# kolinko/effort

Measured on AMD Instinct MI355X. Metric: effective GB/s + tokens/s vs effort %, Mistral-7B FFN 4096x11008 fp16, higher is better.
Workload: dtype f16

## Files before the change

### effort_amd/_lib.py

```python
from __future__ import annotations

import ctypes as C
import os
import subprocess

_HERE = os.path.dirname(os.path.abspath(__file__))
LAB_LIB_PATH = os.path.join(_HERE, "libeffort_hip_lab.so")
LIB_PATH = (LAB_LIB_PATH if os.environ.get("EFFORT_HIP_LIB") == "lab" else os.environ.get("EFFORT_HIP_LIB")) or os.path.join(_HERE, "libeffort_hip.so")

ERRORS = {
    -1: "EFFORT_ERR_ARG", -2: "EFFORT_ERR_SHAPE", -3: "EFFORT_ERR_EFFORT", -4: "EFFORT_ERR_HIP",
    -5: "EFFORT_ERR_KIND", -6: "EFFORT_ERR_CONVERT", -7: "EFFORT_ERR_BLAS", -8: "EFFORT_ERR_COMM",
}


class EffortError(RuntimeError):
    def __init__(self, code: int, where: str, detail: str = ""):
        self.code = code
        super().__init__(f"{where}: {ERRORS.get(code, code)} {detail}".strip())


def build(verbose: bool = False) -> str:
    cmd = ["make", "-C", os.path.join(_HERE, "csrc"), "-j8", "all"]
    res = subprocess.run(cmd, capture_output=not verbose, text=True)
    if res.returncode != 0:
        raise RuntimeError("building libeffort_hip.so failed:\n" + (res.stdout or "") + (res.stderr or ""))
    return LIB_PATH


_P = C.c_void_p
_SIGS = {
    "effort_create": (_P, [C.c_int, _P]),
    "effort_destroy": (None, [_P]),
    "effort_set_stream": (C.c_int, [_P, _P]),
    "effort_sync": (C.c_int, [_P]),
    "effort_set_overlap": (C.c_int, [_P, C.c_int]),
    "effort_set_row_reuse": (C.c_int, [_P, C.c_int]),
    "effort_join": (C.c_int, [_P]),
    "effort_last_error": (C.c_char_p, [_P]),
    "effort_version": (C.c_char_p, []),
    "effort_weights_fp16": (_P, [_P, _P, _P, _P, C.c_int, C.c_int, C.c_int, C.c_int]),
    "effort_weights_fp16_pitched": (_P, [_P, _P, C.c_int, _P, _P, C.c_int, C.c_int, C.c_int, C.c_int]),
    "effort_aligned_row_pitch": (C.c_int, [C.c_int]),
    "effort_weights_q4": (_P, [_P, _P, _P, _P, _P, C.c_int64, C.c_int, C.c_int, C.c_int]),
    "effort_weights_free": (None, [_P]),
    "effort_weights_refresh": (C.c_int, [_P]),
    "effort_weights_align_rows": (C.c_int, [_P]),
    "effort_weights_row_pitch": (C.c_int, [_P]),
    "effort_weights_get_bound": (C.c_int, [_P, C.POINTER(C.c_float)]),
    "effort_weights_set_bound": (C.c_int, [_P, C.POINTER(C.c_float)]),
    "effort_weights_column_shard": (_P, [_P, C.c_int, C.c_int]),
    "effort_comm_unique_id": (C.c_int, [_P]),
    "effort_comm_create": (C.c_int, [_P, C.c_int, C.c_int, _P]),
    "effort_comm_destroy": (C.c_int, [_P]),
    "effort_comm_rank": (C.c_int, [_P]),
    "effort_comm_world": (C.c_int, [_P]),
    "effort_allgather_outputs": (C.c_int, [_P, _P, _P, C.c_int]),
    "effort_bucketmul": (C.c_int, [_P, _P, _P, _P, _P, C.c_double]),
    "effort_bucketmul_q4": (C.c_int, [_P, _P, _P, _P, _P, C.c_double]),
    "effort_bucketmul_group": (C.c_int, [_P, C.c_int, _P, _P, _P, _P, _P]),
    "effort_bucketmul_q4_group": (C.c_int, [_P, C.c_int, _P, _P, _P, _P, _P]),
    "effort_bucketmul_group_fused": (C.c_int, [_P, C.c_int, _P, _P, _P, _P, _P, _P, _P, _P]),
    "effort_bucketmul_q4_group_fused": (C.c_int, [_P, C.c_int, _P, _P, _P, _P, _P, _P, _P, _P]),
    "effort_group_dispatch_count": (C.c_int, [_P, C.c_int, C.POINTER(C.c_uint32)]),
    "effort_group_cutoff": (C.c_int, [_P, C.c_int, C.POINTER(C.c_float)]),
    "effort_debug_occupancy": (C.c_int, [_P, C.c_int, C.c_int, C.c_int, C.c_int]),
    "effort_set_persistent": (C.c_int, [_P, C.c_int]),
    "effort_debug_hook_lane": (C.c_int, [_P, C.c_int]),
    "effort_add_rmsnorm_mul": (C.c_int, [_P, _P, _P, _P, _P, C.c_int]),
    "effort_rope_kv": (C.c_int, [_P, _P, _P, _P, _P, _P, _P, _P, C.c_int, C.c_int, C.c_int, C.c_int, C.c_float]),
    "effort_attention": (C.c_int, [_P, _P, _P, _P, _P, _P, C.c_int, C.c_int, C.c_int]),
    "effort_rope_attention": (C.c_int, [_P, _P, _P, _P, _P, _P, _P, _P, C.c_int, C.c_int, C.c_int, C.c_int, C.c_float]),
    "effort_silu_mul": (C.c_int, [_P, _P, _P, _P, C.c_int]),
    "effort_fetch_row": (C.c_int, [_P, _P, _P, _P, C.c_int]),
    "effort_argmax": (C.c_int, [_P, _P, C.c_int, _P, _P, _P, C.c_int]),
    "effort_decode_status": (C.c_int, [_P, C.POINTER(C.c_int)]),
    "effort_sample": (C.c_int, [_P, _P, C.c_int, _P, _P, _P, _P, C.c_int, _P, _P]),
    "effort_topk": (C.c_int, [_P, _P, C.c_int, C.c_int, _P, _P]),
    "effort_sample_bits": (C.c_uint32, [C.c_uint32, C.c_uint32, C.c_uint32, C.c_uint32]),
    "effort_convert_status": (C.c_int, [_P, C.POINTER(C.c_int)]),
    "effort_q4_outlier_count": (C.c_int64, [C.c_int, C.c_int, C.c_double]),
    "effort_convert_q4": (C.c_int, [_P, _P, C.c_int, C.c_int, C.c_double, _P, _P, _P, _P]),
    "effort_top2_softmax": (C.c_int, [_P, _P, C.c_int, _P, _P]),
    "effort_mix2": (C.c_int, [_P, _P, _P, _P, _P, C.c_int]),
    "effort_moe_route": (C.c_int, [_P, _P, _P, _P, C.c_int, C.c_int, _P, _P, _P]),
    "effort_mix2_add": (C.c_int, [_P, _P, _P, _P, _P, C.c_int]),
    "effort_dense_gemv": (C.c_int, [_P, _P, _P, _P, C.c_int, C.c_int]),
    "effort_dense_gemv_expert": (C.c_int, [_P, _P, _P, _P, _P, C.c_int, C.c_int, C.c_int]),
    "effort_set_dense_backend": (C.c_int, [_P, C.c_int]),
    "effort_last_dispatch_count": (C.c_int, [_P, C.POINTER(C.c_uint32)]),
    "effort_last_cutoff": (C.c_int, [_P, C.POINTER(C.c_float)]),
    "effort_calc_dispatch": (C.c_int, [_P, _P, _P, _P, C.c_double, _P, _P]),
    "effort_convert_fp16": (C.c_int, [_P, _P, C.c_int, C.c_int, _P, _P, _P]),
    "effort_convert_fp16_pitched": (C.c_int, [_P, _P, C.c_int, C.c_int, _P, C.c_int, _P, _P]),
    "effort_cosine": (C.c_int, [_P, _P, _P, C.c_int, C.POINTER(C.c_float)]),
    "effort_set_split_cutoff": (C.c_int, [_P, C.c_int]),
    "effort_set_tuning": (C.c_int, [_P, C.c_int, C.c_int, C.c_int]),
    "effort_is_lab_build": (C.c_int, []),
    "effort_enable_kernel_timing": (C.c_int, [_P, C.c_int]),
    "effort_debug_stamps": (C.c_int, [_P, C.POINTER(C.c_ulonglong)]),
    "effort_debug_slice_counts": (C.c_int, [_P, C.c_int, C.POINTER(C.c_uint32), C.c_int]),
    "effort_debug_plan": (C.c_int, [C.c_int, C.c_int, C.c_int, C.c_int, _P, _P, _P, _P, _P, _P, C.c_int, C.c_int, C.c_int, C.c_int, _P, _P, _P, _P, _P, _P, _P, _P, _P]),
    "effort_debug_check_bundle": (C.c_int, [C.c_int, C.c_int, C.c_int, C.c_int, C.c_int, C.c_int]),
    "effort_debug_variants": (C.c_int, [C.c_int, _P, C.c_int]),
    "effort_debug_last_variant": (C.c_int, [_P, C.c_int, _P]),
    "effort_debug_lanes": (C.c_int, [C.c_int, C.c_int, _P, C.c_int64, _P]),
    "effort_debug_trace": (C.c_int, [_P, C.POINTER(C.c_ulonglong), C.c_int]),
    "effort_kernel_clock": (C.c_int, [_P, C.POINTER(C.c_double), C.POINTER(C.c_int)]),
    "effort_kernel_timing": (C.c_int, [_P, C.POINTER(C.c_double), C.POINTER(C.c_double), C.POINTER(C.c_double), C.POINTER(C.c_int)]),
}

_lib = None


def lib() -> C.CDLL:
    global _lib
    if _lib is None:
        if not os.path.exists(LIB_PATH):
            raise RuntimeError(
                f"{LIB_PATH} is missing: the HIP extension has not been built "
                "(run `python -c 'import __graft_entry__ as g; g.build()'` or `make -C effort_amd/csrc`). "
                "effort_amd has no CPU fallback.")
        import torch
        l = C.CDLL(LIB_PATH)
        for name, (res, args) in _SIGS.items():
            if (name.startswith("effort_debug_") or name == "effort_is_lab_build") and os.environ.get("EFFORT_HIP_LIB") and not hasattr(l, name):
                continue
            fn = getattr(l, name)
            fn.restype = res
            fn.argtypes = args
        _lib = l
    return _lib


def exported_symbols() -> list[str]:
    return sorted(_SIGS)
```

### effort_amd/csrc/api.hip

```cpp
#include <dlfcn.h>
#include <rccl/rccl.h>
#include <rocblas/rocblas.h>

#include <cstdio>
#include <cstring>
#include <map>
#include <mutex>
#include <new>
#include <vector>

#include "../../include/effort_hip.h"
#include "../../include/effort_hip_debug.h"
#include "effort_internal.h"
#include "lanes.h"
#include "plan.h"
#include "sample_device.h"

using namespace effort;

static constexpr size_t kStampBytes = (size_t)(kTraceOff + kTraceItems * 12) * 8;

struct Lane {
    hipStream_t own = nullptr;
    hipEvent_t done = nullptr;
    bool dirty = false;
    float* d_cutoff = nullptr;
    uint32_t* d_count = nullptr;
    float* d_slabs = nullptr;
    uint32_t* d_counters = nullptr;
    uint32_t* d_sliceCounts = nullptr;
    uint32_t* d_queue = nullptr;
    uint32_t lastCalls = 1, lastSliceOff[effort::kMaxGroup] = {0}, lastSlices[effort::kMaxGroup] = {0};
    uint32_t lastLaunches = 0;
    effort::LaunchedVariant lastVariant[effort::kMaxLaunches] = {};
};

struct effort_ctx {
    static constexpr int kMaxLanes = effort::kMaxLanes;
    int device = 0;
    hipStream_t stream = nullptr;
    int numCU = 256;
    Lane lane[kMaxLanes];
    LaneBook book;
    int lastLane = 0;
    hipEvent_t forkEv = nullptr;
    size_t slabBytes = 0;
    uint32_t* d_blockScratch = nullptr;
    uint16_t* d_vhalf = nullptr;
    size_t vhalfElems = 0;
    float* d_cos = nullptr;
    uint16_t* d_convVals = nullptr;
    size_t convElems = 0;
    int* d_status = nullptr;
    int persistent = -1;
    static constexpr uint32_t kMaxTiles = 1024, kMaxSlices = 4096;
    static constexpr size_t kSlabBytes = (size_t)64 << 20;
    unsigned long long* d_tstamp = nullptr;
    double wallClockKHz = 100000.0;
    rocblas_handle blas = nullptr;
    ncclComm_t comm = nullptr;
    int commRank = 0, commWorld = 1;
    bool denseRocblas = false;
    int tuneW = 0, tuneE = 0, tuneS = 0;
    bool splitCutoff = false;
    bool rowReuse = false;
    bool timing = false;
    bool clock = false;
    bool trace = false;
    static constexpr int kMaxSamples = 4096;
    hipEvent_t* ev = nullptr;
    int nSamples = 0;
    char err[256] = {0};
};

struct effort_w {
    effort_ctx* ctx = nullptr;
    Format fmt = kFp16;
    const uint16_t* buckets = nullptr;
    const uint16_t* bucketsSrc = nullptr;
    uint16_t* aligned = nullptr;
    uint32_t rowPitch = 0;
    uint32_t srcPitch = 0;
    const void* stats = nullptr;
    const uint16_t* probes = nullptr;
    uint32_t inDim = 0, outDim = 0, rowsPerIn = 0, numExperts = 1, cols = 0;
    bool view = false;
    effort_w* parent = nullptr;
    uint32_t viewTrim = 0;
    int views = 0;
    bool dead = false;
    float* rankBound = nullptr;
    uint16_t* means16 = nullptr;
    uint64_t nOutliers = 0;
    uint32_t* olBlockPtr = nullptr;
    uint32_t* olEntry = nullptr;
    uint32_t* olMeta = nullptr;
};

static int fail(effort_ctx* c, int code, const char* what, hipError_t e = hipSuccess) {
    if (c) {
        if (e != hipSuccess) snprintf(c->err, sizeof(c->err), "%s: %s", what, hipGetErrorString(e));
        else snprintf(c->err, sizeof(c->err), "%s", what);
    }
    return code;
}
#define HIP_TRY(ctx, call)                                                   \
    do {                                                                     \
        hipError_t e_ = (call);                                              \
        if (e_ != hipSuccess) return fail((ctx), EFFORT_ERR_HIP, #call, e_); \
    } while (0)

struct RcclApi {
    void* lib = nullptr;
    ncclResult_t (*GetUniqueId)(ncclUniqueId*) = nullptr;
    ncclResult_t (*CommInitRank)(ncclComm_t*, int, ncclUniqueId, int) = nullptr;
    ncclResult_t (*CommDestroy)(ncclComm_t) = nullptr;
    ncclResult_t (*AllGather)(const void*, void*, size_t, ncclDataType_t, ncclComm_t, hipStream_t) = nullptr;
    const char* (*GetErrorString)(ncclResult_t) = nullptr;
    bool ok = false;
};
static const RcclApi& rccl() {
    static RcclApi api = [] {
        RcclApi a;
        for (const char* name : {"librccl.so.1", "librccl.so", "/opt/rocm/lib/librccl.so.1", "/opt/rocm/lib/librccl.so"}) {
            a.lib = dlopen(name, RTLD_NOW | RTLD_GLOBAL);
            if (a.lib) break;
        }
        if (!a.lib) return a;
        a.GetUniqueId = reinterpret_cast<decltype(a.GetUniqueId)>(dlsym(a.lib, "ncclGetUniqueId"));
        a.CommInitRank = reinterpret_cast<decltype(a.CommInitRank)>(dlsym(a.lib, "ncclCommInitRank"));
        a.CommDestroy = reinterpret_cast<decltype(a.CommDestroy)>(dlsym(a.lib, "ncclCommDestroy"));
        a.AllGather = reinterpret_cast<decltype(a.AllGather)>(dlsym(a.lib, "ncclAllGather"));
        a.GetErrorString = reinterpret_cast<decltype(a.GetErrorString)>(dlsym(a.lib, "ncclGetErrorString"));
        a.ok = a.GetUniqueId && a.CommInitRank && a.CommDestroy && a.AllGather && a.GetErrorString;
        return a;
    }();
    return api;
}

extern "C" const char* effort_version(void) { return "effort-hip 0.1 (gfx950)"; }
static char g_createErr[256] = "null context";
extern "C" const char* effort_last_error(effort_ctx* c) { return c ? c->err : g_createErr; }

static bool lane_alloc(effort_ctx* c, Lane& L) {
    bool ok = hipMalloc(&L.d_cutoff, 512) == hipSuccess && hipMalloc(&L.d_count, 16) == hipSuccess &&
              hipMalloc(&L.d_slabs, c->slabBytes) == hipSuccess && hipMalloc(&L.d_counters, effort_ctx::kMaxTiles * 4) == hipSuccess &&
              hipMalloc(&L.d_sliceCounts, effort_ctx::kMaxSlices * 4) == hipSuccess && hipMalloc(&L.d_queue, kQueueWords * 4) == hipSuccess;
    if (!ok) return false;
    hipMemset(L.d_counters, 0, effort_ctx::kMaxTiles * 4);
    hipMemset(L.d_sliceCounts, 0, effort_ctx::kMaxSlices * 4);
    hipMemset(L.d_queue, 0, kQueueWords * 4);
    hipMemset(L.d_cutoff, 0, 512);
    hipMemset(L.d_count, 0, 16);
    return true;
}
static std::mutex g_poolMutex;
static std::map<int, std::vector<hipStream_t>> g_streamPool;
static std::map<int, std::vector<hipEvent_t>> g_eventPool;
static hipStream_t pool_stream(int device) {
    std::lock_guard<std::mutex> lk(g_poolMutex);
    auto& pool = g_streamPool[device];
    if (!pool.empty()) { hipStream_t s = pool.back(); pool.pop_back(); return s; }
    hipStream_t s = nullptr;
    return hipStreamCreateWithFlags(&s, hipStreamNonBlocking) == hipSuccess ? s : nullptr;
}
static hipEvent_t pool_event(int device) {
    std::lock_guard<std::mutex> lk(g_poolMutex);
    auto& pool = g_eventPool[device];
    if (!pool.empty()) { hipEvent_t e = pool.back(); pool.pop_back(); return e; }
    hipEvent_t e = nullptr;
    return hipEventCreateWithFlags(&e, hipEventDisableTiming) == hipSuccess ? e : nullptr;
}
static void pool_put(int device, hipStream_t s) { if (s) { std::lock_guard<std::mutex> lk(g_poolMutex); g_streamPool[device].push_back(s); } }
static void pool_put(int device, hipEvent_t e) { if (e) { std::lock_guard<std::mutex> lk(g_poolMutex); g_eventPool[device].push_back(e); } }

static void lane_free(int device, Lane& L) {
    pool_put(device, L.own);
    pool_put(device, L.done);
    hipFree(L.d_cutoff); hipFree(L.d_count); hipFree(L.d_slabs); hipFree(L.d_counters); hipFree(L.d_sliceCounts); hipFree(L.d_queue);
    L = Lane();
}

extern "C" effort_ctx* effort_create(int device, void* stream) {
    if (hipSetDevice(device) != hipSuccess) return nullptr;
    effort_ctx* c = new (std::nothrow) effort_ctx();
    if (!c) return nullptr;
    c->device = device;
    c->stream = reinterpret_cast<hipStream_t>(stream);
    hipDeviceProp_t prop;
    if (hipGetDeviceProperties(&prop, device) == hipSuccess) c->numCU = prop.multiProcessorCount;
    c->slabBytes = effort_ctx::kSlabBytes;
    {
        static std::mutex m; static std::map<int, bool> prepared;
        std::lock_guard<std::mutex> lk(m);
        if (!prepared[device]) {
            const hipError_t pe = bucket_mul_prepare_device();
            if (pe != hipSuccess) { snprintf(g_createErr, sizeof(g_createErr), "effort_create: kernel attributes: %s", hipGetErrorString(pe)); delete c; return nullptr; }
            prepared[device] = true;
        }
    }
    bool ok = lane_alloc(c, c->lane[0]) && hipMalloc(&c->d_blockScratch, 4096 * 4) == hipSuccess &&
              hipMalloc(&c->d_cos, 16) == hipSuccess && hipMalloc(&c->d_status, 16) == hipSuccess &&
              hipMalloc(&c->d_tstamp, kStampBytes) == hipSuccess;
    if (!ok) { snprintf(g_createErr, sizeof(g_createErr), "effort_create: out of device memory for the context scratch"); effort_destroy(c); return nullptr; }
    int khz = 0;
    if (hipDeviceGetAttribute(&khz, hipDeviceAttributeWallClockRate, device) == hipSuccess && khz > 0) c->wallClockKHz = khz;
    hipMemset(c->d_tstamp, 0, kStampBytes);
    { unsigned long long init[2] = {~0ull, 0ull}; hipMemcpy(c->d_tstamp, init, 16, hipMemcpyHostToDevice); }
    hipMemset(c->d_status, 0, 16);
    return c;
}

static hipError_t lane_mark(Lane& L) {
    if (!L.dirty) return hipSuccess;
    const hipError_t e = hipEventRecord(L.done, L.own);
    if (e == hipSuccess) L.dirty = false;
    return e;
}
static hipError_t wait_for_lanes(effort_ctx* c, hipStream_t st, uint32_t set) {
    for (int i = 0; i < effort_ctx::kMaxLanes; i++) if (set >> i & 1u) {
        hipError_t e = lane_mark(c->lane[i]);
        if (e == hipSuccess) e = hipStreamWaitEvent(st, c->lane[i].done, 0);
        if (e != hipSuccess) return e;
    }
    return hipSuccess;
}
static unsigned long long capture_of(hipStream_t st) {
    hipStreamCaptureStatus cap = hipStreamCaptureStatusNone;
    unsigned long long id = 0;
    if (hipStreamGetCaptureInfo(st, &cap, &id) != hipSuccess) { (void)hipGetLastError(); return 0; }
    return cap == hipStreamCaptureStatusActive ? (id ? id : ~0ull) : 0ull;
}
static bool lanes_match_capture(effort_ctx* c, unsigned long long now) {
    uint32_t dropped = 0;
    if (!c->book.match_capture(now, &dropped)) { snprintf(c->err, sizeof(c->err), "%s", kLanesPendingBeforeCapture); return false; }
    for (int i = 0; i < effort_ctx::kMaxLanes; i++) if (dropped >> i & 1u) c->lane[i].dirty = false;
    return true;
}
static int join_lanes(effort_ctx* c) {
    if (c->book.pending_lanes()) {
        if (!lanes_match_capture(c, capture_of(c->stream))) return EFFORT_ERR_ARG;
        const hipError_t e = wait_for_lanes(c, c->stream, c->book.pending_lanes());
        if (e != hipSuccess) { snprintf(c->err, sizeof(c->err), "join: %s", hipGetErrorString(e)); return EFFORT_ERR_HIP; }
    }
    c->book.join();
    return EFFORT_OK;
}
struct LaneChoice {
    bool laned = false;
    LanePick pick;
    LaunchRanges ranges;
    unsigned long long capNow = 0;
    bool forked = false;
};
static int choose_lane(effort_ctx* c, LaneChoice& lc, int n, const effort_w* const* ws, const float* const* vs, const uint32_t* const* expNos,
                       float* const* outs, const void* const* vAux, const float* const* resids) {
    if (lc.laned) {
        lc.capNow = capture_of(c->stream);
        if (!lanes_match_capture(c, lc.capNow)) return EFFORT_ERR_ARG;
        if (c->book.full()) { const int jrc = join_lanes(c); if (jrc != EFFORT_OK) return jrc; }
        for (int i = 0; i < n; i++)
            lc.ranges.call(vs[i], expNos ? expNos[i] : nullptr, vAux ? vAux[i] : nullptr, resids ? resids[i] : nullptr, outs[i], ws[i]->inDim, ws[i]->outDim);
        lc.pick = c->book.pick(lc.ranges);
    } else if (c->book.nLanes > 1) {
        { const int jrc = join_lanes(c); if (jrc != EFFORT_OK) return jrc; }
    }
    return EFFORT_OK;
}
static int fork_lane(effort_ctx* c, LaneChoice& lc) {
    if (!lc.laned || lc.forked) return EFFORT_OK;
    Lane& L = c->lane[lc.pick.lane];
    bool wait = true;
    if (lc.capNow == 0) {
        const hipError_t q = hipStreamQuery(c->stream);
        if (q == hipSuccess) wait = false;
        else {
            (void)hipGetLastError();
            if (q != hipErrorNotReady) return fail(c, EFFORT_ERR_HIP, "hipStreamQuery", q);
        }
    }
    if (wait) {
        HIP_TRY(c, hipEventRecord(c->forkEv, c->stream));
        HIP_TRY(c, hipStreamWaitEvent(L.own, c->forkEv, 0));
    }
    lc.forked = true;
    L.dirty = true;
    const uint32_t waits = c->book.commit(lc.pick, lc.ranges, lc.capNow, wait);
    const hipError_t e = wait_for_lanes(c, L.own, waits);
    if (e != hipSuccess) { c->book.keep_pending(waits, lc.capNow); return fail(c, EFFORT_ERR_HIP, "lane wait", e); }
    return EFFORT_OK;
}

extern "C" int effort_set_overlap(effort_ctx* c, int lanes) {
    if (!c || lanes < 1 || lanes > effort_ctx::kMaxLanes) return EFFORT_ERR_ARG;
    hipSetDevice(c->device);
    int rc = join_lanes(c);
    if (rc != EFFORT_OK) return rc;
    if (lanes > 1) {
        if (!c->forkEv && !(c->forkEv = pool_event(c->device))) return fail(c, EFFORT_ERR_HIP, "set_overlap: event");
        for (int i = 0; i < lanes; i++) {
            Lane& L = c->lane[i];
            if (!L.d_slabs && !lane_alloc(c, L)) return fail(c, EFFORT_ERR_HIP, "set_overlap: out of device memory for a lane's scratch");
            if (!L.own && !(L.own = pool_stream(c->device))) return fail(c, EFFORT_ERR_HIP, "set_overlap: stream");
            if (!L.done && !(L.done = pool_event(c->device))) return fail(c, EFFORT_ERR_HIP, "set_overlap: event");
        }
    }
    c->book.reset(lanes); c->lastLane = 0;
    return EFFORT_OK;
}
extern "C" int effort_join(effort_ctx* c) {
    if (!c) return EFFORT_ERR_ARG;
    return join_lanes(c);
}

extern "C" void effort_destroy(effort_ctx* c) {
    if (!c) return;
    hipSetDevice(c->device);
    for (int i = 0; i < effort_ctx::kMaxLanes; i++) if (c->lane[i].own) hipStreamSynchronize(c->lane[i].own);
    hipStreamSynchronize(c->stream);
    if (c->comm) rccl().CommDestroy(c->comm);
    if (c->blas) rocblas_destroy_handle(c->blas);
    if (c->ev) { for (int i = 0; i < effort_ctx::kMaxSamples * 4; i++) if (c->ev[i]) hipEventDestroy(c->ev[i]); delete[] c->ev; }
    for (int i = 0; i < effort_ctx::kMaxLanes; i++) lane_free(c->device, c->lane[i]);
    pool_put(c->device, c->forkEv);
    hipFree(c->d_blockScratch); hipFree(c->d_vhalf); hipFree(c->d_cos); hipFree(c->d_convVals); hipFree(c->d_status); hipFree(c->d_tstamp);
    delete c;
}

extern "C" int effort_set_stream(effort_ctx* c, void* stream) {
    if (!c) return EFFORT_ERR_ARG;
    if (reinterpret_cast<hipStream_t>(stream) != c->stream && join_lanes(c) != EFFORT_OK) return EFFORT_ERR_HIP;
    c->stream = reinterpret_cast<hipStream_t>(stream);
    if (c->blas) rocblas_set_stream(c->blas, c->stream);
    return EFFORT_OK;
}

extern "C" int effort_sync(effort_ctx* c) {
    if (!c) return EFFORT_ERR_ARG;
    { const int jrc = join_lanes(c); if (jrc != EFFORT_OK) return jrc; }
    HIP_TRY(c, hipStreamSynchronize(c->stream));
    return EFFORT_OK;
}

static int check_shape(uint32_t inDim, uint32_t outDim) {
    if (inDim < (uint32_t)kProbes || outDim == 0 || outDim % 32 || outDim > 16384) return EFFORT_ERR_SHAPE;
    return EFFORT_OK;
}
static int check_bundle(Format fmt, int inDim, int outDim, int percentLoad, int numExperts, int rowPitchBytes, uint32_t* pitchOut) {
    if (inDim <= 0 || outDim <= 0 || numExperts < 1 || inDim > 65535 || check_shape((uint32_t)inDim, (uint32_t)outDim) != EFFORT_OK) return EFFORT_ERR_SHAPE;
    int pitch;
    if (fmt == kFp16) {
        if (percentLoad < 1 || percentLoad > 16) return EFFORT_ERR_SHAPE;
        pitch = rowPitchBytes ? rowPitchBytes : outDim / 16 * 2;
        if (pitch < outDim / 16 * 2 || pitch % 4) return EFFORT_ERR_SHAPE;
    } else {
        if (rowPitchBytes) return EFFORT_ERR_SHAPE;
        percentLoad = 8; pitch = outDim / 32 * 2;
    }
    const size_t rows = (size_t)numExperts * (size_t)percentLoad * (size_t)inDim;
    if (rows * (size_t)pitch > 0xFFFFFFFFull || rows * 8u > 0xFFFFFFFFull) return EFFORT_ERR_SHAPE;
    if (pitchOut) *pitchOut = (uint32_t)pitch;
    return EFFORT_OK;
}
extern "C" int effort_debug_check_bundle(int q4, int inDim, int outDim, int percentLoad, int numExperts, int rowPitchBytes) {
    return check_bundle(q4 ? kQ4 : kFp16, inDim, outDim, percentLoad, numExperts, rowPitchBytes, nullptr);
}

static int register_bound(effort_ctx* c, effort_w* w) {
    hipSetDevice(c->device);
    const size_t rows = (size_t)w->numExperts * w->rowsPerIn * w->inDim;
    float* scratch = nullptr;
    bool ok = (w->rankBound || hipMalloc(&w->rankBound, (size_t)w->numExperts * 4) == hipSuccess) && hipMalloc(&scratch, rows * 4) == hipSuccess;
    if (ok) ok = launch_rank_bound(w->fmt, w->bucketsSrc, w->srcPitch / 2u, w->stats, w->numExperts, w->rowsPerIn, w->inDim, w->cols, scratch, w->rankBound, c->stream) == hipSuccess;
    if (ok && w->fmt == kFp16) {
        ok = w->means16 || hipMalloc(&w->means16, rows * 2) == hipSuccess;
        if (ok) ok = launch_compact_means(w->stats, w->means16, (uint32_t)rows, c->stream) == hipSuccess;
    }
    if (ok) ok = hipStreamSynchronize(c->stream) == hipSuccess;
    hipFree(scratch);
    return ok ? EFFORT_OK : fail(c, EFFORT_ERR_HIP, "weight registration: rank bound");
}

extern "C" int effort_aligned_row_pitch(int outDim) {
    if (outDim <= 0 || outDim % 32 || outDim > 16384) return EFFORT_ERR_SHAPE;
    return (outDim / 16 * 2 + 127) / 128 * 128;
}

extern "C" effort_w* effort_weights_fp16_pitched(effort_ctx* c, const void* buckets, int rowPitchBytes, const void* stats, const void* probes,
                                                 int inDim, int outDim, int percentLoad, int numExperts) {
    if (!c || !buckets || !stats || !probes) { fail(c, EFFORT_ERR_ARG, "effort_weights_fp16: null argument"); return nullptr; }
    uint32_t pitch = 0;
    if (check_bundle(kFp16, inDim, outDim, percentLoad, numExperts, rowPitchBytes, &pitch) != EFFORT_OK) {
        fail(c, EFFORT_ERR_SHAPE, "effort_weights_fp16: unsupported shape or row pitch (a multiple of 4 bytes >= 2*cols; buckets < 4 GiB; stats, 8 bytes a bucket row, < 4 GiB)"); return nullptr; }
    effort_w* w = new (std::nothrow) effort_w();
    if (!w) return nullptr;
    w->ctx = c; w->fmt = kFp16;
    w->buckets = static_cast<const uint16_t*>(buckets); w->stats = stats; w->probes = static_cast<const uint16_t*>(probes);
    w->inDim = inDim; w->outDim = outDim; w->rowsPerIn = percentLoad; w->numExperts = numExperts; w->cols = outDim / 16;
    w->bucketsSrc = w->buckets; w->rowPitch = w->srcPitch = pitch;
    if (register_bound(c, w) != EFFORT_OK) { effort_weights_free(w); return nullptr; }
    return w;
}
extern "C" effort_w* effort_weights_fp16(effort_ctx* c, const void* buckets, const void* stats, const void* probes,
                                         int inDim, int outDim, int percentLoad, int numExperts) {
    return effort_weights_fp16_pitched(c, buckets, 0, stats, probes, inDim, outDim, percentLoad, numExperts);
}

extern "C" effort_w* effort_weights_q4(effort_ctx* c, const void* buckets, const void* stats, const void* probes,
                                       const void* outliers, int64_t nOutliers, int inDim, int outDim, int numExperts) {
    if (!c || !buckets || !stats || !probes) { fail(c, EFFORT_ERR_ARG, "effort_weights_q4: null argument"); return nullptr; }
    if (nOutliers < 0 || check_bundle(kQ4, inDim, outDim, 8, numExperts, 0, nullptr) != EFFORT_OK) {
        fail(c, EFFORT_ERR_SHAPE, "effort_weights_q4: unsupported shape (or buckets >= 4 GiB, or stats, 8 bytes a bucket row, >= 4 GiB)"); return nullptr; }
    effort_w* w = new (std::nothrow) effort_w();
    if (!w) return nullptr;
    w->ctx = c; w->fmt = kQ4;
    w->buckets = static_cast<const uint16_t*>(buckets); w->stats = stats; w->probes = static_cast<const uint16_t*>(probes);
    w->inDim = inDim; w->outDim = outDim; w->rowsPerIn = 8; w->numExperts = numExperts; w->cols = outDim / 32;
    w->bucketsSrc = w->buckets; w->rowPitch = w->srcPitch = w->cols * 2u;
    if (register_bound(c, w) != EFFORT_OK) { effort_weights_free(w); return nullptr; }
    if (outliers && nOutliers > 0) {
        if (outDim > 65536) { fail(c, EFFORT_ERR_SHAPE, "effort_weights_q4: outliers need outDim <= 65536"); effort_weights_free(w); return nullptr; }
        hipSetDevice(c->device);
        {
            int bad[2] = {0, 0};
            bool okv = hipMemsetAsync(c->d_status + 2, 0, 8, c->stream) == hipSuccess &&
                       launch_validate_outliers(static_cast<const float*>(outliers), (uint64_t)nOutliers, (uint32_t)inDim, (uint32_t)outDim, c->d_status + 2, c->stream) == hipSuccess &&
                       hipMemcpyAsync(bad, c->d_status + 2, 8, hipMemcpyDeviceToHost, c->stream) == hipSuccess && hipStreamSynchronize(c->stream) == hipSuccess;
            if (!okv || bad[0] || bad[1]) {
                fail(c, okv ? EFFORT_ERR_ARG : EFFORT_ERR_HIP, !okv ? "effort_weights_q4: outlier validation" :
                     bad[0] ? "effort_weights_q4: outlier entries outside the matrix (inIdx >= inDim or outIdx >= outDim)"
                            : "effort_weights_q4: outlier values that are not f16 numbers (the table comes from an f16 matrix, q4_draft.py:58-67)");
                effort_weights_free(w); return nullptr;
            }
        }
        uint32_t *tmp = nullptr, *rowPtr = nullptr;
        w->nOutliers = (uint64_t)nOutliers;
        const uint32_t olBlocks = ((uint32_t)outDim + 63u) / 64u;
        bool ok = hipMalloc(&rowPtr, ((size_t)outDim + 2) * 4) == hipSuccess && hipMalloc(&w->olBlockPtr, ((size_t)olBlocks + 1) * 4) == hipSuccess &&
                  hipMalloc(&w->olMeta, (size_t)olBlocks * 64 * 4) == hipSuccess &&
                  hipMalloc(&w->olEntry, ((size_t)nOutliers + 64) * 4) == hipSuccess && hipMalloc(&tmp, 4 * (size_t)nOutliers * 4) == hipSuccess;
        if (ok) ok = hipMemsetAsync(w->olEntry + (size_t)nOutliers, 0, 64 * 4, c->stream) == hipSuccess;
        if (ok) ok = launch_build_outlier_index(static_cast<const float*>(outliers), w->nOutliers, (uint32_t)inDim, (uint32_t)outDim, rowPtr, w->olBlockPtr,
                                                w->olEntry, w->olMeta, tmp, c->stream) == hipSuccess;
        if (ok) ok = hipStreamSynchronize(c->stream) == hipSuccess;
        hipFree(tmp);
        uint32_t longest = 0;
        if (ok) ok = hipMemcpy(&longest, rowPtr + (size_t)outDim + 1, 4, hipMemcpyDeviceToHost) == hipSuccess;
        hipFree(rowPtr);
        if (!ok) { fail(c, EFFORT_ERR_HIP, "effort_weights_q4: outlier index"); effort_weights_free(w); return nullptr; }
        if (longest >= (1u << 24)) { fail(c, EFFORT_ERR_SHAPE, "effort_weights_q4: more than 2^24 outliers on one output"); effort_weights_free(w); return nullptr; }
    }
    return w;
}

static int copy_aligned(effort_w* w) {
    const size_t rows = (size_t)w->numExperts * w->rowsPerIn * w->inDim;
    HIP_TRY(w->ctx, hipMemcpy2DAsync(w->aligned, w->rowPitch, w->bucketsSrc, w->srcPitch, (size_t)w->cols * 2, rows, hipMemcpyDeviceToDevice, w->ctx->stream));
    HIP_TRY(w->ctx, hipStreamSynchronize(w->ctx->stream));
    return EFFORT_OK;
}
extern "C" int effort_weights_refresh(effort_w* w) {
    if (!w || !w->ctx || w->dead) return EFFORT_ERR_ARG;
    if (w->view) return fail(w->ctx, EFFORT_ERR_ARG, "effort_weights_refresh: a column shard takes its bound from the full handle -- refresh that one and shard again");
    hipSetDevice(w->ctx->device);
    int rc = join_lanes(w->ctx);
    if (rc == EFFORT_OK) rc = register_bound(w->ctx, w);
    if (rc == EFFORT_OK && w->aligned) rc = copy_aligned(w);
    return rc;
}
extern "C" int effort_weights_align_rows(effort_w* w) {
    if (!w || !w->ctx || w->dead) return EFFORT_ERR_ARG;
    if (w->aligned || w->rowPitch % 128u == 0u) return EFFORT_OK;
    hipSetDevice(w->ctx->device);
    const uint32_t pitch = (w->cols * 2u + 127u) / 128u * 128u;
    const size_t rows = (size_t)w->numExperts * w->rowsPerIn * w->inDim;
    if (rows * pitch > 0xFFFFFFFFull) return fail(w->ctx, EFFORT_ERR_SHAPE, "effort_weights_align_rows: the padded buckets would reach 4 GiB");
    if (hipMalloc(&w->aligned, rows * pitch) != hipSuccess) return fail(w->ctx, EFFORT_ERR_HIP, "effort_weights_align_rows: out of device memory");
    HIP_TRY(w->ctx, hipMemsetAsync(w->aligned, 0, rows * pitch, w->ctx->stream));
    w->rowPitch = pitch;
    const int rc = copy_aligned(w);
    if (rc != EFFORT_OK) { hipFree(w->aligned); w->aligned = nullptr; w->rowPitch = w->srcPitch; return rc; }
    w->buckets = w->aligned;
    return EFFORT_OK;
}
extern "C" int effort_weights_row_pitch(const effort_w* w) { return w ? (int)w->rowPitch : EFFORT_ERR_ARG; }
extern "C" int effort_weights_get_bound(effort_w* w, float* host_out) {
    if (!w || !w->ctx || !host_out || !w->rankBound) return EFFORT_ERR_ARG;
    HIP_TRY(w->ctx, hipMemcpy(host_out, w->rankBound, (size_t)w->numExperts * 4, hipMemcpyDeviceToHost));
    return EFFORT_OK;
}
extern "C" int effort_weights_set_bound(effort_w* w, const float* host_in) {
    if (!w || !w->ctx || !host_in || !w->rankBound || w->dead) return EFFORT_ERR_ARG;
    for (uint32_t e = 0; e < w->numExperts; e++) if (!(host_in[e] >= 0.0f)) return EFFORT_ERR_ARG;
    { const int jrc = join_lanes(w->ctx); if (jrc != EFFORT_OK) return jrc; }
    HIP_TRY(w->ctx, hipStreamSynchronize(w->ctx->stream));
    HIP_TRY(w->ctx, hipMemcpy(w->rankBound, host_in, (size_t)w->numExperts * 4, hipMemcpyHostToDevice));
    return EFFORT_OK;
}

static std::mutex g_viewMutex;
extern "C" void effort_weights_free(effort_w* w) {
    if (!w) return;
    if (w->view) {
        effort_w* const par = w->parent;
        hipFree(w->rankBound);
        delete w;
        bool last = false;
        if (par) { std::lock_guard<std::mutex> lk(g_viewMutex); last = --par->views == 0 && par->dead; if (last) par->dead = false; }
        if (last) effort_weights_free(par);
        return;
    }
    {
        std::lock_guard<std::mutex> lk(g_viewMutex);
        if (w->views > 0) { w->dead = true; return; }
    }
    hipFree(w->olBlockPtr); hipFree(w->olEntry); hipFree(w->olMeta);
    hipFree(w->aligned); hipFree(w->rankBound); hipFree(w->means16);
    delete w;
}

extern "C" effort_w* effort_weights_column_shard(const effort_w* full, int rank, int world) {
    if (!full || !full->ctx) return nullptr;
    effort_ctx* c = full->ctx;
    const uint32_t unit = full->fmt == kFp16 ? 16u : 32u;
    if (world < 1 || rank < 0 || rank >= world || full->cols % (uint32_t)world || (full->cols / (uint32_t)world) % 2u) {
        fail(c, EFFORT_ERR_SHAPE, "effort_weights_column_shard: the bucket columns must split evenly into an even number per rank"); return nullptr; }
    const uint32_t per = full->cols / (uint32_t)world, outDim = per * unit;
    if (check_shape(full->inDim, outDim) != EFFORT_OK) { fail(c, EFFORT_ERR_SHAPE, "effort_weights_column_shard: shard shape"); return nullptr; }
    if (full->nOutliers && outDim % 64u) {
        fail(c, EFFORT_ERR_SHAPE, "effort_weights_column_shard: the shard must hold whole blocks of the outlier index"); return nullptr; }
    effort_w* w = new (std::nothrow) effort_w();
    if (!w) return nullptr;
    {
        std::lock_guard<std::mutex> lk(g_viewMutex);
        if (full->view || full->dead) { fail(c, EFFORT_ERR_ARG, "effort_weights_column_shard: shard a full, live handle"); delete w; return nullptr; }
        const_cast<effort_w*>(full)->views++;
    }
    *w = *full;
    w->view = true; w->parent = const_cast<effort_w*>(full); w->views = 0; w->dead = false;
    w->aligned = nullptr; w->rankBound = nullptr;
    w->buckets = full->buckets + (size_t)rank * per;
    w->viewTrim = (uint32_t)((size_t)rank * per * 2u);
    w->bucketsSrc = w->buckets; w->srcPitch = full->rowPitch;
    w->cols = per; w->outDim = outDim;
    hipSetDevice(c->device);
    if (hipMalloc(&w->rankBound, (size_t)w->numExperts * 4) != hipSuccess ||
        hipMemcpy(w->rankBound, full->rankBound, (size_t)w->numExperts * 4, hipMemcpyDeviceToDevice) != hipSuccess) {
        fail(c, EFFORT_ERR_HIP, "effort_weights_column_shard: bound"); hipFree(w->rankBound);
        effort_w* const par = w->parent;
        delete w;
        bool last;
        { std::lock_guard<std::mutex> lk(g_viewMutex); last = --par->views == 0 && par->dead; if (last) par->dead = false; }
        if (last) effort_weights_free(par);
        return nullptr; }
    if (full->nOutliers) {
        w->olBlockPtr = full->olBlockPtr + (size_t)rank * outDim / 64u;
        w->olMeta = full->olMeta + (size_t)rank * outDim;
    }
    return w;
}
extern "C" int effort_comm_unique_id(void* id_out) {
    if (!id_out) return EFFORT_ERR_ARG;
    static_assert(sizeof(ncclUniqueId) == EFFORT_COMM_ID_BYTES, "effort_hip.h: EFFORT_COMM_ID_BYTES");
    if (!rccl().ok) return EFFORT_ERR_COMM;
    return rccl().GetUniqueId(static_cast<ncclUniqueId*>(id_out)) == ncclSuccess ? EFFORT_OK : EFFORT_ERR_COMM;
}
extern "C" int effort_comm_create(effort_ctx* c, int rank, int world, const void* id) {
    if (!c || !id || world < 1 || rank < 0 || rank >= world) return fail(c, EFFORT_ERR_ARG, "comm_create: bad argument");
    if (c->comm) return fail(c, EFFORT_ERR_ARG, "comm_create: the context has a communicator already");
    hipSetDevice(c->device);
    ncclUniqueId uid;
    memcpy(&uid, id, sizeof(uid));
    if (!rccl().ok) return fail(c, EFFORT_ERR_COMM, "comm_create: librccl.so could not be opened (dlopen) -- multi-GPU needs RCCL");
    const ncclResult_t r = rccl().CommInitRank(&c->comm, world, uid, rank);
    if (r != ncclSuccess) { c->comm = nullptr; snprintf(c->err, sizeof(c->err), "ncclCommInitRank: %s", rccl().GetErrorString(r)); return EFFORT_ERR_COMM; }
    c->commRank = rank; c->commWorld = world;
    return EFFORT_OK;
}
extern "C" int effort_comm_destroy(effort_ctx* c) {
    if (!c) return EFFORT_ERR_ARG;
    if (c->comm) { hipSetDevice(c->device); effort_sync(c); rccl().CommDestroy(c->comm); c->comm = nullptr; c->commRank = 0; c->commWorld = 1; }
    return EFFORT_OK;
}
extern "C" int effort_comm_rank(effort_ctx* c) { return c ? c->commRank : EFFORT_ERR_ARG; }
extern "C" int effort_comm_world(effort_ctx* c) { return c ? c->commWorld : EFFORT_ERR_ARG; }
extern "C" int effort_allgather_outputs(effort_ctx* c, const float* send, float* recv, int count) {
    if (!c || !send || !recv || count < 1) return fail(c, EFFORT_ERR_ARG, "allgather_outputs: bad argument");
    if (!c->comm) return fail(c, EFFORT_ERR_ARG, "allgather_outputs: no communicator (effort_comm_create)");
    { const int jrc = join_lanes(c); if (jrc != EFFORT_OK) return jrc; }
    const ncclResult_t r = rccl().AllGather(send, recv, (size_t)count, ncclFloat, c->comm, c->stream);
    if (r != ncclSuccess) { snprintf(c->err, sizeof(c->err), "ncclAllGather: %s", rccl().GetErrorString(r)); return EFFORT_ERR_COMM; }
    return EFFORT_OK;
}

static int ensure_timing(effort_ctx* c) {
    if (c->ev) return EFFORT_OK;
    c->ev = new (std::nothrow) hipEvent_t[effort_ctx::kMaxSamples * 4]();
    if (!c->ev) return EFFORT_ERR_HIP;
    for (int i = 0; i < effort_ctx::kMaxSamples * 4; i++) HIP_TRY(c, hipEventCreate(&c->ev[i]));
    return EFFORT_OK;
}

static PlanEnv plan_env(const effort_ctx* c, bool laned, bool thinEffort) {
    PlanEnv env;
    env.numCU = c->numCU; env.nLanes = c->book.nLanes; env.laned = laned;
    env.persistent = c->persistent; env.tuneW = c->tuneW; env.tuneE = c->tuneE; env.tuneS = c->tuneS;
    env.splitCutoff = c->splitCutoff; env.clock = c->clock;
    env.slabBytes = c->slabBytes; env.maxTiles = effort_ctx::kMaxTiles; env.maxSlices = effort_ctx::kMaxSlices;
    env.thinEffort = thinEffort;
#ifdef EFFORT_LAB
    static const uint32_t ablate = getenv("EFFORT_ABLATE") ? (uint32_t)atoi(getenv("EFFORT_ABLATE")) : 0u;
    static const bool noJobs = getenv("EFFORT_NO_CUTJOBS") != nullptr, noCompact = getenv("EFFORT_NO_COMPACT_MEANS") != nullptr;
    env.ablate = ablate; env.noJobs = noJobs; env.noCompact = noCompact;
    if (getenv("EFFORT_TAIL_CALLS")) {
        env.tailCalls = atoi(getenv("EFFORT_TAIL_CALLS"));
        env.tailMult = getenv("EFFORT_TAIL_MULT") ? atoi(getenv("EFFORT_TAIL_MULT")) : 2;
    }
#endif
    return env;
}
static PlanCall plan_call(const effort_w* w, int pre, bool resid) {
    return PlanCall{w->inDim, w->outDim, w->cols, w->rowsPerIn, w->rowPitch, w->numExperts, w->means16 != nullptr, (uint16_t)pre, resid};
}
static bool thin_effort(int n, const double* efforts) {
    double sum = 0.0;
    for (int i = 0; i < n; i++) sum += efforts[i];
    return sum < 0.08 * n;
}

static int do_group(effort_ctx* c, Format fmt, int n, const effort_w* const* ws, const float* const* vs,
                    const uint32_t* const* expNos, float* const* outs, const double* efforts,
                    const int* prologues = nullptr, const void* const* vAux = nullptr, const float* const* resids = nullptr) {
    if (!c || !ws || !vs || !outs || !efforts) return fail(c, EFFORT_ERR_ARG, "bucketmul: null argument");
    if (n < 1 || n > kMaxGroup) return fail(c, EFFORT_ERR_ARG, "bucketmul: group size outside 1..32");
    PlanCall pc[kMaxGroup];
    for (int i = 0; i < n; i++) {
        if (!ws[i] || !vs[i] || !outs[i]) return fail(c, EFFORT_ERR_ARG, "bucketmul: null argument");
        if (ws[i]->dead) return fail(c, EFFORT_ERR_ARG, "bucketmul: the handle was freed (its buffers live on only for its column shards)");
        if (ws[i]->fmt != fmt) return fail(c, EFFORT_ERR_KIND, "bucketmul: weight handle of the wrong kind");
        if (!(efforts[i] >= 0.0 && efforts[i] <= 1.0)) return fail(c, EFFORT_ERR_EFFORT, "bucketmul: effort outside [0,1]");
        const int pre = prologues ? prologues[i] : 0;
        if (pre < 0 || pre > 2 || (pre && (!vAux || !vAux[i]))) return fail(c, EFFORT_ERR_ARG, "bucketmul: bad input prologue");
        if (pre && c->splitCutoff) return fail(c, EFFORT_ERR_KIND, "bucketmul: input prologues need the fused cutoff");
        if (pre && fmt == kQ4 && ws[i]->olBlockPtr && (uint32_t)ws[i]->inDim > bucket_mul_ol_lds_floats())
            return fail(c, EFFORT_ERR_SHAPE, "bucketmul: an input prologue on a Q4 handle with outliers needs inDim <= 16384 (materialise the input, or register without outliers)");
        pc[i] = plan_call(ws[i], pre, resids && resids[i]);
    }
    LaneChoice lc;
    lc.laned = c->book.nLanes > 1 && !c->timing && !c->clock;
    const PlanEnv env = plan_env(c, lc.laned, thin_effort(n, efforts));
    GroupPlan plan;
    if (plan_group(fmt, env, n, pc, &plan) != EFFORT_OK) return fail(c, plan.err, plan.msg);
    const bool tm = c->timing && c->nSamples < effort_ctx::kMaxSamples;
    hipEvent_t* ev = tm ? c->ev + 4 * c->nSamples : nullptr;
    { const int lrc = choose_lane(c, lc, n, ws, vs, expNos, outs, vAux, resids); if (lrc != EFFORT_OK) return lrc; }
    Lane& L = c->lane[lc.pick.lane];
    const hipStream_t st = lc.laned ? L.own : c->stream;
    c->lastLane = lc.pick.lane;
    if (tm) HIP_TRY(c, hipEventRecord(ev[0], st));
    L.lastLaunches = 0;
    for (uint32_t l = 0; l < plan.nLaunches; l++) {
        const LaunchPlan& lp = plan.launch[l];
        GroupKArgs ga;
        memset(&ga, 0, sizeof(ga));
        ga.groupDone = L.d_counters + effort_ctx::kMaxTiles - 1;
        ga.slabs = L.d_slabs; ga.counters = L.d_counters; ga.sliceCounts = L.d_sliceCounts; ga.cutoff = L.d_cutoff + lp.first;
        ga.tstamp = c->clock ? c->d_tstamp : nullptr;
        ga.ablate = env.ablate; ga.trace = (c->clock && c->trace) ? 1u : 0u;
        ga.split = (c->splitCutoff ? 1u : 0u) | (lp.compact ? 4u : 0u) | (c->rowReuse ? 8u : 0u);
        ga.numCU = (uint32_t)c->numCU; ga.queue = L.d_queue;
        ga.count = lp.count; ga.totalTiles = lp.totalTiles; ga.totalItems = lp.totalItems;
        ga.persistent = lp.persistent; ga.cutJobs = lp.cutJobs; ga.staggerSleeps = lp.staggerSleeps;
        for (uint32_t k = 0; k < lp.count; k++) {
            const int i = (int)(lp.first + k);
            const effort_w* w = ws[i];
            const CallPlan& p = plan.call[i];
            CallDesc& a = ga.call[k];
            a.buckets = w->buckets; a.stats = lp.compact ? (const void*)w->means16 : w->stats; a.rankBound = w->rankBound; a.probes = w->probes; a.v = vs[i];
            a.expNo = expNos ? expNos[i] : nullptr; a.out = outs[i];
            a.ol = OutlierIndex{fmt == kQ4 ? w->olBlockPtr : nullptr, w->olEntry, w->olMeta};
            a.q = (uint16_t)(int)((double)(kProbes - 1) * (1.0 - efforts[i]));
            a.bucketsTrim = (uint16_t)w->viewTrim;
            a.pre = pc[i].pre; a.vAux = a.pre ? vAux[i] : nullptr; a.resid = resids ? resids[i] : nullptr;
            a.slabOff = p.slabOff; a.tileOff = (uint16_t)p.tileOff; a.sliceOff = (uint16_t)p.sliceOff; a.geom = (uint16_t)p.geom;
            ga.geom[p.geom] = p.g;
            ga.wgEnd8[k] = (uint16_t)p.itemEnd8;
            L.lastSliceOff[i] = p.sliceOff; L.lastSlices[i] = p.g.slices;
        }
        { const int frc = fork_lane(c, lc); if (frc != EFFORT_OK) return frc; }
        if (c->splitCutoff && !(env.ablate & 1u)) HIP_TRY(c, launch_find_cutoff_group(ga, st));
        HIP_TRY(c, launch_bucket_mul(fmt, plan.W, plan.E, ga, st, &L.lastVariant[l]));
        L.lastLaunches = l + 1u;
    }
    L.lastCalls = (uint32_t)n;
    if (tm) { HIP_TRY(c, hipEventRecord(ev[1], st)); c->nSamples++; }
    return EFFORT_OK;
}

extern "C" int effort_bucketmul(effort_ctx* c, const effort_w* w, const float* v, const uint32_t* expNo, float* out, double effort) {
    return do_group(c, kFp16, 1, &w, &v, &expNo, &out, &effort);
}
extern "C" int effort_bucketmul_q4(effort_ctx* c, const effort_w* w, const float* v, const uint32_t* expNo, float* out, double effort) {
    return do_group(c, kQ4, 1, &w, &v, &expNo, &out, &effort);
}
extern "C" int effort_bucketmul_group(effort_ctx* c, int n, const effort_w* const* ws, const float* const* vs,
                                      const uint32_t* const* expNos, float* const* outs, const double* efforts) {
    return do_group(c, kFp16, n, ws, vs, expNos, outs, efforts);
}
extern "C" int effort_bucketmul_group_fused(effort_ctx* c, int n, const effort_w* const* ws, const float* const* vs,
                                            const uint32_t* const* expNos, float* const* outs, const double* efforts,
                                            const int* prologues, const void* const* vAux, const float* const* resids) {
    return do_group(c, kFp16, n, ws, vs, expNos, outs, efforts, prologues, vAux, resids);
}
extern "C" int effort_bucketmul_q4_group_fused(effort_ctx* c, int n, const effort_w* const* ws, const float* const* vs,
                                               const uint32_t* const* expNos, float* const* outs, const double* efforts,
                                               const int* prologues, const void* const* vAux, const float* const* resids) {
    return do_group(c, kQ4, n, ws, vs, expNos, outs, efforts, prologues, vAux, resids);
}
extern "C" int effort_bucketmul_q4_group(effort_ctx* c, int n, const effort_w* const* ws, const float* const* vs,
                                         const uint32_t* const* expNos, float* const* outs, const double* efforts) {
    return do_group(c, kQ4, n, ws, vs, expNos, outs, efforts);
}

extern "C" int effort_calc_dispatch(effort_ctx* c, const effort_w* w, const float* v, const uint32_t* expNo, double effort,
                                    float* dispatch, uint32_t* count) {
    if (!c || !w || !v || !dispatch || w->dead) return fail(c, EFFORT_ERR_ARG, "calc_dispatch: null argument (or a freed handle)");
    if (!(effort >= 0.0 && effort <= 1.0)) return fail(c, EFFORT_ERR_EFFORT, "calc_dispatch: effort outside [0,1]");
    { const int jrc = join_lanes(c); if (jrc != EFFORT_OK) return jrc; }
    Lane& L = c->lane[0];
    c->lastLane = 0;
    const PlanCall pc = plan_call(w, 0, false);
    GroupPlan plan;
    if (plan_group(w->fmt, plan_env(c, false, false), 1, &pc, &plan) != EFFORT_OK) return fail(c, plan.err, "calc_dispatch: geometry");
    const MulGeom& g = plan.call[0].g;
    const uint32_t q = (uint32_t)(int)((double)(kProbes - 1) * (1.0 - effort));
    HIP_TRY(c, launch_find_cutoff(v, w->probes, expNo, q, L.d_cutoff, L.d_count, nullptr, c->stream));
    HIP_TRY(c, launch_calc_dispatch(w->fmt, w->stats, v, expNo, L.d_cutoff, g, dispatch, count, L.d_count, c->d_blockScratch, c->stream));
    L.lastCalls = 1; L.lastSlices[0] = 0;
    L.lastLaunches = 0;
    return EFFORT_OK;
}

extern "C" int effort_group_dispatch_count(effort_ctx* c, int idx, uint32_t* host_out) {
    if (!c || !host_out || idx < 0 || (uint32_t)idx >= c->lane[c->lastLane].lastCalls) return EFFORT_ERR_ARG;
    { const int jrc = join_lanes(c); if (jrc != EFFORT_OK) return jrc; }
    Lane& L = c->lane[c->lastLane];
    if (L.lastSlices[idx] == 0) {
        HIP_TRY(c, hipMemcpyAsync(host_out, L.d_count, 4, hipMemcpyDeviceToHost, c->stream));
        HIP_TRY(c, hipStreamSynchronize(c->stream));
        return EFFORT_OK;
    }
    static thread_local uint32_t h[effort_ctx::kMaxSlices];
    HIP_TRY(c, hipMemcpyAsync(h, L.d_sliceCounts + L.lastSliceOff[idx], (size_t)L.lastSlices[idx] * 4, hipMemcpyDeviceToHost, c->stream));
    HIP_TRY(c, hipStreamSynchronize(c->stream));
    uint32_t n = 0;
    for (uint32_t i = 0; i < L.lastSlices[idx]; i++) n += h[i];
    *host_out = n;
    return EFFORT_OK;
}
extern "C" int effort_debug_slice_counts(effort_ctx* c, int idx, uint32_t* host, int maxSlices) {
    if (!c || !host || idx < 0 || (uint32_t)idx >= c->lane[c->lastLane].lastCalls || maxSlices < 1) return EFFORT_ERR_ARG;
    { const int jrc = join_lanes(c); if (jrc != EFFORT_OK) return jrc; }
    Lane& L = c->lane[c->lastLane];
    const uint32_t n = L.lastSlices[idx] < (uint32_t)maxSlices ? L.lastSlices[idx] : (uint32_t)maxSlices;
    if (n) HIP_TRY(c, hipMemcpyAsync(host, L.d_sliceCounts + L.lastSliceOff[idx], (size_t)n * 4, hipMemcpyDeviceToHost, c->stream));
    HIP_TRY(c, hipStreamSynchronize(c->stream));
    return (int)n;
}
extern "C" int effort_debug_plan(int q4, int numCU, int lanes, int n, const int* inDim, const int* outDim, const int* percentLoad,
                                 const int* prologue, const int* hasResid, const double* effort, int persistent, int tuneW, int tuneE, int tuneS,
                                 int* we, int* slices, int* tiles, int* sliceRows, int* launchOf,
                                 int* launchPersistent, int* launchCutJobs, int* launchCompact, int* launchStagger) {
    if (numCU < 1 || lanes < 1 || lanes > effort_ctx::kMaxLanes || n < 1 || n > kMaxGroup || !inDim || !outDim || !effort || !we || !slices || !tiles ||
        !sliceRows || !launchOf || !launchPersistent || !launchCutJobs || !launchCompact || !launchStagger) return EFFORT_ERR_ARG;
    const Format fmt = q4 ? kQ4 : kFp16;
    effort_ctx c0;
    c0.numCU = numCU; c0.book.nLanes = lanes; c0.persistent = persistent; c0.tuneW = tuneW; c0.tuneE = tuneE; c0.tuneS = tuneS;
    c0.slabBytes = effort_ctx::kSlabBytes;
    PlanCall pc[kMaxGroup];
    for (int i = 0; i < n; i++) {
        const int load = q4 ? 8 : (percentLoad ? percentLoad[i] : 16);
        if (inDim[i] <= 0 || outDim[i] <= 0 || check_shape((uint32_t)inDim[i], (uint32_t)outDim[i]) != EFFORT_OK || load < 1 || load > 16) return EFFORT_ERR_SHAPE;
        if (!(effort[i] >= 0.0 && effort[i] <= 1.0)) return EFFORT_ERR_EFFORT;
        const uint32_t cols = (uint32_t)outDim[i] / (q4 ? 32u : 16u);
        pc[i] = PlanCall{(uint32_t)inDim[i], (uint32_t)outDim[i], cols, (uint32_t)load, cols * 2u, 1u, !q4, (uint16_t)(prologue ? prologue[i] : 0), hasResid && hasResid[i]};
    }
    GroupPlan plan;
    const int rc = plan_group(fmt, plan_env(&c0, lanes > 1, thin_effort(n, effort)), n, pc, &plan);
    if (rc != EFFORT_OK) return rc;
    we[0] = plan.W; we[1] = plan.E;
    for (int i = 0; i < n; i++) {
        const CallPlan& p = plan.call[i];
        slices[i] = (int)p.g.slices; tiles[i] = (int)p.g.tiles; sliceRows[i] = (int)p.g.sliceRows; launchOf[i] = (int)p.launch;
    }
    for (uint32_t l = 0; l < plan.nLaunches; l++) {
        const LaunchPlan& lp = plan.launch[l];
        launchPersistent[l] = (int)lp.persistent; launchCutJobs[l] = (int)lp.cutJobs; launchCompact[l] = lp.compact ? 1 : 0; launchStagger[l] = (int)lp.staggerSleeps;
    }
    return (int)plan.nLaunches;
}
extern "C" int effort_debug_variants(int q4, int* rows, int maxRows) {
    if (maxRows < 0 || (maxRows > 0 && !rows)) return EFFORT_ERR_ARG;
    return bucket_mul_variants(q4 ? kQ4 : kFp16, rows, maxRows);
}
extern "C" int effort_debug_last_variant(effort_ctx* c, int launch, int* out8) {
    if (!c || !out8 || launch < 0) return EFFORT_ERR_ARG;
    const Lane& L = c->lane[c->lastLane];
    if ((uint32_t)launch >= L.lastLaunches) return EFFORT_ERR_ARG;
    const LaunchedVariant& v = L.lastVariant[launch];
    const uint32_t w[8] = {v.W, v.E, v.fused, v.compact, v.lean, v.persistent, v.grid, v.totalItems};
    for (int i = 0; i < 8; i++) out8[i] = (int)w[i];
    return EFFORT_OK;
}
extern "C" int effort_group_cutoff(effort_ctx* c, int idx, float* host_out) {
    if (!c || !host_out || idx < 0 || (uint32_t)idx >= c->lane[c->lastLane].lastCalls) return EFFORT_ERR_ARG;
    { const int jrc = join_lanes(c); if (jrc != EFFORT_OK) return jrc; }
    Lane& L = c->lane[c->lastLane];
    HIP_TRY(c, hipMemcpyAsync(host_out, L.d_cutoff + idx, 4, hipMemcpyDeviceToHost, c->stream));
    HIP_TRY(c, hipStreamSynchronize(c->stream));
    return EFFORT_OK;
}
extern "C" int effort_last_dispatch_count(effort_ctx* c, uint32_t* host_out) { return effort_group_dispatch_count(c, 0, host_out); }
extern "C" int effort_last_cutoff(effort_ctx* c, float* host_out) { return effort_group_cutoff(c, 0, host_out); }

extern "C" int effort_set_dense_backend(effort_ctx* c, int rocblas) {
    if (!c) return EFFORT_ERR_ARG;
    c->denseRocblas = rocblas != 0;
    return EFFORT_OK;
}
extern "C" int effort_dense_gemv(effort_ctx* c, const void* W, const float* v, float* out, int inDim, int outDim) {
    if (!c || !W || !v || !out || inDim <= 0 || outDim <= 0) return fail(c, EFFORT_ERR_ARG, "dense_gemv: bad argument");
    { const int jrc = join_lanes(c); if (jrc != EFFORT_OK) return jrc; }
    if (inDim % 16) return fail(c, EFFORT_ERR_SHAPE, "dense_gemv: inDim % 16 != 0 (helpers/mps.swift:18)");
    if (!c->denseRocblas && dense_gemv_supported((uint32_t)inDim, (uint32_t)outDim)) {
        HIP_TRY(c, launch_dense_gemv(static_cast<const uint16_t*>(W), v, out, (uint32_t)inDim, (uint32_t)outDim, c->stream));
        return EFFORT_OK;
    }
    if (!c->blas) {
        if (rocblas_create_handle(&c->blas) != rocblas_status_success) return fail(c, EFFORT_ERR_BLAS, "rocblas_create_handle");
        rocblas_set_stream(c->blas, c->stream);
        rocblas_set_pointer_mode(c->blas, rocblas_pointer_mode_host);
    }
    if ((size_t)inDim > c->vhalfElems) {
        HIP_TRY(c, hipStreamSynchronize(c->stream));
        hipFree(c->d_vhalf); c->d_vhalf = nullptr; c->vhalfElems = 0;
        HIP_TRY(c, hipMalloc(&c->d_vhalf, (size_t)inDim * 2));
        c->vhalfElems = inDim;
    }
    HIP_TRY(c, launch_f32_to_f16(v, c->d_vhalf, inDim, c->stream));
    const float alpha = 1.0f, beta = 0.0f;
    rocblas_status s = rocblas_hssgemv_strided_batched(c->blas, rocblas_operation_transpose, inDim, outDim, &alpha,
                                                       static_cast<const rocblas_half*>(W), inDim, 0,
                                                       reinterpret_cast<const rocblas_half*>(c->d_vhalf), 1, 0, &beta, out, 1, 0, 1);
    if (s != rocblas_status_success) return fail(c, EFFORT_ERR_BLAS, "rocblas_hssgemv_strided_batched");
    return EFFORT_OK;
}
extern "C" int effort_dense_gemv_expert(effort_ctx* c, const void* W, const uint32_t* expNo, const float* v, float* out, int inDim, int outDim,
                                        int numExperts) {
    if (!c || !W || !expNo || !v || !out || inDim <= 0 || outDim <= 0 || numExperts <= 0) return fail(c, EFFORT_ERR_ARG, "dense_gemv_expert: bad argument");
    { const int jrc = join_lanes(c); if (jrc != EFFORT_OK) return jrc; }
    if (!dense_gemv_supported((uint32_t)inDim, (uint32_t)outDim) || (size_t)numExperts * outDim * inDim * 2 > 0xFFFFFFFFull)
        return fail(c, EFFORT_ERR_SHAPE, "dense_gemv_expert: inDim % 16 != 0, inDim > 65536, or a stack of 4 GiB or more");
    HIP_TRY(c, launch_dense_gemv_expert(static_cast<const uint16_t*>(W), expNo, v, out, (uint32_t)inDim, (uint32_t)outDim, (uint32_t)numExperts, c->stream));
    return EFFORT_OK;
}

extern "C" int effort_convert_fp16_pitched(effort_ctx* c, const void* W, int outDim, int inDim, void* buckets, int rowPitchBytes, void* stats, void* probes) {
    if (!c || !W || !buckets || !stats || !probes) return fail(c, EFFORT_ERR_ARG, "convert_fp16: null argument");
    { const int jrc = join_lanes(c); if (jrc != EFFORT_OK) return jrc; }
    if (outDim <= 0 || inDim < kProbes || !(outDim >= kProbes || kProbes % outDim == 0) || outDim > 16384 || inDim > 32000 ||
        outDim % 16 || (outDim / 16) % 4)
        return fail(c, EFFORT_ERR_CONVERT, "convert_fp16: bucketize preconditions violated");
    const int pitch = rowPitchBytes ? rowPitchBytes : outDim / 16 * 2;
    if (pitch < outDim / 16 * 2 || pitch % 8) return fail(c, EFFORT_ERR_CONVERT, "convert_fp16: row pitch must be a multiple of 8 bytes >= 2*cols");
    const size_t elems = (size_t)outDim * inDim;
    if (elems > c->convElems) {
        HIP_TRY(c, hipStreamSynchronize(c->stream));
        hipFree(c->d_convVals); c->d_convVals = nullptr; c->convElems = 0;
        HIP_TRY(c, hipMalloc(&c->d_convVals, elems * 2));
        c->convElems = elems;
    }
    HIP_TRY(c, launch_convert_fp16(static_cast<const uint16_t*>(W), outDim, inDim, static_cast<uint16_t*>(buckets), (uint32_t)pitch / 2u,
                                   static_cast<uint16_t*>(stats), static_cast<uint16_t*>(probes), c->d_convVals, c->d_status, c->stream));
    return EFFORT_OK;
}
extern "C" int effort_convert_fp16(effort_ctx* c, const void* W, int outDim, int inDim, void* buckets, void* stats, void* probes) {
    return effort_convert_fp16_pitched(c, W, outDim, inDim, buckets, 0, stats, probes);
}

extern "C" int64_t effort_q4_outlier_count(int inDim, int outDim, double perc) {
    if (inDim <= 0 || outDim <= 0 || !(perc >= 0.0 && perc <= 1.0)) return EFFORT_ERR_ARG;
    return (int64_t)((double)((int64_t)inDim * outDim) * perc);
}
extern "C" int effort_convert_q4(effort_ctx* c, const void* core2, int inDim, int outDim, double perc, void* buckets, void* stats, void* probes,
                                 void* outliers) {
    if (!c || !core2 || !buckets || !stats || !probes) return fail(c, EFFORT_ERR_ARG, "convert_q4: null argument");
    { const int jrc = join_lanes(c); if (jrc != EFFORT_OK) return jrc; }
    if (inDim <= 0 || outDim <= 0 || outDim % 32 || (int64_t)inDim * outDim >= (1ll << 32) || !(perc >= 0.0 && perc <= 1.0))
        return fail(c, EFFORT_ERR_CONVERT, "convert_q4: outDim % 32 != 0 (q4_draft.py:299), or a matrix of 2^32 elements or more");
    const int64_t cnt = effort_q4_outlier_count(inDim, outDim, perc);
    if (cnt >= (1ll << 31)) return fail(c, EFFORT_ERR_CONVERT, "convert_q4: 2^31 outliers or more (the candidate sort counts in int)");
    if (cnt > 0 && !outliers) return fail(c, EFFORT_ERR_ARG, "convert_q4: outliers buffer missing");
    hipSetDevice(c->device);
    HIP_TRY(c, launch_convert_q4(static_cast<const uint16_t*>(core2), (uint32_t)inDim, (uint32_t)outDim, (uint32_t)cnt, static_cast<uint16_t*>(buckets),
                                 static_cast<float*>(stats), static_cast<uint16_t*>(probes), static_cast<float*>(outliers), c->numCU, c->stream));
    return EFFORT_OK;
}

extern "C" int effort_cosine(effort_ctx* c, const float* a, const float* b, int n, float* host_out) {
    if (!c || !a || !b || !host_out || n <= 0) return EFFORT_ERR_ARG;
    { const int jrc = join_lanes(c); if (jrc != EFFORT_OK) return jrc; }
    HIP_TRY(c, launch_cosine(a, b, n, c->d_cos, c->stream));
    HIP_TRY(c, hipMemcpyAsync(host_out, c->d_cos, 4, hipMemcpyDeviceToHost, c->stream));
    HIP_TRY(c, hipStreamSynchronize(c->stream));
    return EFFORT_OK;
}

extern "C" int effort_add_rmsnorm_mul(effort_ctx* c, float* h, const float* delta, const void* w, float* out, int n) {
    if (!c || !h || !w || !out || n <= 0) return fail(c, EFFORT_ERR_ARG, "add_rmsnorm_mul: bad argument");
    { const int jrc = join_lanes(c); if (jrc != EFFORT_OK) return jrc; }
    HIP_TRY(c, launch_add_rmsnorm_mul(h, delta, static_cast<const uint16_t*>(w), out, (uint32_t)n, c->stream));
    return EFFORT_OK;
}
extern "C" int effort_rope_kv(effort_ctx* c, const float* xq, const float* xk, const float* xv, float* qOut, float* kCache,
                              float* vCache, const uint32_t* pos, int numHeads, int numHeadsKV, int headDim, int maxTokens, float ropeBase) {
    if (!c || !xq || !xk || !xv || !qOut || !kCache || !vCache || !pos) return fail(c, EFFORT_ERR_ARG, "rope_kv: null argument");
    { const int jrc = join_lanes(c); if (jrc != EFFORT_OK) return jrc; }
    if (numHeads <= 0 || numHeadsKV <= 0 || numHeads % numHeadsKV || headDim < 2 || headDim > 1024 || headDim % 2 || !(ropeBase > 1.0f) || maxTokens <= 0)
        return fail(c, EFFORT_ERR_SHAPE, "rope_kv: bad head geometry");
    HIP_TRY(c, launch_rope_kv(xq, xk, xv, qOut, kCache, vCache, pos, numHeads, numHeadsKV, headDim, ropeBase, (uint32_t)maxTokens, c->d_status + 1, c->stream));
    return EFFORT_OK;
}
extern "C" int effort_attention(effort_ctx* c, const float* q, const float* kCache, const float* vCache, const uint32_t* pos,
                                float* out, int numHeads, int headDim, int maxTokens) {
    if (!c || !q || !kCache || !vCache || !pos || !out) return fail(c, EFFORT_ERR_ARG, "attention: null argument");
    { const int jrc = join_lanes(c); if (jrc != EFFORT_OK) return jrc; }
    if (numHeads <= 0 || maxTokens <= 0 || maxTokens > 8192 || (headDim != 64 && headDim != 128 && headDim != 256))
        return fail(c, EFFORT_ERR_SHAPE, "attention: headDim 64/128/256, maxTokens <= 8192");
    HIP_TRY(c, launch_attention(q, kCache, vCache, pos, out, numHeads, headDim, maxTokens, c->stream));
    return EFFORT_OK;
}
extern "C" int effort_rope_attention(effort_ctx* c, const float* xq, const float* xk, const float* xv, float* kCache, float* vCache,
                                     const uint32_t* pos, float* out, int numHeads, int numHeadsKV, int headDim, int maxTokens, float ropeBase) {
    if (!c || !xq || !xk || !xv || !kCache || !vCache || !pos || !out) return fail(c, EFFORT_ERR_ARG, "rope_attention: null argument");
    { const int jrc = join_lanes(c); if (jrc != EFFORT_OK) return jrc; }
    if (numHeads <= 0 || numHeadsKV <= 0 || numHeads % numHeadsKV || maxTokens <= 0 || maxTokens > 8192 || !(ropeBase > 1.0f) ||
        (headDim != 64 && headDim != 128 && headDim != 256))
        return fail(c, EFFORT_ERR_SHAPE, "rope_attention: headDim 64/128/256, maxTokens <= 8192");
    HIP_TRY(c, launch_rope_attention(xq, xk, xv, kCache, vCache, pos, out, numHeads, numHeadsKV, headDim, maxTokens, ropeBase, c->d_status + 1, c->stream));
    return EFFORT_OK;
}
extern "C" int effort_silu_mul(effort_ctx* c, const float* x1, const float* x3, float* out, int n) {
    if (!c || !x1 || !x3 || !out || n <= 0) return fail(c, EFFORT_ERR_ARG, "silu_mul: bad argument");
    { const int jrc = join_lanes(c); if (jrc != EFFORT_OK) return jrc; }
    HIP_TRY(c, launch_silu_mul(x1, x3, out, (uint32_t)n, c->stream));
    return EFFORT_OK;
}
extern "C" int effort_fetch_row(effort_ctx* c, const void* emb, const uint32_t* id, float* out, int n) {
    if (!c || !emb || !id || !out || n <= 0) return fail(c, EFFORT_ERR_ARG, "fetch_row: bad argument");
    { const int jrc = join_lanes(c); if (jrc != EFFORT_OK) return jrc; }
    HIP_TRY(c, launch_fetch_row(static_cast<const uint16_t*>(emb), id, out, (uint32_t)n, c->stream));
    return EFFORT_OK;
}
extern "C" int effort_top2_softmax(effort_ctx* c, const float* gate, int n, uint32_t* idx2, float* val2) {
    if (!c || !gate || !idx2 || !val2 || n < 1) return fail(c, EFFORT_ERR_ARG, "top2_softmax: bad argument");
    { const int jrc = join_lanes(c); if (jrc != EFFORT_OK) return jrc; }
    HIP_TRY(c, launch_top2_softmax(gate, (uint32_t)n, idx2, val2, c->stream));
    return EFFORT_OK;
}
extern "C" int effort_mix2(effort_ctx* c, const float* f0, const float* f1, const float* val2, float* out, int n) {
    if (!c || !f0 || !f1 || !val2 || !out || n <= 0) return fail(c, EFFORT_ERR_ARG, "mix2: bad argument");
    { const int jrc = join_lanes(c); if (jrc != EFFORT_OK) return jrc; }
    HIP_TRY(c, launch_mix2(f0, f1, val2, out, (uint32_t)n, c->stream));
    return EFFORT_OK;
}
extern "C" int effort_moe_route(effort_ctx* c, const float* h, const void* normW, const void* gateW, int n, int numExperts, float* gateOut,
                                uint32_t* idx2, float* val2) {
    if (!c || !h || !normW || !gateW || !idx2 || !val2) return fail(c, EFFORT_ERR_ARG, "moe_route: null argument");
    { const int jrc = join_lanes(c); if (jrc != EFFORT_OK) return jrc; }
    if (n <= 0 || numExperts <= 0 || !moe_route_supported((uint32_t)n, (uint32_t)numExperts))
        return fail(c, EFFORT_ERR_SHAPE, "moe_route: n % 16 == 0, 16 <= n <= 16384, 1 <= numExperts <= 64");
    HIP_TRY(c, launch_moe_route(h, static_cast<const uint16_t*>(normW), static_cast<const uint16_t*>(gateW), (uint32_t)n, (uint32_t)numExperts, gateOut,
                                idx2, val2, c->stream));
    return EFFORT_OK;
}
extern "C" int effort_mix2_add(effort_ctx* c, float* h, const float* f0, const float* f1, const float* val2, int n) {
    if (!c || !h || !f0 || !f1 || !val2 || n <= 0) return fail(c, EFFORT_ERR_ARG, "mix2_add: bad argument");
    { const int jrc = join_lanes(c); if (jrc != EFFORT_OK) return jrc; }
    HIP_TRY(c, launch_mix2_add(h, f0, f1, val2, (uint32_t)n, c->stream));
    return EFFORT_OK;
}
extern "C" int effort_argmax(effort_ctx* c, const float* logits, int n, uint32_t* idOut, uint32_t* pos, uint32_t* history, int historyLen) {
    if (!c || !logits || !idOut || !pos || n <= 0 || (history && historyLen <= 0)) return fail(c, EFFORT_ERR_ARG, "argmax: bad argument");
    { const int jrc = join_lanes(c); if (jrc != EFFORT_OK) return jrc; }
    HIP_TRY(c, launch_argmax(logits, (uint32_t)n, idOut, pos, history, (uint32_t)(history ? historyLen : 0), c->d_status + 1, c->stream));
    return EFFORT_OK;
}
extern "C" int effort_sample(effort_ctx* c, const float* logits, int n, const effort_sample_params* params, uint32_t* idOut, uint32_t* pos,
                             uint32_t* history, int historyLen, uint32_t* topkIdx, float* topkVal) {
    if (!c || !logits || !params || !idOut || !pos || n <= 0 || (history && historyLen <= 0)) return fail(c, EFFORT_ERR_ARG, "sample: bad argument");
    { const int jrc = join_lanes(c); if (jrc != EFFORT_OK) return jrc; }
    HIP_TRY(c, launch_sample(logits, (uint32_t)n, params, idOut, pos, history, (uint32_t)(history ? historyLen : 0), c->d_status + 1, topkIdx, topkVal,
                             c->stream));
    return EFFORT_OK;
}
extern "C" int effort_topk(effort_ctx* c, const float* logits, int n, int k, uint32_t* idx, float* val) {
    if (!c || !logits || !idx || !val || n <= 0 || k < 1 || k > EFFORT_SAMPLE_MAX_K) return fail(c, EFFORT_ERR_ARG, "topk: bad argument (1 <= k <= 64)");
    { const int jrc = join_lanes(c); if (jrc != EFFORT_OK) return jrc; }
    HIP_TRY(c, launch_topk(logits, (uint32_t)n, (uint32_t)k, idx, val, c->stream));
    return EFFORT_OK;
}
extern "C" uint32_t effort_sample_bits(uint32_t seedLo, uint32_t seedHi, uint32_t stream, uint32_t pos) { return philox_x0(seedLo, seedHi, stream, pos); }
extern "C" int effort_decode_status(effort_ctx* c, int* host_out) {
    if (!c || !host_out) return EFFORT_ERR_ARG;
    { const int jrc = join_lanes(c); if (jrc != EFFORT_OK) return jrc; }
    HIP_TRY(c, hipMemcpyAsync(host_out, c->d_status + 1, 4, hipMemcpyDeviceToHost, c->stream));
    HIP_TRY(c, hipMemsetAsync(c->d_status + 1, 0, 4, c->stream));
    HIP_TRY(c, hipStreamSynchronize(c->stream));
    return EFFORT_OK;
}
extern "C" int effort_convert_status(effort_ctx* c, int* host_out) {
    if (!c || !host_out) return EFFORT_ERR_ARG;
    { const int jrc = join_lanes(c); if (jrc != EFFORT_OK) return jrc; }
    HIP_TRY(c, hipMemcpyAsync(host_out, c->d_status, 4, hipMemcpyDeviceToHost, c->stream));
    HIP_TRY(c, hipMemsetAsync(c->d_status, 0, 4, c->stream));
    HIP_TRY(c, hipStreamSynchronize(c->stream));
    return EFFORT_OK;
}

extern "C" int effort_set_tuning(effort_ctx* c, int W, int E, int S) {
    if (!c) return EFFORT_ERR_ARG;
    if ((W || E) && !supported(W ? W : 16, E ? E : 1)) return fail(c, EFFORT_ERR_ARG, "set_tuning: unsupported (waves, elems)");
    if (S < 0) return EFFORT_ERR_ARG;
    c->tuneW = W; c->tuneE = E; c->tuneS = S;
    return EFFORT_OK;
}

extern "C" int effort_debug_occupancy(effort_ctx* c, int q4, int W, int E, int ldsBytes) {
    if (!c || !supported(W, E)) return EFFORT_ERR_ARG;
    return bucket_mul_occupancy(q4 ? kQ4 : kFp16, W, E, (size_t)ldsBytes);
}

extern "C" int effort_set_persistent(effort_ctx* c, int wgPerCU) {
    if (!c || wgPerCU < -1 || wgPerCU > 8) return EFFORT_ERR_ARG;
    c->persistent = wgPerCU;
    return EFFORT_OK;
}

extern "C" int effort_debug_hook_lane(effort_ctx* c, int lane) {
    if (!c || lane < 0 || lane >= c->book.nLanes) return EFFORT_ERR_ARG;
    c->lastLane = lane;
    return EFFORT_OK;
}

extern "C" int effort_set_row_reuse(effort_ctx* c, int reuse) {
    if (!c) return EFFORT_ERR_ARG;
    c->rowReuse = reuse != 0;
    return EFFORT_OK;
}

extern "C" int effort_set_split_cutoff(effort_ctx* c, int split) {
    if (!c) return EFFORT_ERR_ARG;
    c->splitCutoff = split != 0;
    return EFFORT_OK;
}

#ifdef EFFORT_LAB
static constexpr bool kLabBuild = true;
#else
static constexpr bool kLabBuild = false;
#endif
static int lab_only(effort_ctx* c) { return fail(c, EFFORT_ERR_KIND, "device-clock stamps / traces are compiled into libeffort_hip_lab.so only (EFFORT_HIP_LIB=lab)"); }
extern "C" int effort_is_lab_build(void) { return kLabBuild ? 1 : 0; }

extern "C" int effort_enable_kernel_timing(effort_ctx* c, int enable) {
    if (!c) return EFFORT_ERR_ARG;
    if (!kLabBuild && enable >= 2) return lab_only(c);
    if (enable == 1) { int rc = ensure_timing(c); if (rc != EFFORT_OK) return rc; }
    c->timing = enable == 1;
    c->clock = kLabBuild && enable != 0;
    c->trace = kLabBuild && enable == 3;
    if (c->trace) HIP_TRY(c, hipMemsetAsync(c->d_tstamp + kTraceOff, 0, (size_t)kTraceItems * 96, c->stream));
    c->nSamples = 0;
    HIP_TRY(c, hipMemsetAsync(c->d_tstamp, 0, 4096, c->stream));
    HIP_TRY(c, hipMemsetAsync(c->d_tstamp, 0xFF, 8, c->stream));
    return EFFORT_OK;
}

extern "C" int effort_debug_stamps(effort_ctx* c, unsigned long long* host32) {
    if (!c || !host32) return EFFORT_ERR_ARG;
    if (!kLabBuild) return lab_only(c);
    HIP_TRY(c, hipMemcpyAsync(host32, c->d_tstamp + 8, 192, hipMemcpyDeviceToHost, c->stream));
    unsigned long long lines[32 * 8];
    HIP_TRY(c, hipMemcpyAsync(lines, c->d_tstamp + 64, sizeof(lines), hipMemcpyDeviceToHost, c->stream));
    HIP_TRY(c, hipStreamSynchronize(c->stream));
    for (int i = 0; i < 8; i++) { host32[24 + i] = 0; for (int l = 0; l < 32; l++) host32[24 + i] += lines[l * 8 + i]; }
    return EFFORT_OK;
}

extern "C" int effort_debug_trace(effort_ctx* c, unsigned long long* host, int maxRecords) {
    if (!c || !host || maxRecords < 1 || maxRecords > kTraceItems) return EFFORT_ERR_ARG;
    if (!kLabBuild) return lab_only(c);
    HIP_TRY(c, hipMemcpyAsync(host, c->d_tstamp + kTraceOff, (size_t)maxRecords * 64, hipMemcpyDeviceToHost, c->stream));
    HIP_TRY(c, hipMemcpyAsync(host + (size_t)maxRecords * 8, c->d_tstamp + kTraceOff + (size_t)kTraceItems * 8, (size_t)maxRecords * 32, hipMemcpyDeviceToHost, c->stream));
    HIP_TRY(c, hipStreamSynchronize(c->stream));
    return EFFORT_OK;
}

extern "C" int effort_kernel_clock(effort_ctx* c, double* mul_us_avg, int* n_launches) {
    if (!c) return EFFORT_ERR_ARG;
    if (!kLabBuild) return lab_only(c);
    unsigned long long h[4] = {0, 0, 0, 0};
    HIP_TRY(c, hipMemcpyAsync(h, c->d_tstamp, 32, hipMemcpyDeviceToHost, c->stream));
    HIP_TRY(c, hipStreamSynchronize(c->stream));
// ... 23 lines not shown
```

### effort_amd/csrc/bucket_mul.hip

```cpp
#include <cstring>
#include <type_traits>

#include "cutoff_device.h"

namespace effort {

constexpr int kBatch = 16;
template <int E> __host__ __device__ constexpr int batch_rows() { return E >= 4 ? 8 : kBatch; }
constexpr int kRounds = 16;

#ifndef EFFORT_ABLATE_NOSCATTER
#define EFFORT_ABLATE_NOSCATTER 0
#endif
#ifndef EFFORT_ABLATE_NOLOAD
#define EFFORT_ABLATE_NOLOAD 0
#endif

constexpr int kMinWavesPerEU = 4;

#ifndef EFFORT_ROW_AUX
#define EFFORT_ROW_AUX 2
#endif
constexpr int kRowAux = EFFORT_ROW_AUX;
#define GA_PERSISTENT(ga) (PERSIST ? (ga).persistent : 0u)
#define GA_CUTJOBS(ga) (PERSIST ? (ga).cutJobs : 0u)
#ifndef EFFORT_LAB
#define EFFORT_PRODUCT_ONLY 1
#if defined(EFFORT_CUT_FINE) || defined(EFFORT_LEAN_STAMPS) || EFFORT_ABLATE_NOSCATTER || EFFORT_ABLATE_NOLOAD
#error "lab switches need -DEFFORT_LAB (they belong in libeffort_hip_lab.so / build/variants, never in the shipped library)"
#endif
#endif
#ifdef EFFORT_PRODUCT_ONLY
constexpr bool kProductOnly = true;
#else
constexpr bool kProductOnly = false;
#endif
#ifdef EFFORT_PRODUCT_ONLY
#define GA_TSTAMP(ga) ((unsigned long long*)nullptr)
#define GA_ABLATE(ga) 0u
#define GA_TRACE(ga) 0u
#elif defined(EFFORT_LEAN_STAMPS)
#define GA_TSTAMP(ga) ((ga).tstamp)
#define GA_ABLATE(ga) (PERSIST ? (ga).ablate : 0u)
#define GA_TRACE(ga) 0u
#else
#define GA_TSTAMP(ga) (PERSIST ? (ga).tstamp : nullptr)
#define GA_ABLATE(ga) (PERSIST ? (ga).ablate : 0u)
#define GA_TRACE(ga) (PERSIST ? (ga).trace : 0u)
#endif
#ifdef EFFORT_LEAN_STAMPS
constexpr bool kLeanStamps = true;
#else
constexpr bool kLeanStamps = false;
#endif
constexpr uint32_t kMaxLdsBytes = 160u * 1024u - 1024u;
constexpr int kSc1 = 16;

template <int FMT> struct Fmt;
template <> struct Fmt<kFp16> { static constexpr int kAcc = 16, kSlots = 16; };
template <> struct Fmt<kQ4> { static constexpr int kAcc = 32, kSlots = 64; };

template <int FMT> struct MeanT;
template <> struct MeanT<kFp16> { typedef uint16_t type; };
template <> struct MeanT<kQ4> { typedef float type; };

template <int E> struct Piece;
template <> struct Piece<1> {
    uint32_t w;
    template <int AUX> __device__ __forceinline__ void load(__amdgpu_buffer_rsrc_t r, uint32_t voff, uint32_t soff) { w = __builtin_amdgcn_raw_buffer_load_b16(r, voff, soff, AUX); }
    __device__ __forceinline__ uint32_t word(int) const { return w & 0xFFFFu; }
    __device__ __forceinline__ uint32_t dword(int) const { return w; }
};
template <> struct Piece<2> {
    uint32_t w;
    template <int AUX> __device__ __forceinline__ void load(__amdgpu_buffer_rsrc_t r, uint32_t voff, uint32_t soff) { w = __builtin_amdgcn_raw_buffer_load_b32(r, voff, soff, AUX); }
    __device__ __forceinline__ uint32_t word(int j) const { return (w >> (16 * j)) & 0xFFFFu; }
    __device__ __forceinline__ uint32_t dword(int) const { return w; }
};
template <> struct Piece<4> {
    uint32_t w[2];
    template <int AUX> __device__ __forceinline__ void load(__amdgpu_buffer_rsrc_t r, uint32_t voff, uint32_t soff) {
        auto t = __builtin_amdgcn_raw_buffer_load_b64(r, voff, soff, AUX); w[0] = t[0]; w[1] = t[1];
    }
    __device__ __forceinline__ uint32_t word(int j) const { return (w[j >> 1] >> (16 * (j & 1))) & 0xFFFFu; }
    __device__ __forceinline__ uint32_t dword(int j) const { return w[j >> 1]; }
};
__host__ __device__ inline uint32_t align_up(uint32_t x, uint32_t a) { return (x + a - 1) / a * a; }

constexpr int kOlBatch = 16;
constexpr uint32_t kOlLdsFloats = 16384;
template <int E> __host__ __device__ inline uint32_t ol_outputs_per_item(const MulGeom& g) { return align_up((32u * E * 64u + g.slices - 1u) / g.slices, 64u); }
constexpr uint32_t kOlEarlyFloats = 4096;
constexpr int kOlMerged = 8;
constexpr uint32_t kOlSumFloats = 1024;
template <int E> __host__ __device__ inline uint32_t ol_scratch_bytes(const MulGeom& g) {
    const uint32_t per = ol_outputs_per_item<E>(g);
    return (per > kOlSumFloats ? per : kOlSumFloats) * 4u + (g.inDim <= kOlLdsFloats ? g.inDim * 4u : 0u);
}

template <int FMT, int E, int W>
__host__ __device__ inline LdsPlan plan_lds(const MulGeom* geoms, int nGeoms, bool merge) {
    uint32_t slots = 0, vrows = 0, ol = 0, vEarly = 0;
    for (int i = 0; i < nGeoms; i++) {
        const MulGeom& g = geoms[i];
        if (!g.slices) continue;
        slots = slots > g.slots ? slots : g.slots;
        const uint32_t vr = align_up(g.sliceRows, 64);
        vrows = vrows > vr ? vrows : vr;
        if (FMT != kFp16) {
            const uint32_t x = ol_scratch_bytes<E>(g); ol = ol > x ? ol : x;
            if (merge && W == 8 && g.inDim <= kOlEarlyFloats) vEarly = vEarly > g.inDim * 4u ? vEarly : g.inDim * 4u;
        }
    }
    LdsPlan p;
    uint32_t o = 0;
    p.offM = o; o += align_up(slots, 64) * 4;
    p.offV[0] = o; o += vrows * 4;
    p.offV[1] = FMT == kFp16 ? o : p.offV[0];
    if (FMT == kFp16) o += vrows * 4;
    if (FMT != kFp16 && o < ol) o = align_up(ol, 16);
    p.offA = o; o += (uint32_t)Fmt<FMT>::kSlots * E * 64 * 4;
    p.offL = o; o += align_up(slots * 2, 16);
    const uint32_t tbl = cutoff_table_bytes(64 * W);
    if (o < p.offA + tbl) o = p.offA + tbl;
    p.offC = o; o += 2048;
    p.offO = vEarly ? o : 0u; o += vEarly;
    static_assert(kCutoffLdsBytes <= 1280, "the cutoff scratch must end below the flags of the misc region");
    p.total = o;
    return p;
}
struct ItemRef { uint32_t ci, t, s; };

__device__ __forceinline__ bool locate_item(const GroupKArgs& ga, const uint32_t item, ItemRef& r) {
    uint32_t ci = 0;
    for (uint32_t i = 0; i + 1 < ga.count; i++) if ((item >> 3) >= (uint32_t)ga.wgEnd8[i]) ci = i + 1;
    ci = __builtin_amdgcn_readfirstlane(ci);
    const MulGeom& g = ga.geom[ga.call[ci].geom];
    const uint32_t b = item - (ci ? (uint32_t)ga.wgEnd8[ci - 1] * 8u : 0u), xcd = b & 7u, k = b >> 3;
    r.ci = ci;
    if ((g.slices & 7u) == 0u) {
        r.s = (k / g.tiles) * 8u + ((xcd + ci) & 7u); r.t = k % g.tiles;
        return true;
    }
    const uint32_t per = (uint32_t)ga.wgEnd8[ci] - (ci ? (uint32_t)ga.wgEnd8[ci - 1] : 0u);
    const uint32_t idx = ((xcd + ci) & 7u) * per + k;
    r.s = idx / g.tiles; r.t = idx - r.s * g.tiles;
    return r.s < g.slices;
}

typedef uint32_t u32x4 __attribute__((ext_vector_type(4)));
__device__ __forceinline__ void lds_dma_dword(const u32x4 rsrc, const uint32_t voff, const uint32_t ldsAddr) {
    uint32_t keep;
    asm volatile("s_mov_b32 %0, m0\n\ts_mov_b32 m0, %2\n\ts_nop 0\n\tbuffer_load_dword %1, %3, 0 offen lds\n\ts_mov_b32 m0, %0"
                 : "=&s"(keep) : "v"(voff), "s"(ldsAddr), "s"(rsrc) : "memory");
}
__device__ __forceinline__ u32x4 make_rsrc(const void* base, uint32_t bytes) {
    const uint64_t p = (uint64_t)(size_t)base;
    u32x4 r;
    r[0] = __builtin_amdgcn_readfirstlane((uint32_t)p); r[1] = __builtin_amdgcn_readfirstlane((uint32_t)(p >> 32) & 0xFFFFu);
    r[2] = __builtin_amdgcn_readfirstlane(bytes); r[3] = 0x00020000u;
    return r;
}

template <int FMT, int W, bool COMPACT>
__device__ __forceinline__ void stage_issue(const GroupKArgs& ga, const ItemRef& r, const int tid, char* smem, const LdsPlan& lp, const uint32_t par) {
    constexpr int NT = 64 * W;
    using lds_v = __attribute__((address_space(3))) void;
    const CallDesc& a = ga.call[__builtin_amdgcn_readfirstlane(r.ci)];
    const MulGeom& g = ga.geom[a.geom];
    const uint32_t wave = __builtin_amdgcn_readfirstlane(tid >> 6);
    const uint32_t B = g.sliceRows, j0 = __builtin_amdgcn_readfirstlane(r.s) * B, nb = min(B, g.inDim - j0), lg = g.sliceLog2;
    const uint32_t e = a.expNo ? a.expNo[0] : 0u;
    const uint32_t rowBase = e * g.expertRows;
    const uint32_t rowsPerIn = g.rowsPerIn, inDim = g.inDim, mask = (1u << lg) - 1u;
    const uint32_t nSlots = FMT == kFp16 ? (rowsPerIn << lg) : (nb << 3);
    constexpr bool compact = COMPACT && FMT == kFp16;
    const u32x4 rs = make_rsrc(a.stats, (uint32_t)((size_t)g.numExperts * g.expertRows * (compact ? 2u : 8u)));
    const u32x4 rv = make_rsrc(a.v, inDim * 4u);
    const uint32_t ldsM = __builtin_amdgcn_readfirstlane((uint32_t)(size_t)(lds_v*)(smem + lp.offM));
    const uint32_t ldsV = __builtin_amdgcn_readfirstlane((uint32_t)(size_t)(lds_v*)(smem + ((par & 1u) ? lp.offV[1] : lp.offV[0])));
    if constexpr (compact) {
#pragma unroll
        for (int rr = 0; rr < kRounds / 2; rr++) {
            if (((uint32_t)(rr * NT) + wave * 64u) * 2u >= nSlots) continue;
            const uint32_t c = ((uint32_t)(rr * NT) + (uint32_t)tid) * 2u, rank = c >> lg, jl = c & mask;
            const bool ok = rank < rowsPerIn && jl < nb;
            lds_dma_dword(rs, (rowBase + (ok ? rank * inDim + j0 + jl : j0)) * 2u, ldsM + ((uint32_t)(rr * NT) + wave * 64u) * 4u);
        }
    } else
#pragma unroll
    for (int rr = 0; rr < kRounds; rr++) {
        if ((uint32_t)(rr * NT) + wave * 64u >= nSlots) continue;
        const uint32_t c = rr * NT + tid;
        uint32_t voff;
        if (FMT == kFp16) {
            const uint32_t rank = c >> lg, jl = c & mask;
            const bool ok = rank < rowsPerIn && jl < nb;
            voff = (rowBase + (ok ? rank * inDim + j0 + jl : j0)) * 8u + 4u;
        } else {
            voff = ((rowBase + j0 * 8u + (c < nSlots ? c : 0u)) * 2u + 1u) * 4u;
        }
        lds_dma_dword(rs, voff, ldsM + ((uint32_t)(rr * NT) + wave * 64u) * 4u);
    }
#pragma unroll
    for (int u = 0; u < (FMT == kFp16 ? 1 : 2); u++) {
        if ((uint32_t)(u * NT) + wave * 64u >= nb) continue;
        lds_dma_dword(rv, (j0 + (uint32_t)(u * NT + tid)) * 4u, ldsV + ((uint32_t)(u * NT) + wave * 64u) * 4u);
    }
}

template <int FMT, int E, int W, bool FUSED, bool COMPACT, bool PERSIST, typename Prefetch>
__device__ __forceinline__ void mul_item(const GroupKArgs& ga, const uint32_t item, const ItemRef& ref, char* smem, const LdsPlan& lp, uint32_t& cachedCall,
                                         float& cachedCutoff, const uint32_t par, const bool staged, const bool firstItem, Prefetch prefetch) {
    constexpr int NACC = Fmt<FMT>::kAcc;
    constexpr int TILE_F = NACC * E * 64;
    constexpr int TILE_L = Fmt<FMT>::kSlots * E * 64;
    constexpr int NT = 64 * W;
    constexpr int VPT = 4096 / NT;
    constexpr int KB = batch_rows<E>();

    const uint32_t ci = __builtin_amdgcn_readfirstlane(ref.ci), s = __builtin_amdgcn_readfirstlane(ref.s), t = __builtin_amdgcn_readfirstlane(ref.t);
    const CallDesc& a = ga.call[ci];
    const MulGeom& g = ga.geom[a.geom];
    float* const a_slabs = ga.slabs + (size_t)a.slabOff * 64u;
    uint32_t* const a_counters = ga.counters + a.tileOff;
    uint32_t* const a_sliceCounts = ga.sliceCounts + a.sliceOff;
    float* const a_cutoff = ga.cutoff + ci;
    (void)item;

    int tid0 = threadIdx.x;
    asm volatile("" : "+v"(tid0));
    const int tid = tid0, lane = tid & 63;
#ifdef EFFORT_CUT_FINE
    const bool wstamp = false;
#else
    const bool wstamp = GA_TSTAMP(ga) && tid == 0;
#endif
    unsigned long long ph[6] = {0, 0, 0, 0, 0, 0};
    if (wstamp) ph[0] = wall_clock64();
#ifdef EFFORT_CUT_FINE
    const bool stampCut = GA_TSTAMP(ga) && item == 0 && tid == 0, stamp = false;
#define EFFORT_PSTAMP(i) if (stampCut) GA_TSTAMP(ga)[26 + (i)] = clock64();
#else
#define EFFORT_PSTAMP(i)
    const bool stamp = GA_TSTAMP(ga) && item == 0 && tid == 0;
    const bool stampCut = stamp;
#endif
    if (stamp) GA_TSTAMP(ga)[16] = wall_clock64();
    const int wave = __builtin_amdgcn_readfirstlane(tid >> 6);
    const uint32_t B = g.sliceRows;
    const uint32_t offC = __builtin_amdgcn_readfirstlane(lp.offC), offL = __builtin_amdgcn_readfirstlane(lp.offL), offM = __builtin_amdgcn_readfirstlane(lp.offM);
    const uint32_t offA = __builtin_amdgcn_readfirstlane(lp.offA);
    int* acc = reinterpret_cast<int*>(smem + offA);
    float* vblk = reinterpret_cast<float*>(smem + __builtin_amdgcn_readfirstlane((par & 1u) ? lp.offV[1] : lp.offV[0]));
    uint32_t* flags = reinterpret_cast<uint32_t*>(smem + offC + 1280);
    float* wbound = reinterpret_cast<float*>(smem + offC + 1344);
    uint16_t* list = reinterpret_cast<uint16_t*>(smem + offL);
    const uint32_t* m32 = reinterpret_cast<const uint32_t*>(smem + offM);
    const float* means = reinterpret_cast<const float*>(smem + offM);

    const uint32_t j0 = s * B;
    uint32_t vSlabOff = (s * g.tiles + t) * (uint32_t)(TILE_F * 4), vSlabBytes = (uint32_t)min((size_t)0xFFFFFFFFu, (size_t)g.slices * g.tiles * TILE_F * 4);
    uint32_t vSlices = g.slices, vSliceStride = g.tiles * (uint32_t)(TILE_F * 4);
    if constexpr (!PERSIST) asm volatile("" : "+v"(vSlabOff), "+v"(vSlabBytes), "+v"(vSlices), "+v"(vSliceStride));
    const uint32_t nb = min(B, g.inDim - j0);
    const uint32_t e = a.expNo ? a.expNo[0] : 0u;

    EFFORT_PSTAMP(1)
    if (!staged) stage_issue<FMT, W, COMPACT>(ga, ref, tid, smem, lp, par);
    EFFORT_PSTAMP(2)
    constexpr bool kPreZero = !PERSIST;
    if constexpr (kPreZero) cutoff_table_zero<NT>(reinterpret_cast<uint32_t*>(smem + offA), tid);
    constexpr bool kOlMerge = FMT != kFp16 && W == 8 && (!PERSIST || kProductOnly);
    const uint32_t olPer = ol_outputs_per_item<E>(g);
    bool olAny = false, olEarly = false;
    uint32_t olParts = 1u, olStride = 0u;
    uint32_t olBFirst = 0u, olNB = 0u;
    float olVx[kOlMerge ? 8 : 1]; uint32_t olMeta0 = 0u, olBeg0 = 0u, olEnd0 = 0u;
    auto ol_share = [&]() {
        const uint32_t oBeg = min(t * (uint32_t)TILE_F + s * olPer, g.outDim);
        const uint32_t oEnd = max(oBeg, min(min(t * (uint32_t)TILE_F + (s + 1u) * olPer, (t + 1u) * (uint32_t)TILE_F), g.outDim));
        olBFirst = oBeg >> 6; olNB = ((oEnd + 63u) >> 6) - olBFirst;
        olParts = (olNB && olNB < (uint32_t)W) ? (uint32_t)W / olNB : 1u;
        olStride = olNB * 64u;
    };
    if constexpr (FMT != kFp16) {
        olAny = a.ol.blockPtr != nullptr;
        if (olAny) {
            if constexpr (kOlMerge) {
                ol_share();
                olEarly = g.inDim <= kOlEarlyFloats && lp.offO != 0u;
                if (olEarly) {
                    if constexpr (FUSED) {
                        if (a.pre == (uint16_t)kPreNone) {
#pragma unroll
                            for (int u = 0; u < 8; u++) olVx[u] = a.v[min((uint32_t)(u * NT + tid), g.inDim - 1u)];
                        }
                    } else {
#pragma unroll
                    for (int u = 0; u < 8; u++) olVx[u] = a.v[min((uint32_t)(u * NT + tid), g.inDim - 1u)];
                    }
                    if ((uint32_t)wave < olNB * olParts) {
                        const uint32_t bq = (uint32_t)wave / olParts;
                        olMeta0 = a.ol.meta[(size_t)(olBFirst + bq) * 64u + (uint32_t)lane];
                        olBeg0 = a.ol.blockPtr[olBFirst + bq]; olEnd0 = a.ol.blockPtr[olBFirst + bq + 1u];
                    }
                }
            }
        }
    }
    const float rankBound = a.rankBound[e];
    float vj[VPT]; uint16_t prj[VPT];
    const uint16_t* pr = a.probes + (size_t)e * kProbes;
    const bool fused = (ga.split & 1u) == 0u;
#pragma unroll
    for (int i = 0; i < VPT; i++) { vj[i] = 0.0f; prj[i] = 0; }
    const bool needCut = fused && cachedCall != ci;
    const bool viaJob = needCut && GA_CUTJOBS(ga) != 0u && !firstItem;
    const uint32_t pre = FUSED ? (uint32_t)a.pre : (uint32_t)kPreNone;
    float rawn[VPT]; uint32_t auxc[VPT]; uint32_t auxS = 0u;
    uint32_t auxS1 = 0u;
    const bool preAny = FUSED && pre != (uint32_t)kPreNone;
#pragma unroll
    for (int i = 0; i < VPT; i++) { rawn[i] = 0.0f; auxc[i] = 0u; }
    if (preAny) {
        const bool gate = pre == (uint32_t)kPreSiluGate;
        if (needCut || !gate) {
#pragma unroll
            for (int i = 0; i < VPT; i++) rawn[i] = *(a.v + tid + NT * i);
        }
        if (needCut) {
#pragma unroll
            for (int i = 0; i < VPT; i++) {
                auxc[i] = gate ? __float_as_uint(*(reinterpret_cast<const float*>(a.vAux) + tid + NT * i)) : (uint32_t)reinterpret_cast<const uint16_t*>(a.vAux)[tid + NT * i];
                prj[i] = pr[tid + NT * i];
            }
        }
        const uint32_t js = j0 + min((uint32_t)tid, nb - 1u);
        auxS = gate ? __float_as_uint(*(reinterpret_cast<const float*>(a.vAux) + js)) : (uint32_t)reinterpret_cast<const uint16_t*>(a.vAux)[js];
        if constexpr (FUSED && FMT != kFp16) {
            const uint32_t js1 = j0 + min((uint32_t)(tid + NT), nb - 1u);
            auxS1 = gate ? __float_as_uint(*(reinterpret_cast<const float*>(a.vAux) + js1)) : (uint32_t)reinterpret_cast<const uint16_t*>(a.vAux)[js1];
            if (olEarly && !needCut) {
                if (gate) {
#pragma unroll
                    for (int i = 0; i < VPT; i++) rawn[i] = *(a.v + tid + NT * i);
                }
#pragma unroll
                for (int i = 0; i < VPT; i++)
                    auxc[i] = gate ? __float_as_uint(*(reinterpret_cast<const float*>(a.vAux) + tid + NT * i)) : (uint32_t)reinterpret_cast<const uint16_t*>(a.vAux)[tid + NT * i];
            }
        }
    }
    const uint32_t lg = g.sliceLog2;
    const uint32_t nSlots = FMT == kFp16 ? (g.rowsPerIn << lg) : (nb << 3);
    float normInv = 1.0f;
    if (FUSED && pre == kPreRmsNorm) {
        constexpr int R = 1024 / NT;
        static_assert(R >= 1 && R * NT == 1024 && R * W == 16, "fused rmsNorm: the workgroup must divide add_rmsnorm_mul_kernel's 1024 threads");
        float part[R];
#pragma unroll
        for (int r = 0; r < R; r++) part[r] = 0.0f;
#pragma unroll
        for (int i = 0; i < VPT; i++) part[i % R] += rawn[i] * rawn[i];
        for (uint32_t base = 4096u + (uint32_t)tid; base < g.inDim; base += 1024u) {
#pragma unroll
            for (int r = 0; r < R; r++) {
                const uint32_t j = base + (uint32_t)(r * NT);
                if (j < g.inDim) { const float x = *(a.v + j); part[r] += x * x; }
            }
        }
#pragma unroll
        for (int r = 0; r < R; r++) {
            part[r] = wave_sum_f32(part[r]);
            if (lane == 0) wbound[r * W + wave] = part[r];
        }
        __syncthreads();
        float tot = 0.0f;
#pragma unroll
        for (int w2 = 0; w2 < 16; w2++) tot += wbound[w2];
        normInv = 1.0f / sqrtf(tot / (float)g.inDim + 1e-5f);
        __syncthreads();
    }
    auto xform = [&](float x, uint32_t aux) -> float {
        if (!FUSED) return x;
        if (pre == kPreSiluGate) return __uint_as_float(aux) * x / (1.0f + expf(-x));
        if (pre == kPreRmsNorm) return (x * normInv) * half_bits_to_float((uint16_t)aux);
        return x;
    };
    auto load_cut_inputs = [&]() {
        if (preAny) {
#pragma unroll
            for (int i = 0; i < VPT; i++) vj[i] = xform(rawn[i], auxc[i]);
        } else {
#pragma unroll
            for (int i = 0; i < VPT; i++) { vj[i] = *(a.v + tid + NT * i); prj[i] = pr[tid + NT * i]; }
        }
    };
    if constexpr (kPreZero) {
        asm volatile("s_waitcnt lgkmcnt(0)" ::: "memory");
        __builtin_amdgcn_s_barrier();
    }
    if (needCut && !viaJob) load_cut_inputs();
    EFFORT_PSTAMP(3)
    uint32_t* const cutWords = ga.queue + 9 * 16;
    uint32_t cutWord = 0;
    if (viaJob && tid == 0 && !(GA_ABLATE(ga) & 32u)) cutWord = __hip_atomic_load(&cutWords[ci], __ATOMIC_RELAXED, __HIP_MEMORY_SCOPE_AGENT);
    asm volatile("s_waitcnt vmcnt(0)" ::: "memory");
    EFFORT_PSTAMP(4)
    uint32_t vColOK = 0, voff = 0, vRecords = 0, vBuckLo = 0, vBuckHi = 0, vRowPitch = 0, vInDim = 0, vRow0 = 0;
    auto stream_geom = [&]() {
        const uint32_t col = t * (64u * E) + (uint32_t)lane * E;
        vColOK = col < g.cols ? 1u : 0u;
        voff = (vColOK ? col : (g.cols - 1u) / (uint32_t)E * (uint32_t)E) * 2u;
        vRecords = (uint32_t)min((size_t)0xFFFFFFFFu, (size_t)g.numExperts * g.expertRows * g.rowPitch - (size_t)a.bucketsTrim);
        vBuckLo = (uint32_t)(size_t)a.buckets; vBuckHi = (uint32_t)((size_t)a.buckets >> 32);
        vRowPitch = g.rowPitch; vInDim = g.inDim; vRow0 = e * g.expertRows + (FMT == kFp16 ? j0 : j0 * 8u);
    };
    if constexpr (!PERSIST) {
        stream_geom();
        asm volatile("" : "+v"(vColOK), "+v"(voff), "+v"(vRecords), "+v"(vBuckLo), "+v"(vBuckHi), "+v"(vRowPitch), "+v"(vInDim), "+v"(vRow0));
    }
    if constexpr (kOlMerge) {
        if (olEarly) {
            float* const vf = reinterpret_cast<float*>(smem + __builtin_amdgcn_readfirstlane(lp.offO));
#pragma unroll
            for (int u = 0; u < 8; u++) {
                if constexpr (FUSED) { if ((uint32_t)(u * NT + tid) < g.inDim) vf[u * NT + tid] = preAny ? xform(rawn[u % VPT], auxc[u % VPT]) : olVx[u]; }
                else if ((uint32_t)(u * NT + tid) < g.inDim) vf[u * NT + tid] = olVx[u];
            }
        }
    }
    float bound = 0.0f;
#pragma unroll
    for (int u = 0; u < (FMT == kFp16 ? 1 : 2); u++) {
        const uint32_t jl = tid + u * NT;
        if (jl < nb) {
            float x = vblk[jl];
            if constexpr (FUSED && FMT != kFp16) { if (preAny) { x = xform(x, u ? auxS1 : auxS); vblk[jl] = x; } }
            else
            if (preAny) { x = xform(x, auxS); vblk[jl] = x; }
            bound += fabsf(x);
        }
    }
    bound = wave_sum_f32(bound);
    if (lane == 0) wbound[wave] = bound;
    if (tid == 0) { flags[4] = 0u; flags[5] = (uint32_t)(W * KB); }
    if (stamp) GA_TSTAMP(ga)[17] = wall_clock64();
    if (wstamp) ph[1] = wall_clock64();

    uint32_t* tbl = reinterpret_cast<uint32_t*>(smem + offA);
    float cutoff;
    bool fromJob = false;
    if (viaJob) {
        if (tid == 0) {
            for (int spin = 0; spin < ((GA_ABLATE(ga) & 32u) ? 0 : 20000) && !(cutWord >> 31); spin++) {
                __builtin_amdgcn_s_sleep(8);
                cutWord = __hip_atomic_load(&cutWords[ci], __ATOMIC_RELAXED, __HIP_MEMORY_SCOPE_AGENT);
            }
            flags[2] = cutWord >> 31;
            flags[3] = cutWord & 0x7FFFFFFFu;
        }
        __syncthreads();
        fromJob = flags[2] != 0u;
        if (fromJob) { cutoff = __uint_as_float(flags[3]); cachedCall = ci; cachedCutoff = cutoff; }
        else load_cut_inputs();
    }
    if (fromJob) {
    } else if (needCut) {
        cutoff = block_find_cutoff<NT, kPreZero>(vj, prj, a.q, smem + offC, tbl, []() {}, stampCut ? GA_TSTAMP(ga) + 8 : nullptr);
        cachedCall = ci; cachedCutoff = cutoff;
    } else if (fused) {
        cutoff = cachedCutoff;
        __syncthreads();
    } else {
        cutoff = a_cutoff[0];
        __syncthreads();
    }
    const uint32_t slotCap = __builtin_amdgcn_readfirstlane((lp.offV[0] - lp.offM) / 4u) - 1u;
    const uint16_t* m16 = reinterpret_cast<const uint16_t*>(m32);
    auto load_block = [&](int blk, uint32_t (&mraw)[4], float (&vq)[4]) {
#pragma unroll
        for (int u = 0; u < 4; u++) {
            const uint32_t c = min((uint32_t)((blk * 4 + u) * NT + tid), slotCap);
            if constexpr (COMPACT && FMT == kFp16) { mraw[u] = (uint32_t)m16[c] << 16; vq[u] = 0.0f; }
            else { mraw[u] = m32[c]; vq[u] = FMT != kFp16 ? vblk[min(c >> 3, nb - 1u)] : 0.0f; }
        }
    };
    uint32_t mraw0[4]; float vq0[4];
    load_block(0, mraw0, vq0);
    const uint32_t jlSel = (uint32_t)tid & ((1u << lg) - 1u);
    float axRaw = 0.0f;
    if (FMT == kFp16) axRaw = vblk[min(jlSel, nb - 1u)];
    float wb[W];
#pragma unroll
    for (int w2 = 0; w2 < W; w2++) wb[w2] = wbound[w2];
    __builtin_amdgcn_sched_barrier(0);
    for (int i = tid; i < TILE_L; i += NT) acc[i] = 0;
    float L = 0.0f;
#pragma unroll
    for (int w2 = 0; w2 < W; w2++) L += wb[w2];
    L *= rankBound;
    int kexp = 30 - (int)((__float_as_uint(L) >> 23) & 0xFFu) + 126;
    kexp = L > 0.0f ? max(-100, min(100, kexp)) : 0;
    const float scale = __uint_as_float((uint32_t)(127 + kexp) << 23), unscale = __uint_as_float((uint32_t)(127 - kexp) << 23);
    if (stamp) GA_TSTAMP(ga)[18] = wall_clock64();
    if (wstamp) ph[2] = wall_clock64();

    const float ax = (FMT == kFp16 && jlSel < nb) ? fabsf(axRaw) : 0.0f;
    const bool sel = !(GA_ABLATE(ga) & 8u);
    uint32_t keepMask = 0;
// ... 737 lines not shown
```

### effort_amd/csrc/effort_internal.h

```cpp
#pragma once
#include <hip/hip_runtime.h>
#include <hip/hip_fp16.h>
#include <stdint.h>

#include <map>
#include <mutex>
#include <utility>

namespace effort {

constexpr int kWave = 64;
constexpr int kProbes = 4096;
constexpr float kCutoffScale = 100000.0f;

enum Format : int { kFp16 = 0, kQ4 = 1 };

struct MulGeom {
    uint32_t inDim;
    uint32_t outDim;
    uint32_t cols;
    uint32_t rowsPerIn;
    uint32_t expertRows;
    uint32_t tiles;
    uint32_t slices;
    uint32_t sliceRows;
    uint32_t sliceLog2;
    uint32_t slots;
    uint32_t rowPitch;
    uint32_t numExperts;
    uint32_t elems;
};

struct OutlierIndex {
    const uint32_t* blockPtr;
    const uint32_t* entry;
    const uint32_t* meta;
};

#ifndef EFFORT_MAX_GROUP
#define EFFORT_MAX_GROUP 32
#endif
constexpr int kMaxGroup = EFFORT_MAX_GROUP;
constexpr int kMaxGeoms = 4;
constexpr int kQueueWords = 11 * 16;
constexpr int kTraceOff = 512, kTraceItems = 4096;
enum Prologue : uint16_t { kPreNone = 0, kPreSiluGate = 1, kPreRmsNorm = 2 };
struct CallDesc {
    const uint16_t* buckets;
    const void* stats;
    const float* rankBound;
    const uint16_t* probes;
    const float* v;
    const uint32_t* expNo;
    float* out;
    OutlierIndex ol;
    uint16_t q;
    uint16_t bucketsTrim;
    uint32_t slabOff;
    uint16_t tileOff;
    uint16_t sliceOff;
    uint16_t geom;
    uint16_t pre;
    const void* vAux;
    const float* resid;
};
struct LdsPlan { uint32_t offM, offV[2], offA, offL, offC, offO, total; };
struct GroupKArgs {
    uint32_t count;
    uint32_t totalTiles;
    uint32_t persistent;
    uint32_t numCU;
    uint32_t ablate;
    uint32_t split;
    uint32_t cutJobs;
    uint32_t trace;
    LdsPlan lp;
    uint32_t totalItems;
    uint32_t staggerSleeps;
    uint32_t* groupDone;
    uint32_t* queue;
    float* slabs;
    uint32_t* counters;
    uint32_t* sliceCounts;
    float* cutoff;
    unsigned long long* tstamp;
    uint16_t wgEnd8[kMaxGroup];
    MulGeom geom[kMaxGeoms];
    CallDesc call[kMaxGroup];
};
static_assert(sizeof(CallDesc) == 112 && sizeof(GroupKArgs) <= 4000, "the launch descriptor must fit the kernel-argument segment");

__device__ __forceinline__ float half_bits_to_float(uint16_t h) { return __half2float(__ushort_as_half(h)); }

__device__ __forceinline__ float bf16_round(float f) {
    uint32_t u = __float_as_uint(f);
    if ((u & 0x7FFFFFFFu) > 0x7F800000u) u |= 0x00400000u;
    else u += 0x7FFFu + ((u >> 16) & 1u);
    return __uint_as_float(u & 0xFFFF0000u);
}

typedef __bf16 effort_bf16x2 __attribute__((ext_vector_type(2)));
typedef float effort_f32x2 __attribute__((ext_vector_type(2)));
__device__ __forceinline__ uint32_t bf16_pack2(float x, float y) {
    effort_f32x2 v; v[0] = x; v[1] = y;
    const effort_bf16x2 r = __builtin_convertvector(v, effort_bf16x2);
    uint32_t u; __builtin_memcpy(&u, &r, 4); return u;
}

#define EFFORT_DPP_SCAN(v, OP, IDENT)                                                                 \
    v = OP(v, __builtin_amdgcn_update_dpp(IDENT, v, 0x111, 0xf, 0xf, false));          \
    v = OP(v, __builtin_amdgcn_update_dpp(IDENT, v, 0x112, 0xf, 0xf, false));          \
    v = OP(v, __builtin_amdgcn_update_dpp(IDENT, v, 0x114, 0xf, 0xf, false));          \
    v = OP(v, __builtin_amdgcn_update_dpp(IDENT, v, 0x118, 0xf, 0xf, false));          \
    v = OP(v, __builtin_amdgcn_update_dpp(IDENT, v, 0x142, 0xa, 0xf, false));       \
    v = OP(v, __builtin_amdgcn_update_dpp(IDENT, v, 0x143, 0xc, 0xf, false));
__device__ __forceinline__ int dpp_op_add(int a, int b) { return a + b; }
__device__ __forceinline__ int dpp_op_umin(int a, int b) { return (int)min((uint32_t)a, (uint32_t)b); }
__device__ __forceinline__ int dpp_op_umax(int a, int b) { return (int)max((uint32_t)a, (uint32_t)b); }
__device__ __forceinline__ uint32_t wave_prefix_sum_u32(uint32_t x) { int v = (int)x; EFFORT_DPP_SCAN(v, dpp_op_add, 0) return (uint32_t)v; }
__device__ __forceinline__ uint32_t wave_sum_u32(uint32_t x) { int v = (int)x; EFFORT_DPP_SCAN(v, dpp_op_add, 0) return (uint32_t)__builtin_amdgcn_readlane(v, 63); }
__device__ __forceinline__ uint32_t wave_min_u32(uint32_t x) { int v = (int)x; EFFORT_DPP_SCAN(v, dpp_op_umin, -1) return (uint32_t)__builtin_amdgcn_readlane(v, 63); }
__device__ __forceinline__ uint32_t wave_max_u32(uint32_t x) { int v = (int)x; EFFORT_DPP_SCAN(v, dpp_op_umax, 0) return (uint32_t)__builtin_amdgcn_readlane(v, 63); }
__device__ __forceinline__ float wave_sum_f32(float x) {
    int v = __float_as_int(x);
#define EFFORT_FADD_(a, b) __float_as_int(__int_as_float(a) + __int_as_float(b))
    EFFORT_DPP_SCAN(v, EFFORT_FADD_, 0)
#undef EFFORT_FADD_
    return __int_as_float(__builtin_amdgcn_readlane(v, 63));
}

__device__ __forceinline__ float wave_max_f32(float x) {
    int v = __float_as_int(x);
#define EFFORT_FMAX_(a, b) __float_as_int(fmaxf(__int_as_float(a), __int_as_float(b)))
    EFFORT_DPP_SCAN(v, EFFORT_FMAX_, (int)0xFF800000)
#undef EFFORT_FMAX_
    return __int_as_float(__builtin_amdgcn_readlane(v, 63));
}
__device__ __forceinline__ float row16_sum_f32(float x) {
    int v = __float_as_int(x);
#define EFFORT_FADD_(a, b) __float_as_int(__int_as_float(a) + __int_as_float(b))
    v = EFFORT_FADD_(v, __builtin_amdgcn_update_dpp(0, v, 0x111, 0xf, 0xf, false));
    v = EFFORT_FADD_(v, __builtin_amdgcn_update_dpp(0, v, 0x112, 0xf, 0xf, false));
    v = EFFORT_FADD_(v, __builtin_amdgcn_update_dpp(0, v, 0x114, 0xf, 0xf, false));
    v = EFFORT_FADD_(v, __builtin_amdgcn_update_dpp(0, v, 0x118, 0xf, 0xf, false));
#undef EFFORT_FADD_
    return __int_as_float(v);
}

inline hipError_t allow_full_lds(const void* fn) {
    static std::mutex m;
    static std::map<std::pair<const void*, int>, bool> done;
    int dev = 0;
    hipError_t e = hipGetDevice(&dev);
    if (e != hipSuccess) return e;
    std::lock_guard<std::mutex> lk(m);
    bool& d = done[std::make_pair(fn, dev)];
    if (d) return hipSuccess;
    hipFuncAttributes fa;
    e = hipFuncGetAttributes(&fa, fn);
    if (e == hipSuccess) e = hipFuncSetAttribute(fn, hipFuncAttributeMaxDynamicSharedMemorySize, (int)(160u * 1024u - (uint32_t)fa.sharedSizeBytes));
    if (e == hipSuccess) d = true;
    return e;
}

bool dense_gemv_supported(uint32_t inDim, uint32_t outDim);
hipError_t launch_dense_gemv(const uint16_t* W_f16, const float* v, float* out, uint32_t inDim, uint32_t outDim, hipStream_t st);
hipError_t launch_dense_gemv_expert(const uint16_t* W_f16, const uint32_t* expNo, const float* v, float* out, uint32_t inDim, uint32_t outDim,
                                    uint32_t numExperts, hipStream_t st);
hipError_t launch_find_cutoff(const float* v, const uint16_t* probes, const uint32_t* expNo, uint32_t q,
                              float* cutoff, uint32_t* dispatchCount, unsigned long long* tstamp, hipStream_t st);

struct LaunchedVariant { uint32_t W, E, fused, compact, lean, persistent, grid, totalItems; };
hipError_t launch_bucket_mul(Format fmt, int wavesPerGroup, int elemsPerLane, const GroupKArgs& ga, hipStream_t st, LaunchedVariant* ran = nullptr);
int bucket_mul_variants(Format fmt, int* rows, int maxRows);
hipError_t bucket_mul_prepare_device();
hipError_t launch_find_cutoff_group(const GroupKArgs& ga, hipStream_t st);
size_t bucket_mul_lds_bytes(Format fmt, int wavesPerGroup, int elemsPerLane, const MulGeom& g, bool lean);
uint32_t bucket_mul_max_candidates(int wavesPerGroup);
uint32_t bucket_mul_ol_lds_floats();
int bucket_mul_occupancy(Format fmt, int wavesPerGroup, int elemsPerLane, size_t ldsBytes);

hipError_t launch_calc_dispatch(Format fmt, const void* stats, const float* v, const uint32_t* expNo,
                                const float* cutoff, const MulGeom& g, float* dispatch, uint32_t* count,
                                uint32_t* ctxCount, uint32_t* blockScratch, hipStream_t st);

hipError_t launch_convert_fp16(const uint16_t* W, uint32_t outDim, uint32_t inDim, uint16_t* buckets, uint32_t pitchCols,
                               uint16_t* stats, uint16_t* probes, uint16_t* scratchVals, int* status, hipStream_t st);

hipError_t launch_convert_q4(const uint16_t* core2, uint32_t inDim, uint32_t outDim, uint32_t cnt, uint16_t* buckets, float* stats, uint16_t* probes,
                             float* outliers, int numCU, hipStream_t st);

hipError_t launch_compact_means(const void* stats_f16x4, uint16_t* means, uint32_t rows, hipStream_t st);
hipError_t launch_rank_bound(Format fmt, const uint16_t* buckets, uint32_t pitchCols, const void* stats, uint32_t numExperts, uint32_t rowsPerIn,
                             uint32_t inDim, uint32_t cols, float* rowScratch, float* rankBound, hipStream_t st);
hipError_t launch_add_rmsnorm_mul(float* h, const float* delta, const uint16_t* w, float* out, uint32_t n, hipStream_t st);
hipError_t launch_rope_kv(const float* xq, const float* xk, const float* xv, float* qOut, float* kCache, float* vCache,
                          const uint32_t* pos, uint32_t numHeads, uint32_t numHeadsKV, uint32_t headDim, float ropeBase, uint32_t maxTokens,
                          int* status, hipStream_t st);
hipError_t launch_attention(const float* q, const float* kCache, const float* vCache, const uint32_t* pos, float* out,
                            uint32_t numHeads, uint32_t headDim, uint32_t maxTokens, hipStream_t st);
hipError_t launch_rope_attention(const float* xq, const float* xk, const float* xv, float* kCache, float* vCache, const uint32_t* pos,
                                 float* out, uint32_t numHeads, uint32_t numHeadsKV, uint32_t headDim, uint32_t maxTokens, float ropeBase,
                                 int* status, hipStream_t st);
hipError_t launch_silu_mul(const float* x1, const float* x3, float* out, uint32_t n, hipStream_t st);
hipError_t launch_fetch_row(const uint16_t* emb, const uint32_t* id, float* out, uint32_t n, hipStream_t st);
hipError_t launch_top2_softmax(const float* gate, uint32_t n, uint32_t* idx, float* val, hipStream_t st);
hipError_t launch_mix2(const float* f0, const float* f1, const float* val, float* out, uint32_t n, hipStream_t st);
hipError_t launch_mix2_add(float* h, const float* f0, const float* f1, const float* val, uint32_t n, hipStream_t st);
bool moe_route_supported(uint32_t n, uint32_t numExperts);
hipError_t launch_moe_route(const float* h, const uint16_t* w, const uint16_t* gateW, uint32_t n, uint32_t numExperts, float* gateOut,
                            uint32_t* idx, float* val, hipStream_t st);
hipError_t launch_argmax(const float* logits, uint32_t n, uint32_t* idOut, uint32_t* pos, uint32_t* history, uint32_t historyLen,
                         int* status, hipStream_t st);

hipError_t launch_sample(const float* logits, uint32_t n, const void* params, uint32_t* idOut, uint32_t* pos, uint32_t* history, uint32_t historyLen,
                         int* status, uint32_t* topkIdx, float* topkVal, hipStream_t st);
hipError_t launch_topk(const float* logits, uint32_t n, uint32_t k, uint32_t* idx, float* val, hipStream_t st);

hipError_t launch_f32_to_f16(const float* in, uint16_t* out, uint32_t n, hipStream_t st);
hipError_t launch_cosine(const float* a, const float* b, uint32_t n, float* out3, hipStream_t st);
hipError_t launch_validate_outliers(const float* outliers, uint64_t n, uint32_t inDim, uint32_t outDim, int* bad, hipStream_t st);
hipError_t launch_build_outlier_index(const float* outliers, uint64_t n, uint32_t inDim, uint32_t outDim, uint32_t* rowPtr,
                                      uint32_t* blockPtr, uint32_t* entry, uint32_t* meta, uint32_t* tmp, hipStream_t st);
hipError_t launch_sort_pairs_u32(const uint32_t* keysIn, uint32_t* keysOut, const uint32_t* valsIn, uint32_t* valsOut, uint64_t n, hipStream_t st);

}
```

### effort_amd/csrc/plan.h

```cpp
#pragma once
#include "effort_internal.h"

namespace effort {

constexpr int kMaxLaunches = kMaxGroup / kMaxGeoms + 1;

struct PlanEnv {
    int numCU = 256, nLanes = 1;
    bool laned = false;
    int persistent = -1;
    int tuneW = 0, tuneE = 0, tuneS = 0;
    bool splitCutoff = false, clock = false;
    uint32_t ablate = 0;
    bool noJobs = false, noCompact = false;
    size_t slabBytes = 0;
    uint32_t maxTiles = 0, maxSlices = 0;
    bool thinEffort = false;
    int tailCalls = 0, tailMult = 0;
};
struct PlanCall {
    uint32_t inDim, outDim, cols, rowsPerIn, rowPitch, numExperts;
    bool hasMeans16;
    uint16_t pre;
    bool hasResid;
};
struct CallPlan {
    MulGeom g;
    uint32_t mult;
    uint32_t launch, geom;
    uint32_t slabOff, tileOff, sliceOff;
    uint32_t itemEnd8;
};
struct LaunchPlan {
    uint32_t first, count;
    uint32_t persistent, cutJobs, staggerSleeps;
    bool compact;
    uint32_t totalItems, totalTiles, realItems;
};
struct GroupPlan {
    int W = 0, E = 0;
    int err = 0;
    const char* msg = "";
    uint32_t nLaunches = 0;
    CallPlan call[kMaxGroup];
    LaunchPlan launch[kMaxLaunches];
};

bool supported(int W, int E);
int plan_group(Format fmt, const PlanEnv& env, int n, const PlanCall* calls, GroupPlan* plan);

}
```

### effort_amd/csrc/plan.hip

```cpp
#include <cstring>

#include "../../include/effort_hip.h"
#include "plan.h"

namespace effort {

static uint32_t round8(uint32_t x) { return (x + 7u) / 8u * 8u; }
static uint32_t min_slices(uint32_t inDim) { return round8((inDim + 511u) / 512u); }
static uint32_t max_slices(uint32_t inDim) { return round8((inDim + 127u) / 128u); }
static uint32_t tiles_at(const PlanCall& w, int E) { return (w.cols + 64 * E - 1) / (64 * E); }
static uint32_t group_tiles(int n, const PlanCall* ws, int E) {
    uint32_t t = 0;
    for (int i = 0; i < n; i++) t += tiles_at(ws[i], E);
    return t;
}
static uint32_t padded_items(uint32_t tiles, uint32_t slices) { return round8(tiles * slices); }
static uint32_t padded_min_items(int n, const PlanCall* ws, int E) {
    uint32_t t = 0;
    for (int i = 0; i < n; i++) t += padded_items(tiles_at(ws[i], E), min_slices(ws[i].inDim));
    return t;
}
static bool fits_one_round(const PlanEnv& env, int n, uint32_t tiles, uint32_t allTiles, uint32_t s) {
    const bool same = allTiles == (uint32_t)n * tiles;
    return (same ? (uint32_t)n * padded_items(tiles, s) : allTiles * s + 7u * (uint32_t)n) <= (uint32_t)env.numCU;
}

bool supported(int W, int E) {
    return (W == 16 && (E == 1 || E == 2 || E == 4)) || (W == 8 && (E == 1 || E == 2 || E == 4)) ||
           (W == 4 && (E == 1 || E == 2 || E == 4)) || (W == 2 && E == 4);
}

static uint32_t q4_one_round(const PlanEnv& env, uint32_t inDim, uint32_t groupTiles1) {
    if (env.nLanes > 1 || env.tuneS || !groupTiles1) return 0;
    const uint32_t sMin = (inDim + 831u) / 832u;
    const uint32_t S = (uint32_t)env.numCU * 15u / 8u / groupTiles1;
    return S >= sMin && S >= 2u ? S : 0u;
}
static uint32_t q4_one_per_cu(const PlanEnv& env, uint32_t inDim, uint32_t tiles1, int n, uint32_t groupTiles1) {
    if (env.nLanes > 1 || env.tuneS || n < 3 || n > 9) return 0;
    const uint32_t sMin = (inDim + 831u) / 832u, hi = max_slices(inDim);
    auto fits = [&](uint32_t s) { return fits_one_round(env, n, tiles1, groupTiles1 ? groupTiles1 : (uint32_t)n * tiles1, s); };
    uint32_t S = sMin > 2u ? sMin : 2u;
    if (!fits(S)) return 0;
    const uint32_t top = env.thinEffort ? min_slices(inDim) : hi;
    while (S < top && S < hi && fits(S + 1u)) S++;
    return S;
}
static uint32_t pick_slices(const PlanEnv& env, Format fmt, const PlanCall& w, int groupSize, int E, uint32_t groupTiles = 0, bool fill = true) {
    const uint32_t tiles = tiles_at(w, E);
    const uint32_t lo = min_slices(w.inDim), hi = max_slices(w.inDim);
    if (fmt != kFp16 && (E == 1 || groupSize >= 8) && fill) {
        const uint32_t S = q4_one_per_cu(env, w.inDim, tiles, groupSize, groupTiles);
        if (S) return S;
    }
    if (fmt != kFp16 && E == 1 && groupSize >= 8 && groupTiles) {
        const uint32_t S = q4_one_round(env, w.inDim, groupTiles);
        if (S) return S;
    }
    if (groupSize >= 8 && (fmt != kFp16 || !fill || env.nLanes > 1 || env.thinEffort)) return lo;
    const uint32_t target = (E == 1 && fmt == kFp16) ? (uint32_t)env.numCU : (uint32_t)env.numCU * 3u / 4u;
    const uint32_t allTiles = groupTiles ? groupTiles : (uint32_t)groupSize * tiles;
    uint32_t S = (target / allTiles + 4u) / 8u * 8u;
    if (S < lo) S = lo;
    if (S > hi) S = hi;
    if ((w.inDim & (w.inDim - 1u)) == 0u && (S & (S - 1u)) != 0u) {
        uint32_t up = 8u;
        while (up < S) up <<= 1;
        S = up <= hi ? up : up >> 1;
    }
    if (fmt == kFp16 && fill && groupSize >= 3 && env.nLanes <= 1) {
        auto fits = [&](uint32_t s) { return fits_one_round(env, groupSize, tiles, allTiles, s); };
        if (fits(S)) { if (!env.thinEffort) while (S < hi && fits(S + 1u)) S++; }
        else {
            uint32_t s2 = S;
            while (s2 > lo && !fits(s2)) s2--;
            if (fits(s2)) S = s2;
        }
    }
    return S;
}

static int pick_elems(const PlanEnv& env, Format fmt, int n, const PlanCall* ws) {
    if (env.tuneE) return env.tuneE;
    if (fmt != kFp16) {
        if (n < 8) return 1;
        uint32_t inMax = 0;
        for (int i = 0; i < n; i++) inMax = inMax > ws[i].inDim ? inMax : ws[i].inDim;
        if (n < 10) {
            uint32_t tMax = 0;
            bool same = true;
            for (int i = 0; i < n; i++) {
                const uint32_t t = tiles_at(ws[i], 1);
                same = same && (tMax == 0 || t == tMax); tMax = tMax > t ? tMax : t;
            }
            if (q4_one_per_cu(env, inMax, tMax, n, same ? 0u : group_tiles(n, ws, 1))) return 1;
        }
        if (n >= 10) {
            if (q4_one_round(env, inMax, group_tiles(n, ws, 1))) return 1;
        }
        return 2;
    }
    if (env.tuneS) return 2;
    auto items = [&](int E) {
        uint32_t t = 0;
        const uint32_t gt = group_tiles(n, ws, E);
        for (int i = 0; i < n; i++) t += tiles_at(ws[i], E) * pick_slices(env, fmt, ws[i], n, E, gt, false);
        return t;
    };
    const uint32_t numCU = (uint32_t)env.numCU;
    auto only_wide_tiles_fit = [&] { return padded_min_items(n, ws, 1) > numCU && padded_min_items(n, ws, 2) <= numCU; };
    auto fill = [&](int E) {
        double used = 0, have = 0;
        for (int i = 0; i < n; i++) { used += ws[i].cols; have += (double)tiles_at(ws[i], E) * 64 * E; }
        return have > 0 ? used / have : 1.0;
    };
    const double f1 = fill(1), f2 = fill(2), f4 = fill(4), best = f1 > f2 ? (f1 > f4 ? f1 : f4) : (f2 > f4 ? f2 : f4);
    if (n >= 8) {
        const uint32_t i4 = items(4);
        if (((i4 > numCU / 2 && i4 <= numCU) || i4 >= 3u * numCU) && f4 >= 0.8 * best) return 4;
        if (f2 >= 0.8 * best) return 2;
        if (env.nLanes <= 1 && f2 >= 0.7 * best && only_wide_tiles_fit()) return 2;
        return 1;
    }
    const uint32_t i2 = items(2);
    if (f2 < 0.8 * best) return 1;
    if (n >= 3 && f4 >= 0.8 * best && env.nLanes <= 1) {
        uint32_t lo2 = 0, lo4 = 0;
        for (int i = 0; i < n; i++) {
            const uint32_t lo = min_slices(ws[i].inDim);
            lo2 += tiles_at(ws[i], 2) * lo; lo4 += tiles_at(ws[i], 4) * lo;
        }
        if (lo2 > numCU && lo4 <= numCU * 15u / 16u) return 4;
    }
    bool narrow = true;
    for (int i = 0; i < n; i++) narrow = narrow && ws[i].cols <= 256u;
    if (narrow && f1 >= 0.8 * best && n >= 3 && env.nLanes <= 1 && f2 >= 0.8 * best && only_wide_tiles_fit()) return 2;
    if (narrow && f1 >= 0.8 * best && !(env.nLanes > 1 && n >= 3)) return 1;
    return (i2 * 10u < numCU * 3u / 4u * 6u && items(1) > i2) ? 1 : 2;
}

static uint32_t tile_floats(Format fmt, int E) { return (fmt == kFp16 ? 16u : 32u) * (uint32_t)E * 64u; }
static int choose_geom(const PlanEnv& env, Format fmt, const PlanCall& w, int groupSize, int W, int E, uint32_t groupTiles, uint32_t sliceMult, MulGeom* g) {
    memset(g, 0, sizeof(*g));
    g->inDim = w.inDim; g->outDim = w.outDim; g->cols = w.cols; g->rowsPerIn = w.rowsPerIn;
    g->expertRows = w.rowsPerIn * w.inDim; g->numExperts = w.numExperts;
    g->tiles = tiles_at(w, E);
    g->elems = (uint32_t)E;
    g->rowPitch = w.rowPitch;
    const uint32_t tileFloats = tile_floats(fmt, E);
    const size_t ldsMax = 160 * 1024;
    uint32_t S;
    if (env.tuneS) S = env.tuneS;
    else {
        const uint32_t want = pick_slices(env, fmt, w, groupSize, E, groupTiles) * sliceMult;
        const uint32_t cap = (env.numCU * 2u) / g->tiles / 8 * 8;
        S = cap < want ? cap : want;
    }
    if (S > w.inDim) S = w.inDim / 8 * 8;
    if (S < 1) S = 1;
    const uint32_t maxCand = bucket_mul_max_candidates(W);
    for (;;) {
        g->sliceRows = (w.inDim + S - 1) / S;
        g->slices = (w.inDim + g->sliceRows - 1) / g->sliceRows;
        g->sliceLog2 = 0; while ((1u << g->sliceLog2) < g->sliceRows) g->sliceLog2++;
        g->slots = fmt == kFp16 ? (g->rowsPerIn << g->sliceLog2) : g->sliceRows * 8u;
        const size_t lds = bucket_mul_lds_bytes(fmt, W, E, *g, true);
        const bool fits = lds <= ldsMax && g->slots <= maxCand && (size_t)g->slots * 4 + (size_t)g->sliceRows * 8 + 1024 <= 65536 &&
                          (fmt == kFp16 ? (1u << g->sliceLog2) <= 64u * (uint32_t)W : g->sliceRows <= 128u * (uint32_t)W);
        const size_t slab = (size_t)g->slices * g->tiles * tileFloats * 4;
        if (fits && slab <= env.slabBytes) break;
        if (!fits) { S += 1; if (S > w.inDim + 8) return EFFORT_ERR_SHAPE; }
        else return EFFORT_ERR_SHAPE;
    }
    return EFFORT_OK;
}
static int plan_fail(GroupPlan* P, int code, const char* msg) { P->err = code; P->msg = msg; return code; }

static uint32_t geom_index(MulGeom* geoms, uint32_t& n, const MulGeom& g) {
    uint32_t k = 0;
    while (k < n && memcmp(&geoms[k], &g, sizeof(g)) != 0) k++;
    if (k == n && n < (uint32_t)kMaxGeoms) geoms[n++] = g;
    return k;
}

static void finish_launch(Format fmt, const PlanEnv& env, int W, const PlanCall* ws, const GroupPlan* P, LaunchPlan* lp) {
    const uint32_t R = env.persistent < 0 ? 2u : (uint32_t)env.persistent;
    const uint32_t perCU = (env.persistent < 0 && fmt == kFp16 && !env.laned) ? 6u : R;
    lp->persistent = (R && lp->realItems > (uint32_t)env.numCU * perCU) ? R : 0u;
    bool plain = true;
    for (uint32_t i = 0; i < lp->count; i++) plain = plain && !ws[lp->first + i].pre;
    lp->cutJobs = (lp->persistent && !env.splitCutoff && plain && !env.noJobs) ? (lp->count + 7u) / 8u * 8u : 0u;
    const bool leanGrid = lp->persistent == 0u && W == 8 && !env.clock && !env.ablate;
    bool compact = fmt == kFp16 && !env.noCompact && (leanGrid || (lp->persistent != 0u && plain));
    for (uint32_t i = 0; compact && !leanGrid && i < lp->count; i++) compact = !ws[lp->first + i].hasResid;
    for (uint32_t i = 0; compact && i < lp->count; i++) {
        const MulGeom& g = P->call[lp->first + i].g;
        compact = ws[lp->first + i].hasMeans16 && g.inDim % 2u == 0u && g.sliceRows % 2u == 0u;
    }
    lp->compact = compact;
    lp->staggerSleeps = (lp->persistent && fmt == kQ4 && !env.laned) ? 11u : 0u;
}

int plan_group(Format fmt, const PlanEnv& env, int n, const PlanCall* ws, GroupPlan* P) {
    P->err = EFFORT_OK; P->msg = ""; P->nLaunches = 0;
    const bool laned = env.laned;
    const int W = env.tuneW ? env.tuneW : 8;
    const int E = pick_elems(env, fmt, n, ws);
    P->W = W; P->E = E;
    const char* const noGeometry = "bucketmul: no launch geometry for this shape/tuning";
    if (!supported(W, E)) return plan_fail(P, EFFORT_ERR_ARG, noGeometry);
    const uint32_t groupTiles = group_tiles(n, ws, E);
    MulGeom g1[kMaxGroup], g2[kMaxGroup];
    uint32_t it1[kMaxGroup], base = 0;
    for (int i = 0; i < n; i++) {
        const int rc = choose_geom(env, fmt, ws[i], n, W, E, groupTiles, 1, &g1[i]);
        if (rc != EFFORT_OK) return plan_fail(P, rc, noGeometry);
        it1[i] = padded_items(g1[i].tiles, g1[i].slices);
        base += it1[i];
    }
    int thinFrom = n;
    if (E == 2 && n >= 8 && !laned && !env.tuneS && env.persistent < 0 && !env.thinEffort) {
        const uint32_t round = 2u * (uint32_t)env.numCU, over = base % round;
        if (base > round && over != 0u && over * 32u <= round * 7u && (fmt != kFp16 || base <= 6u * (uint32_t)env.numCU)) {
            int tc = 0;
            uint32_t thin = 0;
            while (tc < n && tc < 4 && (tc < 2 || thin < over)) thin += it1[n - 1 - tc++];
            MulGeom seen[kMaxGeoms];
            uint32_t nSeen = 0, extra = 0;
            bool ok = thin >= over;
            for (int i = 0; ok && i < n; i++) {
                const bool t = i >= n - tc;
                if (t) {
                    ok = choose_geom(env, fmt, ws[i], n, W, E, groupTiles, 2, &g2[i]) == EFFORT_OK;
                    const uint32_t it2 = padded_items(g2[i].tiles, g2[i].slices);
                    ok = ok && it2 > it1[i];
                    extra += it2 - it1[i];
                }
                ok = ok && geom_index(seen, nSeen, t ? g2[i] : g1[i]) < (uint32_t)kMaxGeoms;
            }
            if (ok && (fmt != kFp16 || base + extra <= 6u * (uint32_t)env.numCU)) thinFrom = n - tc;
        }
    }
    uint32_t nGeoms = 0, wg = 0;
    MulGeom geoms[kMaxGeoms];
    size_t slabOff = 0; uint32_t tileOff = 0, sliceOff = 0;
    LaunchPlan* lp = nullptr;
    auto begin = [&](uint32_t firstCall) {
        lp = &P->launch[P->nLaunches++];
        memset(lp, 0, sizeof(*lp));
        lp->first = firstCall;
        nGeoms = 0; wg = 0;
    };
    begin(0);
    for (int i = 0; i < n; i++) {
        uint32_t mult = i >= thinFrom ? 2u : 1u;
        MulGeom g = mult == 2u ? g2[i] : g1[i];
        if (n >= 8 && !env.tuneS && env.tailMult) {
            mult = 1;
            if (i >= n - env.tailCalls) mult = (uint32_t)env.tailMult;
            if (env.tailMult >= 4 && i >= n - env.tailCalls && i < n - env.tailCalls / 2) mult = (uint32_t)env.tailMult / 2;
            const int rc = choose_geom(env, fmt, ws[i], n, W, E, groupTiles, mult, &g);
            if (rc != EFFORT_OK) return plan_fail(P, rc, noGeometry);
        }
        uint32_t gi = geom_index(geoms, nGeoms, g);
        if (gi == (uint32_t)kMaxGeoms) {
            finish_launch(fmt, env, W, ws, P, lp);
            begin((uint32_t)i);
            gi = geom_index(geoms, nGeoms, g);
        }
        CallPlan& a = P->call[i];
        const size_t slab = (size_t)g.slices * g.tiles * tile_floats(fmt, E) * 4;
        if (tileOff + g.tiles + 1 > env.maxTiles || sliceOff + g.slices > env.maxSlices || slabOff + slab > env.slabBytes)
            return plan_fail(P, EFFORT_ERR_SHAPE, "bucketmul: group exceeds the context scratch");
        a.g = g; a.mult = mult; a.launch = P->nLaunches - 1u; a.geom = gi;
        a.slabOff = (uint32_t)(slabOff / 256); a.tileOff = tileOff; a.sliceOff = sliceOff;
        wg += padded_items(g.tiles, g.slices);
        if (wg / 8u > 0xFFFFu) return plan_fail(P, EFFORT_ERR_SHAPE, "bucketmul: group exceeds the launch descriptor's item range");
        a.itemEnd8 = wg / 8u;
        lp->count = (uint32_t)i - lp->first + 1u;
        lp->totalItems = wg; lp->totalTiles += g.tiles; lp->realItems += g.tiles * g.slices;
        slabOff += (slab + 255) / 256 * 256; tileOff += g.tiles; sliceOff += g.slices;
    }
    finish_launch(fmt, env, W, ws, P, lp);
    return EFFORT_OK;
}

}
```

### effort_amd/runtime.py

```python
from __future__ import annotations

import ctypes as C

import torch

from . import _lib


class Gpu:
    def __init__(self, device: int | None = None):
        if not torch.cuda.is_available():
            raise RuntimeError("effort_amd needs an AMD GPU (torch.cuda.is_available() is False); there is no CPU fallback")
        self.device = torch.cuda.current_device() if device is None else int(device)
        self._lib = _lib.lib()
        with torch.cuda.device(self.device):
            stream = torch.cuda.current_stream(self.device).cuda_stream
            self.ctx = self._lib.effort_create(self.device, C.c_void_p(stream))
        self.has_comm = False
        self.dense_rocblas = False
        if not self.ctx:
            raise RuntimeError("effort_create failed: " + (self._lib.effort_last_error(None) or b"").decode())
        self._stream = stream

    def _bind_stream(self):
        cur = torch.cuda.current_stream(self.device)
        stream = cur.cuda_stream
        if stream != self._stream:
            old = getattr(self, "_stream_obj", None)
            if old is not None and not torch.cuda.is_current_stream_capturing():
                try:
                    cur.wait_stream(old)
                except RuntimeError:
                    pass
            self._lib.effort_set_stream(self.ctx, C.c_void_p(stream))
            self._stream = stream
        self._stream_obj = cur

    def check(self, rc: int, where: str):
        if rc != 0:
            detail = self._lib.effort_last_error(self.ctx)
            raise _lib.EffortError(rc, where, detail.decode() if detail else "")

    def eval(self):
        self.check(self._lib.effort_sync(self.ctx), "gpu.eval")

    def set_overlap(self, lanes: int = 4):
        self._bind_stream()
        self.check(self._lib.effort_set_overlap(self.ctx, int(lanes)), "set_overlap")

    def join(self):
        self.check(self._lib.effort_join(self.ctx), "join")

    def set_row_reuse(self, reuse: bool = True):
        self.check(self._lib.effort_set_row_reuse(self.ctx, int(bool(reuse))), "set_row_reuse")

    @staticmethod
    def comm_unique_id() -> bytes:
        buf = (C.c_char * 128)()
        rc = _lib.lib().effort_comm_unique_id(buf)
        if rc != 0:
            raise _lib.EffortError(rc, "comm_unique_id")
        return bytes(buf)

    def comm_create(self, rank: int, world: int, uid: bytes):
        if len(uid) != 128:
            raise ValueError("the communicator id is 128 bytes")
        self._bind_stream()
        self.check(self._lib.effort_comm_create(self.ctx, int(rank), int(world), C.c_char_p(uid)), "comm_create")
        self.has_comm = True

    def comm_destroy(self):
        self.check(self._lib.effort_comm_destroy(self.ctx), "comm_destroy")
        self.has_comm = False

    @property
    def comm_world(self) -> int:
        return int(self._lib.effort_comm_world(self.ctx))

    @property
    def comm_rank(self) -> int:
        return int(self._lib.effort_comm_rank(self.ctx))

    def allgather_outputs(self, send: torch.Tensor, recv: torch.Tensor, count: int | None = None):
        n = int(send.numel() if count is None else count)
        if not (send.is_cuda and recv.is_cuda and send.dtype == torch.float32 and recv.dtype == torch.float32 and send.is_contiguous()
                and recv.is_contiguous() and send.numel() >= n and recv.numel() >= n * self.comm_world):
            raise ValueError("allgather_outputs: contiguous f32 CUDA tensors, recv holding world * count elements")
        self._bind_stream()
        self.check(self._lib.effort_allgather_outputs(self.ctx, C.c_void_p(send.data_ptr()), C.c_void_p(recv.data_ptr()), n), "allgather_outputs")

    def hook_lane(self, lane: int):
        self.check(self._lib.effort_debug_hook_lane(self.ctx, int(lane)), "hook_lane")

    def set_tuning(self, waves: int = 0, elems: int = 0, slices: int = 0):
        self.check(self._lib.effort_set_tuning(self.ctx, waves, elems, slices), "set_tuning")

    def set_split_cutoff(self, split: bool = True):
        self.check(self._lib.effort_set_split_cutoff(self.ctx, int(split)), "set_split_cutoff")

    def enable_kernel_timing(self, mode: int = 1):
        self._bind_stream()
        self.check(self._lib.effort_enable_kernel_timing(self.ctx, int(mode)), "enable_kernel_timing")

    def kernel_clock(self):
        us, n = C.c_double(), C.c_int()
        self.check(self._lib.effort_kernel_clock(self.ctx, C.byref(us), C.byref(n)), "kernel_clock")
        return {"mul_us": us.value, "launches": n.value}

    def set_persistent(self, wg_per_cu: int = -1):
        self.check(self._lib.effort_set_persistent(self.ctx, int(wg_per_cu)), "set_persistent")

    def set_dense_backend(self, rocblas: bool = False):
        self.check(self._lib.effort_set_dense_backend(self.ctx, int(bool(rocblas))), "set_dense_backend")
        self.dense_rocblas = bool(rocblas)

    def convert_status(self) -> int:
        n = C.c_int(0)
        self.check(self._lib.effort_convert_status(self.ctx, C.byref(n)), "convert_status")
        return int(n.value)

    def debug_stamps(self):
        buf = (C.c_ulonglong * 32)()
        self.check(self._lib.effort_debug_stamps(self.ctx, buf), "debug_stamps")
        return list(buf)

    def slice_counts(self, idx: int = 0, n: int = 4096):
        buf = (C.c_uint32 * n)()
        k = self._lib.effort_debug_slice_counts(self.ctx, int(idx), buf, n)
        if k < 0:
            self.check(k, "slice_counts")
        return list(buf[:k])

    def debug_trace(self, n: int = 4096):
        buf = (C.c_ulonglong * (12 * n))()
        self.check(self._lib.effort_debug_trace(self.ctx, buf, n), "debug_trace")
        return [tuple(buf[8 * i:8 * i + 8]) + tuple(buf[8 * n + 4 * i:8 * n + 4 * i + 4]) for i in range(n)]

    def kernel_timing(self):
        mul, cut, integ, n = C.c_double(), C.c_double(), C.c_double(), C.c_int()
        self.check(self._lib.effort_kernel_timing(self.ctx, C.byref(mul), C.byref(cut), C.byref(integ), C.byref(n)), "kernel_timing")
        return {"mul_us": mul.value, "cutoff_us": cut.value, "integrate_us": integ.value, "samples": n.value}

    def last_dispatch_count(self, idx: int = 0) -> int:
        n = C.c_uint32()
        self.check(self._lib.effort_group_dispatch_count(self.ctx, int(idx), C.byref(n)), "last_dispatch_count")
        return int(n.value)

    def last_cutoff(self, idx: int = 0) -> float:
        x = C.c_float()
        self.check(self._lib.effort_group_cutoff(self.ctx, int(idx), C.byref(x)), "last_cutoff")
        return float(x.value)

    def last_variant(self, launch: int = 0) -> dict:
        buf = (C.c_int * 8)()
        self.check(self._lib.effort_debug_last_variant(self.ctx, int(launch), buf), "last_variant")
        return {"variant": (buf[0], buf[1], bool(buf[2]), bool(buf[3]), bool(buf[4])), "persistent": buf[5], "grid": buf[6], "totalItems": buf[7]}

    def close(self):
        if getattr(self, "ctx", None):
            self._lib.effort_destroy(self.ctx)
            self.ctx = None

    def __del__(self):
        try:
            self.close()
        except Exception:
            pass


def plan(calls, *, q4: bool = False, numCU: int = 256, lanes: int = 1, persistent: int = -1, waves: int = 0, elems: int = 0, slices: int = 0) -> dict:
    n = len(calls)
    rows = [tuple(c) + (16, 0, 0)[len(c) - 3:] for c in calls]
    ints = lambda k: (C.c_int * n)(*[int(r[k]) for r in rows])
    out = [(C.c_int * max(n, 2))() for _ in range(9)]
    k = _lib.lib().effort_debug_plan(int(q4), numCU, lanes, n, ints(0), ints(1), ints(3), ints(4), ints(5), (C.c_double * n)(*[float(r[2]) for r in rows]),
                                     persistent, waves, elems, slices, *out)
    if k < 0:
        raise _lib.EffortError(k, "plan")
    we, per_call, per_launch = out[0], out[1:5], out[5:]
    res = {"W": we[0], "E": we[1]}
    res.update({name: list(a[:n]) for name, a in zip(("slices", "tiles", "sliceRows", "launch"), per_call)})
    res.update({name: list(a[:k]) for name, a in zip(("persistent", "cutJobs", "compact", "stagger"), per_launch)})
    return res


def variants(q4: bool = False) -> list[tuple]:
    n = _lib.lib().effort_debug_variants(int(q4), None, 0)
    if n < 0:
        raise _lib.EffortError(n, "variants")
    buf = (C.c_int * (5 * n))()
    k = _lib.lib().effort_debug_variants(int(q4), buf, n)
    if k != n:
        raise _lib.EffortError(min(k, -1), "variants")
    return [(buf[5 * i], buf[5 * i + 1], bool(buf[5 * i + 2]), bool(buf[5 * i + 3]), bool(buf[5 * i + 4])) for i in range(n)]


def lanes(ops, *, lanes: int = 4) -> list[dict]:
    kinds = {"launch": 0, "timed": 1, "join": 2}
    words = []
    for op in ops:
        kind, cap, busy, rd, wr = tuple(op) + (0, (), ())[len(op) - 2:]
        words += [kinds[kind], int(cap), int(bool(busy)), len(rd), len(wr)]
        for lo, hi in list(rd) + list(wr):
            words += [int(lo), int(hi)]
    n, W = len(ops), 18
    out = (C.c_int64 * max(n * W, 1))()
    k = _lib.lib().effort_debug_lanes(lanes, n, (C.c_int64 * max(len(words), 1))(*words), len(words), out)
    if k < 0:
        raise _lib.EffortError(k, "lanes")
    members = lambda mask: tuple(i for i in range(lanes) if mask >> i & 1)
    res = []
    for i in range(n):
        r = out[i * W:(i + 1) * W]
        res.append({"rc": r[0], "joined_first": bool(r[1]), "joined": members(r[2]), "lane": r[3], "fork_waited": bool(r[4]), "waits": members(r[5]),
                    "pending": members(r[6]), "nextLane": r[7], "busyStreak": r[8], "migrated": bool(r[9]),
                    "reads": list(r[10:10 + lanes]), "writes": list(r[14:14 + lanes])})
    return res


_gpus: dict[int, Gpu] = {}


def gpu(device: int | None = None) -> Gpu:
    if not torch.cuda.is_available():
        raise RuntimeError("effort_amd needs an AMD GPU (torch.cuda.is_available() is False); there is no CPU fallback")
    d = torch.cuda.current_device() if device is None else int(device)
    g = _gpus.get(d)
    if g is None:
        g = _gpus[d] = Gpu(d)
    return g
```

### include/effort_hip_debug.h

```cpp
#ifndef EFFORT_HIP_DEBUG_H
#define EFFORT_HIP_DEBUG_H

#include "effort_hip.h"

#ifdef __cplusplus
extern "C" {
#endif

EFFORT_API int effort_set_tuning(effort_ctx* ctx, int wavesPerGroup, int elemsPerLane, int rowSlices);
EFFORT_API int effort_set_split_cutoff(effort_ctx* ctx, int split);

EFFORT_API int effort_set_persistent(effort_ctx* ctx, int wgPerCU);

EFFORT_API int effort_debug_hook_lane(effort_ctx* ctx, int lane);

EFFORT_API int effort_is_lab_build(void);
EFFORT_API int effort_enable_kernel_timing(effort_ctx* ctx, int enable);
EFFORT_API int effort_kernel_clock(effort_ctx* ctx, double* mul_us_avg, int* n_launches);
EFFORT_API int effort_kernel_timing(effort_ctx* ctx, double* mul_us_avg, double* cutoff_us_avg,
                         double* integrate_us_avg, int* n_samples);
EFFORT_API int effort_debug_occupancy(effort_ctx* ctx, int q4, int waves, int elems, int ldsBytes);
EFFORT_API int effort_debug_stamps(effort_ctx* ctx, unsigned long long* host32);
EFFORT_API int effort_debug_slice_counts(effort_ctx* ctx, int idx, uint32_t* host, int maxSlices);
EFFORT_API int effort_debug_plan(int q4, int numCU, int lanes, int n, const int* inDim, const int* outDim, const int* percentLoad,
                      const int* prologue, const int* hasResid, const double* effort, int persistent, int tuneW, int tuneE, int tuneS,
                      int* we, int* slices, int* tiles, int* sliceRows, int* launchOf,
                      int* launchPersistent, int* launchCutJobs, int* launchCompact, int* launchStagger);
EFFORT_API int effort_debug_check_bundle(int q4, int inDim, int outDim, int percentLoad, int numExperts, int rowPitchBytes);
EFFORT_API int effort_debug_variants(int q4, int* rows, int maxRows);
EFFORT_API int effort_debug_last_variant(effort_ctx* ctx, int launch, int* out8);
#define EFFORT_LANES_LAUNCH 0
#define EFFORT_LANES_TIMED 1
#define EFFORT_LANES_JOIN 2
#define EFFORT_LANES_OUT_WORDS 18
EFFORT_API int effort_debug_lanes(int lanes, int nOps, const int64_t* ops, int64_t nWords, int64_t* out);
EFFORT_API int effort_debug_trace(effort_ctx* ctx, unsigned long long* host, int maxRecords);

#ifdef __cplusplus
}
#endif
#endif
```

Measured before the change: 21460.

## Add specialized persistent bucket_rows kernel running two workgroups per CU

Adds a dedicated persistent kernel for fp16 W=8/E=4 compact launches with 2-3 tiles. Its LDS budget is capped so two workgroups fit per CU, and it shares the staging helpers moved into a new header. A planner heuristic turns it on only for multi-lane runs with at least four lanes, no tuning overrides, and enough slices to cover every CU. The aim is better latency hiding through higher occupancy, at the cost of a second kernel path to maintain and a narrow set of eligible shapes.

```diff
diff --git a/effort_amd/_lib.py b/effort_amd/_lib.py
--- a/effort_amd/_lib.py
+++ b/effort_amd/_lib.py
@@ -101,7 +101,10 @@
     "effort_debug_stamps": (C.c_int, [_P, C.POINTER(C.c_ulonglong)]),
     "effort_debug_slice_counts": (C.c_int, [_P, C.c_int, C.POINTER(C.c_uint32), C.c_int]),
     "effort_debug_plan": (C.c_int, [C.c_int, C.c_int, C.c_int, C.c_int, _P, _P, _P, _P, _P, _P, C.c_int, C.c_int, C.c_int, C.c_int, _P, _P, _P, _P, _P, _P, _P, _P, _P]),
-    "effort_debug_check_bundle": (C.c_int, [C.c_int, C.c_int, C.c_int, C.c_int, C.c_int, C.c_int]),
+    "effort_set_row_items": (C.c_int, [_P, C.c_int]),
+    "effort_debug_plan_row_items": (C.c_int, [C.c_int, C.c_int, C.c_int, C.c_int, _P, _P, _P, _P, _P, _P, C.c_int, C.c_int, C.c_int, C.c_int, C.c_int, _P]),
+    "effort_debug_row_items": (C.c_int, [_P, C.c_int]),
+    "effort_debug_check_bundle":(C.c_int, [C.c_int, C.c_int, C.c_int, C.c_int, C.c_int, C.c_int]),
     "effort_debug_variants": (C.c_int, [C.c_int, _P, C.c_int]),
     "effort_debug_last_variant": (C.c_int, [_P, C.c_int, _P]),
     "effort_debug_lanes": (C.c_int, [C.c_int, C.c_int, _P, C.c_int64, _P]),
@@ -124,7 +127,7 @@
         import torch
         l = C.CDLL(LIB_PATH)
         for name, (res, args) in _SIGS.items():
-            if (name.startswith("effort_debug_") or name == "effort_is_lab_build") and os.environ.get("EFFORT_HIP_LIB") and not hasattr(l, name):
+            if (name.startswith("effort_debug_") or name in ("effort_is_lab_build", "effort_set_row_items")) and os.environ.get("EFFORT_HIP_LIB") and not hasattr(l, name):
                 continue
             fn = getattr(l, name)
             fn.restype = res
diff --git a/effort_amd/csrc/api.hip b/effort_amd/csrc/api.hip
--- a/effort_amd/csrc/api.hip
+++ b/effort_amd/csrc/api.hip
@@ -33,6 +33,7 @@
     uint32_t lastCalls = 1, lastSliceOff[effort::kMaxGroup] = {0}, lastSlices[effort::kMaxGroup] = {0};
     uint32_t lastLaunches = 0;
     effort::LaunchedVariant lastVariant[effort::kMaxLaunches] = {};
+    bool lastRows[effort::kMaxLaunches] = {};
 };
 
 struct effort_ctx {
@@ -64,6 +65,8 @@
     int tuneW = 0, tuneE = 0, tuneS = 0;
     bool splitCutoff = false;
     bool rowReuse = false;
+    int rowItems = -1;
+    bool rowsTwoPerCU = false;
     bool timing = false;
     bool clock = false;
     bool trace = false;
@@ -191,13 +194,16 @@
     if (hipGetDeviceProperties(&prop, device) == hipSuccess) c->numCU = prop.multiProcessorCount;
     c->slabBytes = effort_ctx::kSlabBytes;
     {
-        static std::mutex m; static std::map<int, bool> prepared;
+        static std::mutex m; static std::map<int, bool> prepared, rowsTwoPerCU;
         std::lock_guard<std::mutex> lk(m);
         if (!prepared[device]) {
-            const hipError_t pe = bucket_mul_prepare_device();
+            bool two = false;
+            hipError_t pe = bucket_mul_prepare_device();
+            if (pe == hipSuccess) pe = bucket_rows_prepare_device(&two);
             if (pe != hipSuccess) { snprintf(g_createErr, sizeof(g_createErr), "effort_create: kernel attributes: %s", hipGetErrorString(pe)); delete c; return nullptr; }
-            prepared[device] = true;
+            prepared[device] = true; rowsTwoPerCU[device] = two;
         }
+        c->rowsTwoPerCU = rowsTwoPerCU[device];
     }
     bool ok = lane_alloc(c, c->lane[0]) && hipMalloc(&c->d_blockScratch, 4096 * 4) == hipSuccess &&
               hipMalloc(&c->d_cos, 16) == hipSuccess && hipMalloc(&c->d_status, 16) == hipSuccess &&
@@ -689,7 +695,10 @@
         }
         { const int frc = fork_lane(c, lc); if (frc != EFFORT_OK) return frc; }
         if (c->splitCutoff && !(env.ablate & 1u)) HIP_TRY(c, launch_find_cutoff_group(ga, st));
-        HIP_TRY(c, launch_bucket_mul(fmt, plan.W, plan.E, ga, st, &L.lastVariant[l]));
+        const bool rows = c->rowsTwoPerCU && row_items(fmt, env, plan, l, c->rowItems);
+        if (rows) HIP_TRY(c, launch_bucket_rows(ga, st, &L.lastVariant[l]));
+        else HIP_TRY(c, launch_bucket_mul(fmt, plan.W, plan.E, ga, st, &L.lastVariant[l]));
+        L.lastRows[l] = rows;
         L.lastLaunches = l + 1u;
     }
     L.lastCalls = (uint32_t)n;
@@ -767,12 +776,9 @@
     HIP_TRY(c, hipStreamSynchronize(c->stream));
     return (int)n;
 }
-extern "C" int effort_debug_plan(int q4, int numCU, int lanes, int n, const int* inDim, const int* outDim, const int* percentLoad,
-                                 const int* prologue, const int* hasResid, const double* effort, int persistent, int tuneW, int tuneE, int tuneS,
-                                 int* we, int* slices, int* tiles, int* sliceRows, int* launchOf,
-                                 int* launchPersistent, int* launchCutJobs, int* launchCompact, int* launchStagger) {
-    if (numCU < 1 || lanes < 1 || lanes > effort_ctx::kMaxLanes || n < 1 || n > kMaxGroup || !inDim || !outDim || !effort || !we || !slices || !tiles ||
-        !sliceRows || !launchOf || !launchPersistent || !launchCutJobs || !launchCompact || !launchStagger) return EFFORT_ERR_ARG;
+static int debug_plan_group(int q4, int numCU, int lanes, int n, const int* inDim, const int* outDim, const int* percentLoad, const int* prologue, const int* hasResid,
+                            const double* effort, int persistent, int tuneW, int tuneE, int tuneS, PlanEnv* env, GroupPlan* plan) {
+    if (numCU < 1 || lanes < 1 || lanes > effort_ctx::kMaxLanes || n < 1 || n > kMaxGroup || !inDim || !outDim || !effort) return EFFORT_ERR_ARG;
     const Format fmt = q4 ? kQ4 : kFp16;
     effort_ctx c0;
     c0.numCU = numCU; c0.book.nLanes = lanes; c0.persistent = persistent; c0.tuneW = tuneW; c0.tuneE = tuneE; c0.tuneS = tuneS;
@@ -785,8 +791,17 @@
         const uint32_t cols = (uint32_t)outDim[i] / (q4 ? 32u : 16u);
         pc[i] = PlanCall{(uint32_t)inDim[i], (uint32_t)outDim[i], cols, (uint32_t)load, cols * 2u, 1u, !q4, (uint16_t)(prologue ? prologue[i] : 0), hasResid && hasResid[i]};
     }
+    *env = plan_env(&c0, lanes > 1, thin_effort(n, effort));
+    return plan_group(fmt, *env, n, pc, plan);
+}
+extern "C" int effort_debug_plan(int q4, int numCU, int lanes, int n, const int* inDim, const int* outDim, const int* percentLoad,
+                                 const int* prologue, const int* hasResid, const double* effort, int persistent, int tuneW, int tuneE, int tuneS,
+                                 int* we, int* slices, int* tiles, int* sliceRows, int* launchOf,
+                                 int* launchPersistent, int* launchCutJobs, int* launchCompact, int* launchStagger) {
+    if (!we || !slices || !tiles || !sliceRows || !launchOf || !launchPersistent || !launchCutJobs || !launchCompact || !launchStagger) return EFFORT_ERR_ARG;
+    PlanEnv env;
     GroupPlan plan;
-    const int rc = plan_group(fmt, plan_env(&c0, lanes > 1, thin_effort(n, effort)), n, pc, &plan);
+    const int rc = debug_plan_group(q4, numCU, lanes, n, inDim, outDim, percentLoad, prologue, hasResid, effort, persistent, tuneW, tuneE, tuneS, &env, &plan);
     if (rc != EFFORT_OK) return rc;
     we[0] = plan.W; we[1] = plan.E;
     for (int i = 0; i < n; i++) {
@@ -797,6 +812,17 @@
         const LaunchPlan& lp = plan.launch[l];
         launchPersistent[l] = (int)lp.persistent; launchCutJobs[l] = (int)lp.cutJobs; launchCompact[l] = lp.compact ? 1 : 0; launchStagger[l] = (int)lp.staggerSleeps;
     }
+    return (int)plan.nLaunches;
+}
+extern "C" int effort_debug_plan_row_items(int q4, int numCU, int lanes, int n, const int* inDim, const int* outDim, const int* percentLoad,
+                                           const int* prologue, const int* hasResid, const double* effort, int persistent, int tuneW, int tuneE, int tuneS,
+                                           int mode, int* rows) {
+    if (!rows || mode < -1 || mode > 1) return EFFORT_ERR_ARG;
+    PlanEnv env;
+    GroupPlan plan;
+    const int rc = debug_plan_group(q4, numCU, lanes, n, inDim, outDim, percentLoad, prologue, hasResid, effort, persistent, tuneW, tuneE, tuneS, &env, &plan);
+    if (rc != EFFORT_OK) return rc;
+    for (uint32_t l = 0; l < plan.nLaunches; l++) rows[l] = row_items(q4 ? kQ4 : kFp16, env, plan, l, mode) ? 1 : 0;
     return (int)plan.nLaunches;
 }
 extern "C" int effort_debug_variants(int q4, int* rows, int maxRows) {
@@ -810,6 +836,17 @@
     const LaunchedVariant& v = L.lastVariant[launch];
     const uint32_t w[8] = {v.W, v.E, v.fused, v.compact, v.lean, v.persistent, v.grid, v.totalItems};
     for (int i = 0; i < 8; i++) out8[i] = (int)w[i];
+    return EFFORT_OK;
+}
+extern "C" int effort_debug_row_items(effort_ctx* c, int launch) {
+    if (!c || launch < 0) return EFFORT_ERR_ARG;
+    const Lane& L = c->lane[c->lastLane];
+    if ((uint32_t)launch >= L.lastLaunches) return EFFORT_ERR_ARG;
+    return L.lastRows[launch] ? 1 : 0;
+}
+extern "C" int effort_set_row_items(effort_ctx* c, int mode) {
+    if (!c || mode < -1 || mode > 1) return EFFORT_ERR_ARG;
+    c->rowItems = mode;
     return EFFORT_OK;
 }
 extern "C" int effort_group_cutoff(effort_ctx* c, int idx, float* host_out) {
diff --git a/effort_amd/csrc/bucket_device.h b/effort_amd/csrc/bucket_device.h
--- /dev/null
+++ b/effort_amd/csrc/bucket_device.h
@@ -0,0 +1,100 @@
+#pragma once
+#include "cutoff_device.h"
+
+namespace effort {
+
+constexpr int kRounds = 16;
+constexpr int kSc1 = 16;
+
+#ifndef EFFORT_ROW_AUX
+#define EFFORT_ROW_AUX 2
+#endif
+constexpr int kRowAux = EFFORT_ROW_AUX;
+
+template <int E> struct Piece;
+template <> struct Piece<1> {
+    uint32_t w;
+    template <int AUX> __device__ __forceinline__ void load(__amdgpu_buffer_rsrc_t r, uint32_t voff, uint32_t soff) { w = __builtin_amdgcn_raw_buffer_load_b16(r, voff, soff, AUX); }
+    __device__ __forceinline__ uint32_t word(int) const { return w & 0xFFFFu; }
+    __device__ __forceinline__ uint32_t dword(int) const { return w; }
+};
+template <> struct Piece<2> {
+    uint32_t w;
+    template <int AUX> __device__ __forceinline__ void load(__amdgpu_buffer_rsrc_t r, uint32_t voff, uint32_t soff) { w = __builtin_amdgcn_raw_buffer_load_b32(r, voff, soff, AUX); }
+    __device__ __forceinline__ uint32_t word(int j) const { return (w >> (16 * j)) & 0xFFFFu; }
+    __device__ __forceinline__ uint32_t dword(int) const { return w; }
+};
+template <> struct Piece<4> {
+    uint32_t w[2];
+    template <int AUX> __device__ __forceinline__ void load(__amdgpu_buffer_rsrc_t r, uint32_t voff, uint32_t soff) {
+        auto t = __builtin_amdgcn_raw_buffer_load_b64(r, voff, soff, AUX); w[0] = t[0]; w[1] = t[1];
+    }
+    __device__ __forceinline__ uint32_t word(int j) const { return (w[j >> 1] >> (16 * (j & 1))) & 0xFFFFu; }
+    __device__ __forceinline__ uint32_t dword(int j) const { return w[j >> 1]; }
+};
+__host__ __device__ inline uint32_t align_up(uint32_t x, uint32_t a) { return (x + a - 1) / a * a; }
+
+struct ItemRef { uint32_t ci, t, s; };
+
+typedef uint32_t u32x4 __attribute__((ext_vector_type(4)));
+__device__ __forceinline__ void lds_dma_dword(const u32x4 rsrc, const uint32_t voff, const uint32_t ldsAddr) {
+    uint32_t keep;
+    asm volatile("s_mov_b32 %0, m0\n\ts_mov_b32 m0, %2\n\ts_nop 0\n\tbuffer_load_dword %1, %3, 0 offen lds\n\ts_mov_b32 m0, %0"
+                 : "=&s"(keep) : "v"(voff), "s"(ldsAddr), "s"(rsrc) : "memory");
+}
+__device__ __forceinline__ u32x4 make_rsrc(const void* base, uint32_t bytes) {
+    const uint64_t p = (uint64_t)(size_t)base;
+    u32x4 r;
+    r[0] = __builtin_amdgcn_readfirstlane((uint32_t)p); r[1] = __builtin_amdgcn_readfirstlane((uint32_t)(p >> 32) & 0xFFFFu);
+    r[2] = __builtin_amdgcn_readfirstlane(bytes); r[3] = 0x00020000u;
+    return r;
+}
+
+template <int FMT, int W, bool COMPACT>
+__device__ __forceinline__ void stage_issue(const GroupKArgs& ga, const ItemRef& r, const int tid, char* smem, const LdsPlan& lp, const uint32_t par) {
+    constexpr int NT = 64 * W;
+    using lds_v = __attribute__((address_space(3))) void;
+    const CallDesc& a = ga.call[__builtin_amdgcn_readfirstlane(r.ci)];
+    const MulGeom& g = ga.geom[a.geom];
+    const uint32_t wave = __builtin_amdgcn_readfirstlane(tid >> 6);
+    const uint32_t B = g.sliceRows, j0 = __builtin_amdgcn_readfirstlane(r.s) * B, nb = min(B, g.inDim - j0), lg = g.sliceLog2;
+    const uint32_t e = a.expNo ? a.expNo[0] : 0u;
+    const uint32_t rowBase = e * g.expertRows;
+    const uint32_t rowsPerIn = g.rowsPerIn, inDim = g.inDim, mask = (1u << lg) - 1u;
+    const uint32_t nSlots = FMT == kFp16 ? (rowsPerIn << lg) : (nb << 3);
+    constexpr bool compact = COMPACT && FMT == kFp16;
+    const u32x4 rs = make_rsrc(a.stats, (uint32_t)((size_t)g.numExperts * g.expertRows * (compact ? 2u : 8u)));
+    const u32x4 rv = make_rsrc(a.v, inDim * 4u);
+    const uint32_t ldsM = __builtin_amdgcn_readfirstlane((uint32_t)(size_t)(lds_v*)(smem + lp.offM));
+    const uint32_t ldsV = __builtin_amdgcn_readfirstlane((uint32_t)(size_t)(lds_v*)(smem + ((par & 1u) ? lp.offV[1] : lp.offV[0])));
+    if constexpr (compact) {
+#pragma unroll
+        for (int rr = 0; rr < kRounds / 2; rr++) {
+            if (((uint32_t)(rr * NT) + wave * 64u) * 2u >= nSlots) continue;
+            const uint32_t c = ((uint32_t)(rr * NT) + (uint32_t)tid) * 2u, rank = c >> lg, jl = c & mask;
+            const bool ok = rank < rowsPerIn && jl < nb;
+            lds_dma_dword(rs, (rowBase + (ok ? rank * inDim + j0 + jl : j0)) * 2u, ldsM + ((uint32_t)(rr * NT) + wave * 64u) * 4u);
+        }
+    } else
+#pragma unroll
+    for (int rr = 0; rr < kRounds; rr++) {
+        if ((uint32_t)(rr * NT) + wave * 64u >= nSlots) continue;
+        const uint32_t c = rr * NT + tid;
+        uint32_t voff;
+        if (FMT == kFp16) {
+            const uint32_t rank = c >> lg, jl = c & mask;
+            const bool ok = rank < rowsPerIn && jl < nb;
+            voff = (rowBase + (ok ? rank * inDim + j0 + jl : j0)) * 8u + 4u;
+        } else {
+            voff = ((rowBase + j0 * 8u + (c < nSlots ? c : 0u)) * 2u + 1u) * 4u;
+        }
+        lds_dma_dword(rs, voff, ldsM + ((uint32_t)(rr * NT) + wave * 64u) * 4u);
+    }
+#pragma unroll
+    for (int u = 0; u < (FMT == kFp16 ? 1 : 2); u++) {
+        if ((uint32_t)(u * NT) + wave * 64u >= nb) continue;
+        lds_dma_dword(rv, (j0 + (uint32_t)(u * NT + tid)) * 4u, ldsV + ((uint32_t)(u * NT) + wave * 64u) * 4u);
+    }
+}
+
+}
diff --git a/effort_amd/csrc/bucket_mul.hip b/effort_amd/csrc/bucket_mul.hip
--- a/effort_amd/csrc/bucket_mul.hip
+++ b/effort_amd/csrc/bucket_mul.hip
@@ -1,13 +1,12 @@
 #include <cstring>
 #include <type_traits>
 
-#include "cutoff_device.h"
+#include "bucket_device.h"
 
 namespace effort {
 
 constexpr int kBatch = 16;
 template <int E> __host__ __device__ constexpr int batch_rows() { return E >= 4 ? 8 : kBatch; }
-constexpr int kRounds = 16;
 
 #ifndef EFFORT_ABLATE_NOSCATTER
 #define EFFORT_ABLATE_NOSCATTER 0
@@ -18,10 +17,6 @@
 
 constexpr int kMinWavesPerEU = 4;
 
-#ifndef EFFORT_ROW_AUX
-#define EFFORT_ROW_AUX 2
-#endif
-constexpr int kRowAux = EFFORT_ROW_AUX;
 #define GA_PERSISTENT(ga) (PERSIST ? (ga).persistent : 0u)
 #define GA_CUTJOBS(ga) (PERSIST ? (ga).cutJobs : 0u)
 #ifndef EFFORT_LAB
@@ -54,7 +49,6 @@
 constexpr bool kLeanStamps = false;
 #endif
 constexpr uint32_t kMaxLdsBytes = 160u * 1024u - 1024u;
-constexpr int kSc1 = 16;
 
 template <int FMT> struct Fmt;
 template <> struct Fmt<kFp16> { static constexpr int kAcc = 16, kSlots = 16; };
@@ -64,28 +58,6 @@
 template <> struct MeanT<kFp16> { typedef uint16_t type; };
 template <> struct MeanT<kQ4> { typedef float type; };
 
-template <int E> struct Piece;
-template <> struct Piece<1> {
-    uint32_t w;
-    template <int AUX> __device__ __forceinline__ void load(__amdgpu_buffer_rsrc_t r, uint32_t voff, uint32_t soff) { w = __builtin_amdgcn_raw_buffer_load_b16(r, voff, soff, AUX); }
-    __device__ __forceinline__ uint32_t word(int) const { return w & 0xFFFFu; }
-    __device__ __forceinline__ uint32_t dword(int) const { return w; }
-};
-template <> struct Piece<2> {
-    uint32_t w;
-    template <int AUX> __device__ __forceinline__ void load(__amdgpu_buffer_rsrc_t r, uint32_t voff, uint32_t soff) { w = __builtin_amdgcn_raw_buffer_load_b32(r, voff, soff, AUX); }
-    __device__ __forceinline__ uint32_t word(int j) const { return (w >> (16 * j)) & 0xFFFFu; }
-    __device__ __forceinline__ uint32_t dword(int) const { return w; }
-};
-template <> struct Piece<4> {
-    uint32_t w[2];
-    template <int AUX> __device__ __forceinline__ void load(__amdgpu_buffer_rsrc_t r, uint32_t voff, uint32_t soff) {
-        auto t = __builtin_amdgcn_raw_buffer_load_b64(r, voff, soff, AUX); w[0] = t[0]; w[1] = t[1];
-    }
-    __device__ __forceinline__ uint32_t word(int j) const { return (w[j >> 1] >> (16 * (j & 1))) & 0xFFFFu; }
-    __device__ __forceinline__ uint32_t dword(int j) const { return w[j >> 1]; }
-};
-__host__ __device__ inline uint32_t align_up(uint32_t x, uint32_t a) { return (x + a - 1) / a * a; }
 
 constexpr int kOlBatch = 16;
 constexpr uint32_t kOlLdsFloats = 16384;
@@ -129,7 +101,6 @@
     p.total = o;
     return p;
 }
-struct ItemRef { uint32_t ci, t, s; };
 
 __device__ __forceinline__ bool locate_item(const GroupKArgs& ga, const uint32_t item, ItemRef& r) {
     uint32_t ci = 0;
@@ -146,67 +117,6 @@
     const uint32_t idx = ((xcd + ci) & 7u) * per + k;
     r.s = idx / g.tiles; r.t = idx - r.s * g.tiles;
     return r.s < g.slices;
-}
-
-typedef uint32_t u32x4 __attribute__((ext_vector_type(4)));
-__device__ __forceinline__ void lds_dma_dword(const u32x4 rsrc, const uint32_t voff, const uint32_t ldsAddr) {
-    uint32_t keep;
-    asm volatile("s_mov_b32 %0, m0\n\ts_mov_b32 m0, %2\n\ts_nop 0\n\tbuffer_load_dword %1, %3, 0 offen lds\n\ts_mov_b32 m0, %0"
-                 : "=&s"(keep) : "v"(voff), "s"(ldsAddr), "s"(rsrc) : "memory");
-}
-__device__ __forceinline__ u32x4 make_rsrc(const void* base, uint32_t bytes) {
-    const uint64_t p = (uint64_t)(size_t)base;
-    u32x4 r;
-    r[0] = __builtin_amdgcn_readfirstlane((uint32_t)p); r[1] = __builtin_amdgcn_readfirstlane((uint32_t)(p >> 32) & 0xFFFFu);
-    r[2] = __builtin_amdgcn_readfirstlane(bytes); r[3] = 0x00020000u;
-    return r;
-}
-
-template <int FMT, int W, bool COMPACT>
-__device__ __forceinline__ void stage_issue(const GroupKArgs& ga, const ItemRef& r, const int tid, char* smem, const LdsPlan& lp, const uint32_t par) {
-    constexpr int NT = 64 * W;
-    using lds_v = __attribute__((address_space(3))) void;
-    const CallDesc& a = ga.call[__builtin_amdgcn_readfirstlane(r.ci)];
-    const MulGeom& g = ga.geom[a.geom];
-    const uint32_t wave = __builtin_amdgcn_readfirstlane(tid >> 6);
-    const uint32_t B = g.sliceRows, j0 = __builtin_amdgcn_readfirstlane(r.s) * B, nb = min(B, g.inDim - j0), lg = g.sliceLog2;
-    const uint32_t e = a.expNo ? a.expNo[0] : 0u;
-    const uint32_t rowBase = e * g.expertRows;
-    const uint32_t rowsPerIn = g.rowsPerIn, inDim = g.inDim, mask = (1u << lg) - 1u;
-    const uint32_t nSlots = FMT == kFp16 ? (rowsPerIn << lg) : (nb << 3);
-    constexpr bool compact = COMPACT && FMT == kFp16;
-    const u32x4 rs = make_rsrc(a.stats, (uint32_t)((size_t)g.numExperts * g.expertRows * (compact ? 2u : 8u)));
-    const u32x4 rv = make_rsrc(a.v, inDim * 4u);
-    const uint32_t ldsM = __builtin_amdgcn_readfirstlane((uint32_t)(size_t)(lds_v*)(smem + lp.offM));
-    const uint32_t ldsV = __builtin_amdgcn_readfirstlane((uint32_t)(size_t)(lds_v*)(smem + ((par & 1u) ? lp.offV[1] : lp.offV[0])));
-    if constexpr (compact) {
-#pragma unroll
-        for (int rr = 0; rr < kRounds / 2; rr++) {
-            if (((uint32_t)(rr * NT) + wave * 64u) * 2u >= nSlots) continue;
-            const uint32_t c = ((uint32_t)(rr * NT) + (uint32_t)tid) * 2u, rank = c >> lg, jl = c & mask;
-            const bool ok = rank < rowsPerIn && jl < nb;
-            lds_dma_dword(rs, (rowBase + (ok ? rank * inDim + j0 + jl : j0)) * 2u, ldsM + ((uint32_t)(rr * NT) + wave * 64u) * 4u);
-        }
-    } else
-#pragma unroll
-    for (int rr = 0; rr < kRounds; rr++) {
-        if ((uint32_t)(rr * NT) + wave * 64u >= nSlots) continue;
-        const uint32_t c = rr * NT + tid;
-        uint32_t voff;
-        if (FMT == kFp16) {
-            const uint32_t rank = c >> lg, jl = c & mask;
-            const bool ok = rank < rowsPerIn && jl < nb;
-            voff = (rowBase + (ok ? rank * inDim + j0 + jl : j0)) * 8u + 4u;
-        } else {
-            voff = ((rowBase + j0 * 8u + (c < nSlots ? c : 0u)) * 2u + 1u) * 4u;
-        }
-        lds_dma_dword(rs, voff, ldsM + ((uint32_t)(rr * NT) + wave * 64u) * 4u);
-    }
-#pragma unroll
-    for (int u = 0; u < (FMT == kFp16 ? 1 : 2); u++) {
-        if ((uint32_t)(u * NT) + wave * 64u >= nb) continue;
-        lds_dma_dword(rv, (j0 + (uint32_t)(u * NT + tid)) * 4u, ldsV + ((uint32_t)(u * NT) + wave * 64u) * 4u);
-    }
 }
 
 template <int FMT, int E, int W, bool FUSED, bool COMPACT, bool PERSIST, typename Prefetch>
diff --git a/effort_amd/csrc/bucket_rows.hip b/effort_amd/csrc/bucket_rows.hip
--- /dev/null
+++ b/effort_amd/csrc/bucket_rows.hip
@@ -0,0 +1,426 @@
+#include <cstring>
+#include <type_traits>
+
+#include "bucket_device.h"
+
+namespace effort {
+
+constexpr int kRowsW = 8, kRowsE = 4, kRowsNT = 64 * kRowsW;
+constexpr int kRowsTiles = 3;
+constexpr int kRowsKB = 4;
+constexpr int kRowsTileF = 16 * kRowsE * 64;
+static_assert(cutoff_table_bytes(kRowsNT) <= (uint32_t)kRowsTiles * kRowsTileF * 4u, "the cutoff's count table borrows the accumulator region");
+
+static LdsPlan rows_plan_lds(const MulGeom* geoms, int nGeoms) {
+    uint32_t slots = 0, vrows = 0;
+    for (int i = 0; i < nGeoms; i++) {
+        const MulGeom& g = geoms[i];
+        if (!g.slices) continue;
+        slots = slots > g.slots ? slots : g.slots;
+        const uint32_t vr = align_up(g.sliceRows, 64);
+        vrows = vrows > vr ? vrows : vr;
+    }
+    LdsPlan p;
+    p.offM = 0; p.offL = 0;
+    p.offV[0] = p.offV[1] = align_up(slots * 2u, 256);
+    p.offA = p.offV[0] + vrows * 4u;
+    p.offC = p.offA + (uint32_t)kRowsTiles * kRowsTileF * 4u;
+    p.offO = 0;
+    p.total = p.offC + 2048u;
+    return p;
+}
+
+__device__ __forceinline__ bool rows_locate(const GroupKArgs& ga, const uint32_t item, ItemRef& r) {
+    uint32_t ci = 0;
+    for (uint32_t i = 0; i + 1 < ga.count; i++) if ((item >> 3) >= (uint32_t)ga.wgEnd8[i]) ci = i + 1;
+    ci = __builtin_amdgcn_readfirstlane(ci);
+    const MulGeom& g = ga.geom[ga.call[ci].geom];
+    const uint32_t first8 = ci ? (uint32_t)ga.wgEnd8[ci - 1] : 0u;
+    const uint32_t b = item - first8 * 8u, xcd = b & 7u, k = b >> 3;
+    r.ci = ci; r.t = 0;
+    if ((g.slices & 7u) == 0u) r.s = k * 8u + ((xcd + ci) & 7u);
+    else r.s = ((xcd + ci) & 7u) * ((uint32_t)ga.wgEnd8[ci] - first8) + k;
+    return r.s < g.slices;
+}
+
+__device__ __forceinline__ void rows_cutoff_job(const GroupKArgs& ga, const uint32_t ci, char* smem, const LdsPlan& lp) {
+    constexpr int VPT = 4096 / kRowsNT;
+    const CallDesc& a = ga.call[ci];
+    int tid0 = threadIdx.x;
+    asm volatile("" : "+v"(tid0));
+    const int tid = tid0;
+    const uint32_t e = a.expNo ? a.expNo[0] : 0u;
+    const uint16_t* pr = a.probes + (size_t)e * kProbes;
+    float vj[VPT]; uint16_t prj[VPT];
+#pragma unroll
+    for (int i = 0; i < VPT; i++) { vj[i] = a.v[tid + kRowsNT * i]; prj[i] = pr[tid + kRowsNT * i]; }
+    const float cutoff = block_find_cutoff<kRowsNT>(vj, prj, a.q, smem + lp.offC, reinterpret_cast<uint32_t*>(smem + lp.offA), []() {}, nullptr);
+    if (tid == 0) {
+        __hip_atomic_store(&ga.queue[9 * 16 + ci], __float_as_uint(cutoff) | 0x80000000u, __ATOMIC_RELAXED, __HIP_MEMORY_SCOPE_AGENT);
+        __hip_atomic_store(reinterpret_cast<uint32_t*>(ga.cutoff + ci), __float_as_uint(cutoff), __ATOMIC_RELAXED, __HIP_MEMORY_SCOPE_AGENT);
+    }
+    __syncthreads();
+}
+
+__device__ __forceinline__ void rows_item(const GroupKArgs& ga, const ItemRef& ref, char* smem, const LdsPlan& lp, uint32_t& cachedCall, float& cachedCutoff) {
+    constexpr int NT = kRowsNT, W = kRowsW, E = kRowsE, KB = kRowsKB, TILE_F = kRowsTileF, VPT = 4096 / NT;
+    const uint32_t ci = __builtin_amdgcn_readfirstlane(ref.ci), s = __builtin_amdgcn_readfirstlane(ref.s);
+    const CallDesc& a = ga.call[ci];
+    const MulGeom& g = ga.geom[a.geom];
+    float* const a_slabs = ga.slabs + (size_t)a.slabOff * 64u;
+    uint32_t* const a_counters = ga.counters + a.tileOff;
+    uint32_t* const a_sliceCounts = ga.sliceCounts + a.sliceOff;
+
+    int tid0 = threadIdx.x;
+    asm volatile("" : "+v"(tid0));
+    const int tid = tid0, lane = tid & 63;
+    const int wave = __builtin_amdgcn_readfirstlane(tid >> 6);
+    const uint32_t B = g.sliceRows, lg = g.sliceLog2, tiles = g.tiles;
+    const uint32_t offC = __builtin_amdgcn_readfirstlane(lp.offC), offA = __builtin_amdgcn_readfirstlane(lp.offA);
+    int* acc = reinterpret_cast<int*>(smem + offA);
+    float* vblk = reinterpret_cast<float*>(smem + __builtin_amdgcn_readfirstlane(lp.offV[0]));
+    uint32_t* flags = reinterpret_cast<uint32_t*>(smem + offC + 1280);
+    float* wbound = reinterpret_cast<float*>(smem + offC + 1344);
+    uint16_t* list = reinterpret_cast<uint16_t*>(smem + __builtin_amdgcn_readfirstlane(lp.offL));
+    const uint16_t* m16 = reinterpret_cast<const uint16_t*>(smem + __builtin_amdgcn_readfirstlane(lp.offM));
+    const uint32_t j0 = s * B, nb = min(B, g.inDim - j0);
+    const uint32_t e = a.expNo ? a.expNo[0] : 0u;
+    const uint32_t nSlots = g.rowsPerIn << lg;
+
+    stage_issue<kFp16, W, true>(ga, ref, tid, smem, lp, 0u);
+    const float rankBound = a.rankBound[e];
+    const bool needCut = cachedCall != ci;
+    uint32_t* const cutWords = ga.queue + 9 * 16;
+    uint32_t cutWord = 0;
+    if (needCut && tid == 0) cutWord = __hip_atomic_load(&cutWords[ci], __ATOMIC_RELAXED, __HIP_MEMORY_SCOPE_AGENT);
+    asm volatile("s_waitcnt vmcnt(0)" ::: "memory");
+    float bound = 0.0f;
+    if ((uint32_t)tid < nb) bound = fabsf(vblk[tid]);
+    bound = wave_sum_f32(bound);
+    if (lane == 0) wbound[wave] = bound;
+    if (tid == 0) { flags[4] = 0u; flags[5] = (uint32_t)(W * KB); }
+
+    float cutoff;
+    if (needCut) {
+        if (tid == 0) {
+            for (int spin = 0; spin < 20000 && !(cutWord >> 31); spin++) {
+                __builtin_amdgcn_s_sleep(8);
+                cutWord = __hip_atomic_load(&cutWords[ci], __ATOMIC_RELAXED, __HIP_MEMORY_SCOPE_AGENT);
+            }
+            flags[2] = cutWord >> 31;
+            flags[3] = cutWord & 0x7FFFFFFFu;
+        }
+        __syncthreads();
+        if (flags[2] != 0u) cutoff = __uint_as_float(flags[3]);
+        else {
+            const uint16_t* pr = a.probes + (size_t)e * kProbes;
+            float vj[VPT]; uint16_t prj[VPT];
+#pragma unroll
+            for (int i = 0; i < VPT; i++) { vj[i] = *(a.v + tid + NT * i); prj[i] = pr[tid + NT * i]; }
+            cutoff = block_find_cutoff<NT>(vj, prj, a.q, smem + offC, reinterpret_cast<uint32_t*>(smem + offA), []() {}, nullptr);
+        }
+        cachedCall = ci; cachedCutoff = cutoff;
+    } else {
+        cutoff = cachedCutoff;
+        __syncthreads();
+    }
+    const uint32_t jlSel = (uint32_t)tid & ((1u << lg) - 1u);
+    const float axRaw = vblk[min(jlSel, nb - 1u)];
+    float wb[W];
+#pragma unroll
+    for (int w2 = 0; w2 < W; w2++) wb[w2] = wbound[w2];
+    for (int i = tid; i < kRowsTiles * TILE_F; i += NT) acc[i] = 0;
+    float L = 0.0f;
+#pragma unroll
+    for (int w2 = 0; w2 < W; w2++) L += wb[w2];
+    L *= rankBound;
+    int kexp = 30 - (int)((__float_as_uint(L) >> 23) & 0xFFu) + 126;
+    kexp = L > 0.0f ? max(-100, min(100, kexp)) : 0;
+    const float scale = __uint_as_float((uint32_t)(127 + kexp) << 23), unscale = __uint_as_float((uint32_t)(127 - kexp) << 23);
+
+    const float ax = jlSel < nb ? fabsf(axRaw) : 0.0f;
+    uint32_t keepMask = 0;
+    uint32_t before[kRounds];
+    uint32_t wtot = 0;
+#pragma unroll
+    for (int blk = 0; blk < kRounds / 4; blk++) {
+        if (blk > 0 && (uint32_t)(blk * 4 * NT) >= nSlots) {
+#pragma unroll
+            for (int u = 0; u < 4; u++) before[blk * 4 + u] = wtot;
+            continue;
+        }
+        uint32_t mraw[4];
+#pragma unroll
+        for (int u = 0; u < 4; u++) mraw[u] = m16[min((uint32_t)((blk * 4 + u) * NT + tid), nSlots - 1u)];
+#pragma unroll
+        for (int u = 0; u < 4; u++) {
+            const int rr = blk * 4 + u;
+            before[rr] = wtot;
+            const uint32_t c = rr * NT + tid;
+            const bool k = (cutoff < (kCutoffScale * half_bits_to_float((uint16_t)mraw[u])) * ax) & ((c >> lg) < g.rowsPerIn);
+            keepMask |= k ? (1u << rr) : 0u;
+            wtot += (uint32_t)__popcll(__ballot(k));
+        }
+    }
+    __syncthreads();
+    uint32_t wbase = 0;
+    if (lane == 0) wbase = atomicAdd(&flags[4], wtot);
+    wbase = __builtin_amdgcn_readfirstlane(wbase);
+#pragma unroll
+    for (int rr = 0; rr < kRounds; rr++) {
+        if ((uint32_t)(rr * NT) >= nSlots) break;
+        const uint32_t c = rr * NT + tid;
+        const bool k = (keepMask >> rr) & 1u;
+        const unsigned long long m = __ballot(k);
+        const uint32_t pos = wbase + before[rr] + __builtin_amdgcn_mbcnt_hi((uint32_t)(m >> 32), __builtin_amdgcn_mbcnt_lo((uint32_t)m, 0u));
+        if (k) list[pos] = (uint16_t)(((c >> lg) << 12) | (c & ((1u << lg) - 1u)));
+    }
+    __syncthreads();
+    const uint32_t n = flags[4];
+    if (tid == 0) a_sliceCounts[s] = n;
+
+    uint32_t voff[kRowsTiles], okMask = 0;
+#pragma unroll
+    for (int t = 0; t < kRowsTiles; t++) {
+        const uint32_t col = (uint32_t)t * (64u * E) + (uint32_t)lane * E;
+        const bool ok = col < g.cols;
+        okMask |= ok ? (1u << t) : 0u;
+        voff[t] = (ok ? col : (g.cols - 1u) / (uint32_t)E * (uint32_t)E) * 2u;
+    }
+    const uint32_t records = (uint32_t)min((size_t)0xFFFFFFFFu, (size_t)g.numExperts * g.expertRows * g.rowPitch - (size_t)a.bucketsTrim);
+    const __amdgpu_buffer_rsrc_t rsrc = __builtin_amdgcn_make_buffer_rsrc(const_cast<uint16_t*>(a.buckets), 0, (int)__builtin_amdgcn_readfirstlane(records), 0x00020000);
+    const uint32_t rowPitch = g.rowPitch, inDim = g.inDim, row0 = e * g.expertRows + j0;
+    const uint32_t nU = __builtin_amdgcn_readfirstlane(n);
+    uint32_t* const cursor = flags + 5;
+    auto grab = [&]() -> uint32_t {
+        uint32_t bq = 0;
+        if (lane == 0) bq = atomicAdd(cursor, (uint32_t)KB);
+        return __builtin_amdgcn_readfirstlane(bq);
+    };
+    auto decode = [&](uint32_t i0, uint32_t& boff, float& dv) {
+        boff = 0; dv = 0.0f;
+        if (lane < KB && nU) {
+            const uint32_t code = list[min(i0 + (uint32_t)lane, nU - 1u)];
+            const uint32_t rank = code >> 12, jl = code & 4095u;
+            dv = vblk[jl] * scale;
+            boff = (row0 + rank * inDim + jl) * rowPitch;
+        }
+    };
+    typedef Piece<E> RowPieces[KB][kRowsTiles];
+    auto issue = [&](auto aux, RowPieces& piece, uint32_t boff) {
+#pragma unroll
+        for (int u = 0; u < KB; u++) {
+            const uint32_t so = __builtin_amdgcn_readlane(boff, u);
+#pragma unroll
+            for (int t = 0; t < kRowsTiles; t++) piece[u][t].template load<decltype(aux)::value>(rsrc, voff[t], so);
+        }
+    };
+    using lds_i = __attribute__((address_space(3))) int;
+    const uint32_t accB = (uint32_t)(size_t)(lds_i*)(acc + lane);
+    auto row = [&](const Piece<E>& pc, float dd, int t) {
+#pragma unroll
+        for (int j = 0; j < E; j++) {
+            const uint32_t dw = pc.dword(j);
+            uint32_t a2; int qv;
+            asm("v_bfe_u32 %0, %1, %2, 4\n\tv_lshl_add_u32 %0, %0, %3, %4" : "=&v"(a2) : "v"(dw), "n"(16 * (j & 1)), "n"(10), "v"(accB));
+            if (j & 1) asm("v_fma_mix_f32 %0, %1, %2, 0 op_sel:[0,1,0] op_sel_hi:[0,1,0]\n\tv_cvt_rpi_i32_f32 %0, %0" : "=v"(qv) : "v"(dd), "v"(dw));
+            else asm("v_fma_mix_f32 %0, %1, %2, 0 op_sel_hi:[0,1,0]\n\tv_cvt_rpi_i32_f32 %0, %0" : "=v"(qv) : "v"(dd), "v"(dw));
+            __hip_atomic_fetch_add((lds_i*)(size_t)a2 + t * TILE_F + j * 64, qv, __ATOMIC_RELAXED, __HIP_MEMORY_SCOPE_WORKGROUP);
+        }
+    };
+    auto accumulate = [&](const RowPieces& piece, float dv, uint32_t nv) {
+        if (nv == (uint32_t)KB) {
+#pragma unroll
+            for (int u = 0; u < KB; u++) {
+                const float dd = __uint_as_float(__builtin_amdgcn_readlane(__float_as_uint(dv), u));
+#pragma unroll
+                for (int t = 0; t < kRowsTiles; t++) if ((okMask >> t) & 1u) row(piece[u][t], dd, t);
+            }
+        } else {
+#pragma unroll
+            for (int u = 0; u < KB; u++) {
+                if ((uint32_t)u >= nv) continue;
+                const float dd = __uint_as_float(__builtin_amdgcn_readlane(__float_as_uint(dv), u));
+#pragma unroll
+                for (int t = 0; t < kRowsTiles; t++) if ((okMask >> t) & 1u) row(piece[u][t], dd, t);
+            }
+        }
+    };
+    auto stream_rows = [&](auto aux) {
+        RowPieces pa, pb;
+        uint32_t boffA, boffB; float dvA, dvB;
+        uint32_t baseA = (uint32_t)(wave * KB), baseB;
+        if (baseA < nU) { decode(baseA, boffA, dvA); issue(aux, pa, boffA); }
+        while (baseA < nU) {
+            baseB = grab();
+            decode(baseB, boffB, dvB);
+            issue(aux, pb, boffB);
+            accumulate(pa, dvA, __builtin_amdgcn_readfirstlane(min((uint32_t)KB, nU - baseA)));
+            baseA = grab();
+            decode(baseA, boffA, dvA);
+            issue(aux, pa, boffA);
+            accumulate(pb, dvB, __builtin_amdgcn_readfirstlane(baseB < nU ? min((uint32_t)KB, nU - baseB) : 0u));
+        }
+    };
+    if (kRowAux != 0 && (ga.split & 8u) != 0u) stream_rows(std::integral_constant<int, 0>{});
+    else stream_rows(std::integral_constant<int, kRowAux>{});
+    __syncthreads();
+
+    const uint32_t slabBytes = (uint32_t)min((size_t)0xFFFFFFFFu, (size_t)g.slices * tiles * TILE_F * 4);
+    const __amdgpu_buffer_rsrc_t srs = __builtin_amdgcn_make_buffer_rsrc(a_slabs, 0, (int)__builtin_amdgcn_readfirstlane(slabBytes), 0x00020000);
+    const uint32_t nSlices = g.slices, sliceStride = tiles * (uint32_t)(TILE_F * 4);
+    for (uint32_t t = 0; t < tiles; t++) {
+        const uint32_t slabOff = (s * tiles + t) * (uint32_t)(TILE_F * 4);
+        constexpr int kIt = TILE_F / (NT * 2);
+        float s0[kIt], s1[kIt];
+#pragma unroll
+        for (int it = 0; it < kIt; it++) {
+            const int o = tid * 2 + it * NT * 2;
+            s0[it] = (float)acc[t * TILE_F + o] * unscale; s1[it] = (float)acc[t * TILE_F + o + 1] * unscale;
+        }
+#pragma unroll
+        for (int it = 0; it < kIt; it++) {
+            const int o = tid * 2 + it * NT * 2;
+            typedef uint32_t u2 __attribute__((ext_vector_type(2)));
+            u2 pk; pk[0] = __float_as_uint(s0[it]); pk[1] = __float_as_uint(s1[it]);
+            __builtin_amdgcn_raw_buffer_store_b64(pk, srs, (uint32_t)o * 4u, slabOff, kSc1);
+        }
+    }
+    asm volatile("s_waitcnt vmcnt(0)" ::: "memory");
+    __syncthreads();
+    if (tid == 0) {
+        uint32_t last = 0;
+        for (uint32_t t = 0; t < tiles; t++) {
+            const uint32_t ticket = __hip_atomic_fetch_add(&a_counters[t], 1u, __ATOMIC_RELAXED, __HIP_MEMORY_SCOPE_AGENT);
+            last |= (ticket == nSlices - 1u) ? (1u << t) : 0u;
+        }
+        flags[0] = last;
+    }
+    __syncthreads();
+    const uint32_t last = __builtin_amdgcn_readfirstlane(flags[0]);
+    typedef uint32_t u4v __attribute__((ext_vector_type(4)));
+    auto reduce_tile = [&](const uint32_t t, auto kc) {
+        constexpr int kRed = decltype(kc)::value;
+        for (int o = tid * 4; o < TILE_F; o += NT * 4) {
+            const uint32_t vo = t * (uint32_t)(TILE_F * 4) + (uint32_t)o * 4u;
+            float sm[4][4];
+#pragma unroll
+            for (int h = 0; h < 4; h++) { sm[h][0] = 0.0f; sm[h][1] = 0.0f; sm[h][2] = 0.0f; sm[h][3] = 0.0f; }
+            for (uint32_t sl = 0; sl < nSlices; sl += kRed) {
+                u4v r[kRed];
+#pragma unroll
+                for (int i = 0; i < kRed; i++)
+                    r[i] = __builtin_amdgcn_raw_buffer_load_b128(srs, vo, min(sl + i, nSlices - 1u) * sliceStride, kSc1);
+#pragma unroll
+                for (int i = 0; i < kRed; i++) {
+                    if (sl + i < nSlices) {
+#pragma unroll
+                        for (int h = 0; h < 4; h++) sm[h][i & 3] += __uint_as_float(r[i][h]);
+                    }
+                }
+            }
+#pragma unroll
+            for (int h = 0; h < 4; h++) {
+                const float tot = (sm[h][0] + sm[h][1]) + (sm[h][2] + sm[h][3]);
+                const uint32_t oo = (uint32_t)o + h;
+                const uint32_t lane2 = oo & 63u, sj = oo >> 6, j = sj % E, slot = sj / E;
+                const uint32_t c2 = t * (64u * E) + lane2 * E + j;
+                if (c2 < g.cols) a.out[c2 * 16u + slot] = tot;
+            }
+        }
+    };
+    for (uint32_t t = 0; t < tiles; t++) {
+        if (!((last >> t) & 1u)) continue;
+        if (nSlices <= 8u) reduce_tile(t, std::integral_constant<int, 8>{});
+        else reduce_tile(t, std::integral_constant<int, 16>{});
+        if (tid == 0) __hip_atomic_store(&a_counters[t], 0u, __ATOMIC_RELAXED, __HIP_MEMORY_SCOPE_AGENT);
+    }
+}
+
+__global__ __launch_bounds__(kRowsNT, 4) void bucket_rows_kernel(const GroupKArgs ga) {
+    extern __shared__ __attribute__((aligned(16))) char smem[];
+    __shared__ uint32_t s_item;
+    const uint32_t total = ga.totalItems + ga.cutJobs;
+    uint32_t cachedCall = 0xFFFFFFFFu; float cachedCutoff = 0.0f;
+    const uint32_t x = blockIdx.x & 7u;
+    uint32_t dry = 0;
+    auto pull = [&]() -> uint32_t {
+        uint32_t got = total;
+        for (uint32_t tries = 0; tries < 8u && got >= total; tries++) {
+            const uint32_t q = (x + tries) & 7u;
+            if ((dry >> q) & 1u) continue;
+            const uint32_t cand = __hip_atomic_fetch_add(&ga.queue[q * 16u], 1u, __ATOMIC_RELAXED, __HIP_MEMORY_SCOPE_AGENT) * 8u + q;
+            if (cand < total) got = cand; else dry |= 1u << q;
+        }
+        return got;
+    };
+    auto pull_sync = [&]() -> uint32_t {
+        if (threadIdx.x == 0) s_item = pull();
+        __syncthreads();
+        const uint32_t it = __builtin_amdgcn_readfirstlane(s_item);
+        __syncthreads();
+        return it;
+    };
+    const LdsPlan lp = ga.lp;
+    uint32_t item = pull_sync();
+    while (item < total) {
+        if (item < ga.cutJobs) {
+            if (item < ga.count) rows_cutoff_job(ga, item, smem, lp);
+        } else {
+            ItemRef ref;
+            if (rows_locate(ga, item - ga.cutJobs, ref)) rows_item(ga, ref, smem, lp, cachedCall, cachedCutoff);
+        }
+        item = pull_sync();
+    }
+    if (threadIdx.x == 0) {
+        const uint32_t gone = __hip_atomic_fetch_add(&ga.queue[8 * 16], 1u, __ATOMIC_RELAXED, __HIP_MEMORY_SCOPE_AGENT);
+        if (gone == gridDim.x - 1u) {
+            for (int i = 0; i <= 8; i++) __hip_atomic_store(&ga.queue[i * 16], 0u, __ATOMIC_RELAXED, __HIP_MEMORY_SCOPE_AGENT);
+            for (int i = 0; i < kMaxGroup; i++) __hip_atomic_store(&ga.queue[9 * 16 + i], 0u, __ATOMIC_RELAXED, __HIP_MEMORY_SCOPE_AGENT);
+        }
+    }
+}
+
+hipError_t bucket_rows_prepare_device(bool* twoPerCU) {
+    const void* f = reinterpret_cast<const void*>(&bucket_rows_kernel);
+    *twoPerCU = false;
+    hipFuncAttributes fa;
+    hipError_t e = hipFuncGetAttributes(&fa, f);
+    if (e != hipSuccess) return e;
+    if (fa.sharedSizeBytes > 1024u) return hipErrorInvalidValue;
+    e = hipFuncSetAttribute(f, hipFuncAttributeMaxDynamicSharedMemorySize, (int)(160u * 1024u - (uint32_t)fa.sharedSizeBytes));
+    if (e != hipSuccess) return e;
+    MulGeom g;
+    memset(&g, 0, sizeof(g));
+    g.slices = 8; g.slots = (uint32_t)kRounds * kRowsNT; g.sliceRows = 512;
+    int n = 0;
+    if (hipOccupancyMaxActiveBlocksPerMultiprocessor(&n, f, kRowsNT, rows_plan_lds(&g, 1).total) == hipSuccess) *twoPerCU = n >= 2;
+    return hipSuccess;
+}
+
+hipError_t launch_bucket_rows(const GroupKArgs& gaIn, hipStream_t st, LaunchedVariant* ran) {
+    GroupKArgs ga = gaIn;
+    if (!ga.persistent || !ga.cutJobs || !(ga.split & 4u) || (ga.split & 1u) || ga.tstamp || !ga.count) return hipErrorInvalidValue;
+    uint32_t end8 = 0;
+    for (uint32_t i = 0; i < ga.count; i++) {
+        const MulGeom& g = ga.geom[ga.call[i].geom];
+        if (g.elems != (uint32_t)kRowsE || g.tiles < 2u || g.tiles > (uint32_t)kRowsTiles || ga.call[i].pre || ga.call[i].resid) return hipErrorInvalidValue;
+        if (g.slots > (uint32_t)kRounds * kRowsNT || g.slots != (g.rowsPerIn << g.sliceLog2) || (1u << g.sliceLog2) > (uint32_t)kRowsNT || g.sliceRows % 2u) return hipErrorInvalidValue;
+        end8 += (g.slices + 7u) / 8u;
+        ga.wgEnd8[i] = (uint16_t)end8;
+    }
+    ga.totalItems = end8 * 8u;
+    const LdsPlan lp = ga.lp = rows_plan_lds(ga.geom, kMaxGeoms);
+    uint32_t lds = lp.total;
+    const uint32_t force = (160u * 1024u) / 3u + 512u;
+    if (lds < force) lds = force;
+    if (lds > 80u * 1024u || lp.offA > 65536u) return hipErrorInvalidValue;
+    uint32_t grid = ga.numCU * 2u;
+    if (grid > ga.totalItems + ga.cutJobs) grid = ga.totalItems + ga.cutJobs;
+    grid = (grid + 7u) / 8u * 8u;
+    if (ran) *ran = LaunchedVariant{(uint32_t)kRowsW, (uint32_t)kRowsE, 0u, 1u, 0u, ga.persistent, grid, ga.totalItems};
+    hipLaunchKernelGGL(bucket_rows_kernel, dim3(grid), dim3(kRowsNT), lds, st, ga);
+    return hipGetLastError();
+}
+
+}
diff --git a/effort_amd/csrc/effort_internal.h b/effort_amd/csrc/effort_internal.h
--- a/effort_amd/csrc/effort_internal.h
+++ b/effort_amd/csrc/effort_internal.h
@@ -174,6 +174,8 @@
 hipError_t launch_bucket_mul(Format fmt, int wavesPerGroup, int elemsPerLane, const GroupKArgs& ga, hipStream_t st, LaunchedVariant* ran = nullptr);
 int bucket_mul_variants(Format fmt, int* rows, int maxRows);
 hipError_t bucket_mul_prepare_device();
+hipError_t launch_bucket_rows(const GroupKArgs& ga, hipStream_t st, LaunchedVariant* ran = nullptr);
+hipError_t bucket_rows_prepare_device(bool* twoPerCU);
 hipError_t launch_find_cutoff_group(const GroupKArgs& ga, hipStream_t st);
 size_t bucket_mul_lds_bytes(Format fmt, int wavesPerGroup, int elemsPerLane, const MulGeom& g, bool lean);
 uint32_t bucket_mul_max_candidates(int wavesPerGroup);
diff --git a/effort_amd/csrc/plan.h b/effort_amd/csrc/plan.h
--- a/effort_amd/csrc/plan.h
+++ b/effort_amd/csrc/plan.h
@@ -48,5 +48,6 @@
 
 bool supported(int W, int E);
 int plan_group(Format fmt, const PlanEnv& env, int n, const PlanCall* calls, GroupPlan* plan);
+bool row_items(Format fmt, const PlanEnv& env, const GroupPlan& plan, uint32_t launch, int mode);
 
 }
diff --git a/effort_amd/csrc/plan.hip b/effort_amd/csrc/plan.hip
--- a/effort_amd/csrc/plan.hip
+++ b/effort_amd/csrc/plan.hip
@@ -285,4 +285,20 @@
     return EFFORT_OK;
 }
 
-}
+constexpr int kRowItemsMinLanes = 4;
+bool row_items(Format fmt, const PlanEnv& env, const GroupPlan& plan, uint32_t launch, int mode) {
+    if (mode == 0 || launch >= plan.nLaunches) return false;
+    const LaunchPlan& lp = plan.launch[launch];
+    if (fmt != kFp16 || plan.W != 8 || plan.E != 4 || !lp.persistent || !lp.cutJobs || !lp.compact || env.clock || env.ablate) return false;
+    uint32_t slices = 0;
+    for (uint32_t i = 0; i < lp.count; i++) {
+        const MulGeom& g = plan.call[lp.first + i].g;
+        if (g.tiles < 2u || g.tiles > 3u) return false;
+        slices += g.slices;
+    }
+    if (mode > 0) return true;
+    const bool tuned = env.tuneW || env.tuneE || env.tuneS;
+    return env.laned && env.nLanes >= kRowItemsMinLanes && !tuned && slices >= (uint32_t)env.numCU;
+}
+
+}
diff --git a/effort_amd/runtime.py b/effort_amd/runtime.py
--- a/effort_amd/runtime.py
+++ b/effort_amd/runtime.py
@@ -54,6 +54,15 @@
     def set_row_reuse(self, reuse: bool = True):
         self.check(self._lib.effort_set_row_reuse(self.ctx, int(bool(reuse))), "set_row_reuse")
 
+    def set_row_items(self, mode: int = -1):
+        self.check(self._lib.effort_set_row_items(self.ctx, int(mode)), "set_row_items")
+
+    def row_items(self, launch: int = 0) -> int:
+        k = self._lib.effort_debug_row_items(self.ctx, int(launch))
+        if k < 0:
+            self.check(k, "row_items")
+        return k
+
     @staticmethod
     def comm_unique_id() -> bytes:
         buf = (C.c_char * 128)()
@@ -182,6 +191,19 @@
     res.update({name: list(a[:n]) for name, a in zip(("slices", "tiles", "sliceRows", "launch"), per_call)})
     res.update({name: list(a[:k]) for name, a in zip(("persistent", "cutJobs", "compact", "stagger"), per_launch)})
     return res
+
+
+def plan_row_items(calls, *, mode: int = -1, q4: bool = False, numCU: int = 256, lanes: int = 1, persistent: int = -1, waves: int = 0, elems: int = 0,
+                   slices: int = 0) -> list[int]:
+    n = len(calls)
+    rows = [tuple(c) + (16, 0, 0)[len(c) - 3:] for c in calls]
+    ints = lambda k: (C.c_int * n)(*[int(r[k]) for r in rows])
+    out = (C.c_int * max(n, 2))()
+    k = _lib.lib().effort_debug_plan_row_items(int(q4), numCU, lanes, n, ints(0), ints(1), ints(3), ints(4), ints(5), (C.c_double * n)(*[float(r[2]) for r in rows]),
+                                               persistent, waves, elems, slices, int(mode), out)
+    if k < 0:
+        raise _lib.EffortError(k, "plan_row_items")
+    return list(out[:k])
 
 
 def variants(q4: bool = False) -> list[tuple]:
diff --git a/include/effort_hip_debug.h b/include/effort_hip_debug.h
--- a/include/effort_hip_debug.h
+++ b/include/effort_hip_debug.h
@@ -26,6 +26,11 @@
                       const int* prologue, const int* hasResid, const double* effort, int persistent, int tuneW, int tuneE, int tuneS,
                       int* we, int* slices, int* tiles, int* sliceRows, int* launchOf,
                       int* launchPersistent, int* launchCutJobs, int* launchCompact, int* launchStagger);
+EFFORT_API int effort_set_row_items(effort_ctx* ctx, int mode);
+EFFORT_API int effort_debug_plan_row_items(int q4, int numCU, int lanes, int n, const int* inDim, const int* outDim, const int* percentLoad,
+                      const int* prologue, const int* hasResid, const double* effort, int persistent, int tuneW, int tuneE, int tuneS,
+                      int mode, int* rows);
+EFFORT_API int effort_debug_row_items(effort_ctx* ctx, int launch);
 EFFORT_API int effort_debug_check_bundle(int q4, int inDim, int outDim, int percentLoad, int numExperts, int rowPitchBytes);
 EFFORT_API int effort_debug_variants(int q4, int* rows, int maxRows);
 EFFORT_API int effort_debug_last_variant(effort_ctx* ctx, int launch, int* out8);
```

Result: slower. 16310 (-24.0%).
